# Mingqj/DFU3D

Hardware: AMD Instinct MI355X
Metric: pseudo-box frames/sec (34k pts, 6 cams) (higher is better)
Workload: dtype f64; 1 GPU; configs[1] with depth back-projection on (dense): 64 synthetic frames/GPU/step, 34720-pt sweep, 6 cams x 1600x900 depth + 8 instance masks (one bit-packed 1-byte word per pixel), 30-40 objects/scene; views_per_launch_chunk=192, streams=2, parallelism=frames sharded x1

## Files before the change

dfu3d_amd/_build.py:

```python
import glob
import os
import subprocess
import sys

HERE = os.path.dirname(os.path.abspath(__file__))
CSRC = os.path.join(HERE, "csrc")
INCLUDE = os.path.join(os.path.dirname(HERE), "include")
OUT = os.path.join(CSRC, "libdfu3d_hip.so")

FLAGS = [
    "--offload-arch=gfx950", "-O3", "-std=c++17", "-fPIC", "-shared",
    "-ffp-contract=off", "-fhip-fp32-correctly-rounded-divide-sqrt",
    "-fno-fast-math", "-Wall", "-Wno-unused-function",
]


def sources():
    return sorted(glob.glob(os.path.join(CSRC, "*.hip")))


def needs_build():
    return _stale(OUT)


def _deps():
    return (sources() + glob.glob(os.path.join(CSRC, "*.hpp")) + glob.glob(os.path.join(CSRC, "*.inc"))
            + [os.path.join(INCLUDE, "dfu3d.h")])


def _stale(out):
    return not os.path.exists(out) or any(os.path.getmtime(d) > os.path.getmtime(out) for d in _deps())


def _compile(out, extra, verbose):
    import fcntl
    import tempfile
    with open(out + ".lock", "w") as lock:
        fcntl.flock(lock, fcntl.LOCK_EX)
        try:
            if not _stale(out) and not extra.get("force"):
                return out
            hipcc = os.environ.get("HIPCC", "/opt/rocm/bin/hipcc")
            fd, tmp = tempfile.mkstemp(prefix=os.path.basename(out) + ".", suffix=".tmp", dir=os.path.dirname(out))
            os.close(fd)
            cmd = [hipcc] + FLAGS + extra.get("flags", []) + ["-I", INCLUDE, "-I", CSRC] + sources() + ["-o", tmp]
            if verbose:
                print(" ".join(cmd))
            try:
                subprocess.check_call(cmd)
                os.replace(tmp, out)
            finally:
                if os.path.exists(tmp):
                    os.unlink(tmp)
        finally:
            fcntl.flock(lock, fcntl.LOCK_UN)
    return out


def build(force=False, verbose=False):
    if not force and not needs_build():
        return OUT
    return _compile(OUT, {"force": force, "flags": os.environ.get("DFU3D_EXTRA_HIPCC_FLAGS", "").split()}, verbose)


VARIANTS = {
    "keybits14": ["-DDFU3D_DBG_COMBO_KEYBITS=14"],
    "no_mid": ["-DDFU3D_DBG_NO_MID"],
    "timing": ["-DDFU3D_DBG_TIMING"],
    "asan_host": ["-O1", "-g", "-Xarch_host", "-fsanitize=address", "-Xarch_host", "-fsanitize=undefined",
                  "-Xarch_host", "-fno-sanitize-recover=undefined", "-Xarch_host", "-fno-omit-frame-pointer", "-shared-libsan"],
}


def variant_path(name):
    return os.path.join(CSRC, "libdfu3d_hip_%s.so" % name)


def build_variant(name, force=False, verbose=False):
    out = variant_path(name)
    if not force and not _stale(out):
        return out
    return _compile(out, {"force": force, "flags": VARIANTS[name]}, verbose)


if __name__ == "__main__":
    print(build(force="--force" in sys.argv, verbose=True))
```

dfu3d_amd/csrc/chain_stage.hip:

```cpp
#include "common.hpp"

namespace {

struct ChainWs {
  int32_t *fov_idx, *cand_idx, *ag_pt, *ib_pix, *n_fov, *n_ag, *K;
  double *plane;
  uint32_t *a_bits;
  double *a_x, *a_y, *a_z;
  int32_t *n_vox;
  uint32_t *vox_pix, *b_bits;
  double *b_x, *b_y, *b_z;
  void *table;
  uint32_t *pix_bin;
  int32_t *blk_cnt;
  double *px, *py, *pz, *sx, *sy;
  int32_t *label, *sroot, *si3;
  double *fit_ws;
  uint8_t *flags;
  int64_t *base_a, *base_b, *base_ab;
  int32_t *cnt_a, *cnt_b, *cnt_all, *cnt_ab, *tile_off, *queue, *stat_enable;
  double *rad_ab, *mean_d;
  void *vd_scratch;
  void *shadow;
  int32_t *chunk_cnt;
  int64_t *pool_cursor;
  int64_t table_entries;
};

int64_t carve(const dfu3d_chain_cfg *c, char *base, ChainWs *w) {
  int64_t off = 0;
  auto take = [&](int64_t bytes) -> char * {
    char *p = base ? base + off : nullptr;
    off += (bytes + 255) / 256 * 256;
    return p;
  };
  const int64_t V = c->V, S = (int64_t)c->V * c->max_inst, N = V * c->cap_n, X = V * c->cap_vox, P = c->pool_cap;
  ChainWs t;
  t.fov_idx = (int32_t *)take(4 * N); t.cand_idx = (int32_t *)take(4 * N);
  t.ag_pt = (int32_t *)take(4 * N); t.ib_pix = (int32_t *)take(4 * N);
  t.n_fov = (int32_t *)take(4 * V); t.n_ag = (int32_t *)take(4 * V); t.K = (int32_t *)take(4 * V);
  t.plane = (double *)take(8 * V * 4);
  t.a_bits = (uint32_t *)take(4 * N);
  t.a_x = (double *)take(8 * N); t.a_y = (double *)take(8 * N); t.a_z = (double *)take(8 * N);
  t.n_vox = (int32_t *)take(4 * V);
  t.vox_pix = (uint32_t *)take(4 * X); t.b_bits = (uint32_t *)take(4 * X);
  t.b_x = (double *)take(8 * X); t.b_y = (double *)take(8 * X); t.b_z = (double *)take(8 * X);
  t.table_entries = (int64_t)c->geom.t_n * c->geom.p_n;
  int64_t pw = 0, bw = 0;
  if (c->dense) {
    dfu3d_backproject_scratch_words(c->V, c->H, c->W, c->cap_vox, c->geom.max_points_per_voxel, t.table_entries, &pw, &bw);
    t.table = take(V * t.table_entries * DFU3D_TABLE_ENTRY_BYTES);
    t.pix_bin = (uint32_t *)take(4 * pw);
    t.blk_cnt = (int32_t *)take(4 * bw);
  } else {
    t.table = nullptr; t.pix_bin = nullptr; t.blk_cnt = nullptr;
  }
  t.px = (double *)take(8 * P); t.py = (double *)take(8 * P); t.pz = (double *)take(8 * P);
  t.sx = (double *)take(8 * P); t.sy = (double *)take(8 * P);
  t.label = (int32_t *)take(4 * P); t.sroot = (int32_t *)take(4 * P); t.si3 = (int32_t *)take(4 * 3 * P);
  t.fit_ws = (double *)take(8 * dfu3d_lshape_fit_ws_doubles(P, c->cap_rows));
  t.flags = (uint8_t *)take(P);
  t.base_a = (int64_t *)take(8 * S); t.base_b = (int64_t *)take(8 * S); t.base_ab = (int64_t *)take(8 * 2 * S);
  t.cnt_a = (int32_t *)take(4 * S); t.cnt_b = (int32_t *)take(4 * S); t.cnt_all = (int32_t *)take(4 * S);
  t.cnt_ab = (int32_t *)take(4 * 2 * S); t.tile_off = (int32_t *)take(4 * (2 * S + 2));
  t.queue = (int32_t *)take(4 * DFU3D_RF_QUEUE_INTS(P)); t.stat_enable = (int32_t *)take(4 * S);
  t.shadow = take(DFU3D_SHADOW_BYTES(P));
  t.chunk_cnt = (int32_t *)take(4 * dfu3d_segments_scratch_words(c->V, c->cap_n, c->cap_vox));
  t.rad_ab = (double *)take(8 * 2 * S);
  t.mean_d = c->stat_filter ? (double *)take(8 * P) : nullptr;
  t.vd_scratch = c->stat_filter ? (void *)take(dfu3d_voxel_down_sample_scratch_bytes(P)) : nullptr;
  t.pool_cursor = (int64_t *)take(8);
  if (w) *w = t;
  return off;
}

bool cfg_ok(const dfu3d_chain_cfg *c) {
  return c && c->V > 0 && c->H > 0 && c->W > 0 && c->max_inst > 0 && c->max_inst <= DFU3D_MAX_INST &&
         c->cap_n > 0 && c->cap_vox > 0 && c->cap_rows > 0 && c->pool_cap > 0 && c->n_theta > 0 &&
         c->bounds_h > 0 && c->bounds_w > 0 && c->bounds_h <= c->H && c->bounds_w <= c->W &&
         mask_format_ok(c->mask_format, c->max_inst) &&
         (!c->dense || (c->geom.t_n > 0 && c->geom.p_n > 0)) &&
         (!c->stat_filter || (c->stat_voxel > 0.0 && c->stat_nb_neighbors >= 1));
}

__global__ void k_all_points(const int *__restrict__ pt_off, const int *__restrict__ view_frame,
                             int cap_n, int *__restrict__ fov_idx, int *__restrict__ n_fov) {
  const int v = blockIdx.y;
  const int f = view_frame[v];
  const int n = min(pt_off[f + 1] - pt_off[f], cap_n);
  for (int i = blockIdx.x * blockDim.x + threadIdx.x; i < cap_n; i += gridDim.x * blockDim.x)
    fov_idx[(size_t)v * cap_n + i] = i;
  if (blockIdx.x == 0 && threadIdx.x == 0) n_fov[v] = n;
}

__global__ void k_sum_counts(int S, const int *__restrict__ a, const int *__restrict__ b, int *__restrict__ out) {
  const int s = blockIdx.x * blockDim.x + threadIdx.x;
  if (s < S) out[s] = a[s] + b[s];
}

__global__ void k_fill_i32(int n, int v, int *__restrict__ p) {
  const int i = blockIdx.x * blockDim.x + threadIdx.x;
  if (i < n) p[i] = v;
}

}

extern "C" int64_t dfu3d_chain_workspace_bytes(const dfu3d_chain_cfg *cfg) {
  if (!cfg_ok(cfg)) return DFU3D_EINVAL;
  return carve(cfg, nullptr, nullptr);
}

extern "C" int64_t dfu3d_workspace_bytes(int32_t stage, const dfu3d_sizes *z) {
  if (!z || z->V <= 0 || z->max_inst <= 0 || z->max_inst > DFU3D_MAX_INST) return DFU3D_EINVAL;
  auto up = [](int64_t b) { return (b + 255) / 256 * 256; };
  const int64_t V = z->V, S = V * z->max_inst, P = z->pool_cap, N = V * (int64_t)z->cap_n;
  switch (stage) {
    case DFU3D_STAGE_FOV_FILTER:
      return 0;
    case DFU3D_STAGE_SEGMENTS_BUILD:
      return (z->cap_n > 0 && z->cap_vox > 0) ? up(4 * dfu3d_segments_scratch_words(z->V, z->cap_n, z->cap_vox)) : DFU3D_EINVAL;
    case DFU3D_STAGE_PLANE_RANSAC:
      return z->cap_n > 0 ? up(4 * N) : DFU3D_EINVAL;
    case DFU3D_STAGE_PROJECT_LABEL:
      return z->cap_n > 0 ? 2 * up(4 * N) : DFU3D_EINVAL;
    case DFU3D_STAGE_BACKPROJECT_BIN: {
      int64_t pw = 0, bw = 0;
      if (z->table_entries <= 0 ||
          dfu3d_backproject_scratch_words(z->V, z->H, z->W, z->cap_vox, z->max_points_per_voxel, z->table_entries, &pw, &bw))
        return DFU3D_EINVAL;
      return up(V * z->table_entries * DFU3D_TABLE_ENTRY_BYTES) + up(4 * pw) + up(4 * bw);
    }
    case DFU3D_STAGE_RADIUS_FILTER:
      return P > 0 ? up(DFU3D_SHADOW_BYTES(P)) + up(4 * (2 * S + 1)) + up(P) + up(4 * DFU3D_RF_QUEUE_INTS(P)) : DFU3D_EINVAL;
    case DFU3D_STAGE_STAT_FILTER:
      return P > 0 ? up(4 * (S + 1)) + up(P) + up(8 * P) : DFU3D_EINVAL;
    case DFU3D_STAGE_VOXEL_DOWN_SAMPLE:
      return P > 0 ? up(dfu3d_voxel_down_sample_scratch_bytes(P)) : DFU3D_EINVAL;
    case DFU3D_STAGE_BALLQUERY_FUSE:
      return P > 0 ? up(4 * (2 * S + 2)) + up(P) : DFU3D_EINVAL;
    case DFU3D_STAGE_RANGE_CLUSTER:
      return P > 0 ? 2 * up(8 * P) + up(12 * P) : DFU3D_EINVAL;
    case DFU3D_STAGE_LSHAPE_FIT:
      return (P > 0 && z->cap_rows > 0)
                 ? 2 * up(8 * P) + up(4 * P) + up(8 * dfu3d_lshape_fit_ws_doubles(P, z->cap_rows)) : DFU3D_EINVAL;
    case DFU3D_STAGE_PSEUDO_BOXES: {
      dfu3d_chain_cfg c = {};
      c.V = z->V; c.H = z->H; c.W = z->W; c.max_inst = z->max_inst; c.cap_n = z->cap_n; c.cap_vox = z->cap_vox;
      c.cap_rows = z->cap_rows; c.dense = z->dense; c.stat_filter = z->stat_filter; c.pool_cap = z->pool_cap;
      c.bounds_h = z->H; c.bounds_w = z->W; c.n_theta = 1;
      c.geom.max_points_per_voxel = z->max_points_per_voxel;
      c.geom.t_n = 1; c.geom.p_n = (int32_t)z->table_entries;
      if (z->dense && (z->table_entries <= 0 || z->table_entries > 0x7FFFFFFF)) return DFU3D_EINVAL;
      return dfu3d_chain_workspace_bytes(&c);
    }
    default:
      return DFU3D_EINVAL;
  }
}

extern "C" int dfu3d_chain_workspace_init(const dfu3d_chain_cfg *cfg, void *workspace, void *stream) {
  DFU3D_CLEAR_STALE_ERROR();
  if (!cfg_ok(cfg) || !workspace) return DFU3D_EINVAL;
  ChainWs w;
  carve(cfg, (char *)workspace, &w);
  if (cfg->dense) {
    const int rc = dfu3d_bin_table_init(w.table, (int64_t)cfg->V * w.table_entries, stream);
    if (rc) return rc;
  }
  hipLaunchKernelGGL(k_fill_i32, dim3((cfg->V * cfg->max_inst + 255) / 256), dim3(256), 0,
                     (hipStream_t)stream, cfg->V * cfg->max_inst, 1, w.stat_enable);
  DFU3D_LAUNCH_CHECK();
  return DFU3D_OK;
}

#define CHAIN_TRY(call)      \
  do {                       \
    const int rc_ = (call);  \
    if (rc_) return rc_;     \
  } while (0)

extern "C" int dfu3d_pseudo_boxes(
    const dfu3d_chain_cfg *cfg, const float *points, const int32_t *pt_off,
    const int32_t *view_frame, const float *calib, const void *masks, const int32_t *n_inst,
    const float *depth, const int64_t *view_key, const double *plane_in, const int32_t *inst_class,
    const int32_t *inst_is_car, const double *inst_r_lidar, const double *inst_r_pseudo,
    const float *inst_box, const float *inst_score, void *workspace, double *rows, int32_t *n_rows,
    uint32_t *status, void *stream) {
  DFU3D_CLEAR_STALE_ERROR();
  if (!cfg_ok(cfg) || !points || !pt_off || !view_frame || !calib || !masks || !n_inst || !inst_class ||
      !inst_is_car || !inst_r_lidar || !inst_r_pseudo || !inst_box || !inst_score || !workspace || !rows ||
      !n_rows || !status)
    return DFU3D_EINVAL;
  if (!plane_in && !view_key) return DFU3D_EINVAL;
  if (cfg->dense && !depth) return DFU3D_EINVAL;
  ChainWs w;
  carve(cfg, (char *)workspace, &w);
  hipStream_t st = (hipStream_t)stream;
  const int V = cfg->V, M = cfg->max_inst, S = V * M, cap_n = cfg->cap_n;
  if (dfu3d_fill_small_async(n_rows, sizeof(int32_t), status, sizeof(uint32_t), w.pool_cursor, sizeof(int64_t), st) != hipSuccess)
    return DFU3D_ELAUNCH;
  if (cfg->apply_fov) {
    CHAIN_TRY(dfu3d_fov_filter(points, pt_off, view_frame, calib, V, cfg->fov_h, cfg->fov_w, cap_n,
                               w.fov_idx, w.n_fov, stream));
  } else {
    hipLaunchKernelGGL(k_all_points, dim3((cap_n + 255) / 256 < 64 ? (cap_n + 255) / 256 : 64, V), dim3(256), 0, st,
                       pt_off, view_frame, cap_n, w.fov_idx, w.n_fov);
    DFU3D_LAUNCH_CHECK();
  }
  const double *plane = plane_in;
  if (!plane) {
    CHAIN_TRY(dfu3d_plane_ransac(points, pt_off, view_frame, w.fov_idx, w.n_fov, V, cap_n, cfg->plane_max_hs,
                                 cfg->plane_range, cfg->ransac_trials, cfg->ransac_seed, view_key,
                                 w.cand_idx, w.plane, stream));
    plane = w.plane;
  }
  CHAIN_TRY(dfu3d_project_label(points, pt_off, view_frame, calib, plane, w.fov_idx, w.n_fov, masks,
                                cfg->mask_format, n_inst, V, M, cfg->H, cfg->W, cfg->bounds_h, cfg->bounds_w,
                                cap_n, cfg->plane_offset, cfg->plane_range, w.ag_pt,
                                w.ib_pix, w.n_ag, w.K, w.a_bits, w.a_x, w.a_y, w.a_z, stream));
  if (cfg->dense) {
    CHAIN_TRY(dfu3d_backproject_bin(depth, calib, masks, cfg->mask_format, n_inst, V, M, cfg->H, cfg->W, &cfg->geom, 1, w.table,
                                    w.pix_bin, w.blk_cnt, cfg->cap_vox, w.n_vox, w.vox_pix, w.b_bits, w.b_x,
                                    w.b_y, w.b_z, status, DFU3D_BP_ALL, stream));
  } else {
    if (dfu3d_fill_async(w.n_vox, 0, sizeof(int32_t) * V, st) != hipSuccess) return DFU3D_ELAUNCH;
  }
  const bool joint = !cfg->stat_filter;
  CHAIN_TRY(dfu3d_segments_build(w.a_bits, w.a_x, w.a_y, w.a_z, w.K, cap_n, w.b_bits, w.b_x, w.b_y, w.b_z,
                                 w.n_vox, cfg->cap_vox, V, M, cfg->pool_cap, w.pool_cursor, w.px, w.py, w.pz,
                                 w.base_a, w.cnt_a, w.base_b, w.cnt_b, status, inst_r_lidar, inst_r_pseudo,
                                 joint ? w.shadow : nullptr, joint ? w.base_ab : nullptr, w.cnt_ab, w.rad_ab,
                                 w.chunk_cnt, stream));
  if (joint) {
    CHAIN_TRY(dfu3d_radius_filter(w.px, w.py, w.pz, w.base_ab, w.cnt_ab, w.rad_ab, cfg->nb_points, 2 * S,
                                  cfg->pool_cap, w.pool_cursor, w.shadow, w.tile_off, w.flags, w.queue,
                                  DFU3D_RF_FLAGS | DFU3D_RF_RESOLVE, stream));
    CHAIN_TRY(dfu3d_ballquery_fuse_joint(w.px, w.py, w.pz, w.base_a, w.cnt_a, w.base_b, w.cnt_b, cfg->fuse_C,
                                          S, cfg->pool_cap, w.tile_off, w.flags, stream));
  } else {
    CHAIN_TRY(dfu3d_radius_filter(w.px, w.py, w.pz, w.base_a, w.cnt_a, inst_r_lidar, cfg->nb_points, S,
                                  cfg->pool_cap, w.pool_cursor, w.shadow, w.tile_off, w.flags, w.queue,
                                  DFU3D_RF_ALL, stream));
    CHAIN_TRY(dfu3d_radius_filter(w.px, w.py, w.pz, w.base_b, w.cnt_b, inst_r_pseudo, cfg->nb_points, S,
                                  cfg->pool_cap, w.pool_cursor, w.shadow, w.tile_off, w.flags, w.queue,
                                  DFU3D_RF_ALL, stream));
    CHAIN_TRY(dfu3d_voxel_down_sample(w.px, w.py, w.pz, w.base_b, w.cnt_b, w.stat_enable, cfg->stat_voxel, S,
                                      cfg->pool_cap, w.vd_scratch, status, stream));
    CHAIN_TRY(dfu3d_stat_filter(w.px, w.py, w.pz, w.base_b, w.cnt_b, w.stat_enable, cfg->stat_nb_neighbors,
                                cfg->stat_std_ratio, S, cfg->pool_cap, w.tile_off, w.flags, w.mean_d, nullptr,
                                stream));
    CHAIN_TRY(dfu3d_ballquery_fuse(w.px, w.py, w.pz, w.base_a, w.cnt_a, w.base_b, w.cnt_b, cfg->fuse_C, S,
                                   cfg->pool_cap, w.tile_off, w.flags, stream));
  }
  hipLaunchKernelGGL(k_sum_counts, dim3((S + 255) / 256), dim3(256), 0, st, S, w.cnt_a, w.cnt_b, w.cnt_all);
  DFU3D_LAUNCH_CHECK();
  CHAIN_TRY(dfu3d_range_cluster(w.px, w.py, w.base_a, w.cnt_all, S, cfg->R0, cfg->Rd, w.label, w.sx, w.sy,
                                w.si3, cfg->pool_cap, stream));
  CHAIN_TRY(dfu3d_lshape_fit(w.px, w.py, w.pz, w.label, w.base_a, w.cnt_all, S, M, calib, inst_class,
                             inst_is_car, inst_box, inst_score, cfg->n_theta, cfg->dtheta, cfg->car_aspect_max,
                             w.sx, w.sy, w.sroot, cfg->cap_rows, rows, n_rows, status, w.fit_ws, cfg->pool_cap,
                             stream));
  return DFU3D_OK;
}
```

dfu3d_amd/csrc/common.hpp:

```cpp
#pragma once
#include <hip/hip_runtime.h>
#include <stdint.h>

#include "dfu3d.h"

#define DFU3D_WAVE 64

struct ViewCalib {
  float M43[12];
  float P2[12];
  float cu, cv, fu, fv, tx, ty;
  float Minv[12];
  float pad[6];
};
static_assert(sizeof(ViewCalib) == DFU3D_CALIB_FLOATS * 4, "calib record");

__device__ __forceinline__ int lane_id() { return threadIdx.x & 63; }

__device__ __forceinline__ int wave_rank(bool flag, int &wave_total) {
  const unsigned long long m = __ballot(flag);
  wave_total = __popcll(m);
  return __popcll(m & ((1ull << lane_id()) - 1ull));
}

template <int NW>
__device__ __forceinline__ int block_rank(bool flag, int *s_w, int &block_total) {
  int wt;
  const int r = wave_rank(flag, wt);
  const int w = threadIdx.x >> 6;
  if (lane_id() == 0) s_w[w] = wt;
  __syncthreads();
  int off = 0, tot = 0;
#pragma unroll
  for (int i = 0; i < NW; i++) {
    const int c = s_w[i];
    off += (i < w) ? c : 0;
    tot += c;
  }
  __syncthreads();
  block_total = tot;
  return off + r;
}

template <int CTRL, int ROW_MASK>
__device__ __forceinline__ int dpp_move_i(int old, int v) {
  return __builtin_amdgcn_update_dpp(old, v, CTRL, ROW_MASK, 0xF, false);
}
__device__ __forceinline__ int wave_incl_scan(int v) {
  v += dpp_move_i<0x111, 0xF>(0, v);
  v += dpp_move_i<0x112, 0xF>(0, v);
  v += dpp_move_i<0x114, 0xF>(0, v);
  v += dpp_move_i<0x118, 0xF>(0, v);
  v += dpp_move_i<0x142, 0xA>(0, v);
  v += dpp_move_i<0x143, 0xC>(0, v);
  return v;
}
__device__ __forceinline__ int wave_sum_i_dpp(int v) {
  v += dpp_move_i<0xB1, 0xF>(v, v);
  v += dpp_move_i<0x4E, 0xF>(v, v);
  v += dpp_move_i<0x141, 0xF>(v, v);
  v += dpp_move_i<0x140, 0xF>(v, v);
  v += dpp_move_i<0x142, 0xA>(0, v);
  v += dpp_move_i<0x143, 0xC>(0, v);
  return __builtin_amdgcn_readlane(v, 63);
}
__device__ __forceinline__ int wave_min_i_dpp(int v) {
  v = min(v, dpp_move_i<0xB1, 0xF>(v, v));
  v = min(v, dpp_move_i<0x4E, 0xF>(v, v));
  v = min(v, dpp_move_i<0x141, 0xF>(v, v));
  v = min(v, dpp_move_i<0x140, 0xF>(v, v));
  v = min(v, dpp_move_i<0x142, 0xA>(v, v));
  v = min(v, dpp_move_i<0x143, 0xC>(v, v));
  return __builtin_amdgcn_readlane(v, 63);
}
__device__ __forceinline__ uint32_t wave_or_u32_dpp(uint32_t x) {
  int v = (int)x;
  v |= dpp_move_i<0xB1, 0xF>(v, v);
  v |= dpp_move_i<0x4E, 0xF>(v, v);
  v |= dpp_move_i<0x141, 0xF>(v, v);
  v |= dpp_move_i<0x140, 0xF>(v, v);
  v |= dpp_move_i<0x142, 0xA>(0, v);
  v |= dpp_move_i<0x143, 0xC>(0, v);
  return (uint32_t)__builtin_amdgcn_readlane(v, 63);
}

template <int NW>
__device__ __forceinline__ int block_excl_scan(int v, int *s_w, int &block_total) {
  const int inc = wave_incl_scan(v);
  const int w = threadIdx.x >> 6;
  if (lane_id() == 63) s_w[w] = inc;
  __syncthreads();
  int off = 0, tot = 0;
#pragma unroll
  for (int i = 0; i < NW; i++) {
    const int c = s_w[i];
    off += (i < w) ? c : 0;
    tot += c;
  }
  __syncthreads();
  block_total = tot;
  return off + inc - v;
}

__device__ __forceinline__ double shfl_xor_d(double v, int m) {
  int lo = __double2loint(v), hi = __double2hiint(v);
  lo = __shfl_xor(lo, m, 64);
  hi = __shfl_xor(hi, m, 64);
  return __hiloint2double(hi, lo);
}
__device__ __forceinline__ double wave_sum_d(double v) {
#pragma unroll
  for (int m = 32; m >= 1; m >>= 1) v += shfl_xor_d(v, m);
  return v;
}
template <int CTRL, int ROW_MASK>
__device__ __forceinline__ double dpp_move_d(double v) {
  int lo = __double2loint(v), hi = __double2hiint(v);
  lo = __builtin_amdgcn_update_dpp(lo, lo, CTRL, ROW_MASK, 0xF, false);
  hi = __builtin_amdgcn_update_dpp(hi, hi, CTRL, ROW_MASK, 0xF, false);
  return __hiloint2double(hi, lo);
}
__device__ __forceinline__ double min_f64_raw(double a, double b) {
  double r;
  asm("v_min_f64 %0, %1, %2" : "=v"(r) : "v"(a), "v"(b));
  return r;
}
__device__ __forceinline__ double max_f64_raw(double a, double b) {
  double r;
  asm("v_max_f64 %0, %1, %2" : "=v"(r) : "v"(a), "v"(b));
  return r;
}
__device__ __forceinline__ double lane63_d(double v) {
  return __hiloint2double(__builtin_amdgcn_readlane(__double2hiint(v), 63), __builtin_amdgcn_readlane(__double2loint(v), 63));
}
__device__ __forceinline__ double wave_min_d(double v) {
  v = min_f64_raw(v, dpp_move_d<0xB1, 0xF>(v));
  v = min_f64_raw(v, dpp_move_d<0x4E, 0xF>(v));
  v = min_f64_raw(v, dpp_move_d<0x141, 0xF>(v));
  v = min_f64_raw(v, dpp_move_d<0x140, 0xF>(v));
  v = min_f64_raw(v, dpp_move_d<0x142, 0xA>(v));
  v = min_f64_raw(v, dpp_move_d<0x143, 0xC>(v));
  return lane63_d(v);
}
__device__ __forceinline__ double wave_max_d(double v) {
  v = max_f64_raw(v, dpp_move_d<0xB1, 0xF>(v));
  v = max_f64_raw(v, dpp_move_d<0x4E, 0xF>(v));
  v = max_f64_raw(v, dpp_move_d<0x141, 0xF>(v));
  v = max_f64_raw(v, dpp_move_d<0x140, 0xF>(v));
  v = max_f64_raw(v, dpp_move_d<0x142, 0xA>(v));
  v = max_f64_raw(v, dpp_move_d<0x143, 0xC>(v));
  return lane63_d(v);
}
__device__ __forceinline__ unsigned long long wave_sum_u64(unsigned long long v) {
#pragma unroll
  for (int m = 32; m >= 1; m >>= 1) {
    const unsigned int lo = (unsigned int)__shfl_xor((int)(v & 0xFFFFFFFFull), m, 64);
    const unsigned int hi = (unsigned int)__shfl_xor((int)(v >> 32), m, 64);
    v += ((unsigned long long)hi << 32) | lo;
  }
  return v;
}
__device__ __forceinline__ int wave_sum_i(int v) { return wave_sum_i_dpp(v); }

__device__ __forceinline__ void lidar_to_rect_f32(const float *M, float x, float y,
                                                  float z, float r[3]) {
#pragma unroll
  for (int j = 0; j < 3; j++) {
    float acc = x * M[0 * 3 + j];
    acc = __fmaf_rn(y, M[1 * 3 + j], acc);
    acc = __fmaf_rn(z, M[2 * 3 + j], acc);
    acc = acc + M[3 * 3 + j];
    r[j] = acc;
  }
}
__device__ __forceinline__ void rect_to_img_f32(const float *P2, const float r[3],
                                                float &u, float &v, float &depth) {
  float h[3];
#pragma unroll
  for (int j = 0; j < 3; j++) {
    float acc = r[0] * P2[j * 4 + 0];
    acc = __fmaf_rn(r[1], P2[j * 4 + 1], acc);
    acc = __fmaf_rn(r[2], P2[j * 4 + 2], acc);
    acc = acc + P2[j * 4 + 3];
    h[j] = acc;
  }
  u = h[0] / r[2];
  v = h[1] / r[2];
  depth = h[2] - P2[2 * 4 + 3];
}
struct Recip { double rfu, rfv; };
__device__ __forceinline__ Recip make_recip(const ViewCalib &c) {
  Recip r;
  r.rfu = 1.0 / (double)c.fu;
  r.rfv = 1.0 / (double)c.fv;
  return r;
}
__device__ __forceinline__ double div_reused(double a, double b, double r) {
  const double q0 = a * r;
  const uint32_t hi = (uint32_t)__double2hiint(q0) & 0x7FFFFFFFu;
  if (__builtin_expect(hi - 0x07B00000u >= 0x78400000u - 0x07B00000u, 0)) return a / b;
  const double rem = fma(-q0, b, a);
  return fma(rem, r, q0);
}
__device__ __forceinline__ void pixel_to_lidar(const ViewCalib &c, const Recip &rc, int u, int v,
                                               float d, double &x, double &y,
                                               double &z) {
  const double dd = (double)d;
  const double xr = div_reused(((double)u - (double)c.cu) * dd, (double)c.fu, rc.rfu) + (double)c.tx;
  const double yr = div_reused(((double)v - (double)c.cv) * dd, (double)c.fv, rc.rfv) + (double)c.ty;
  const double zr = dd;
  const float *M = c.Minv;
  x = fma(zr, (double)M[6], fma(yr, (double)M[3], xr * (double)M[0])) + (double)M[9];
  y = fma(zr, (double)M[7], fma(yr, (double)M[4], xr * (double)M[1])) + (double)M[10];
  z = fma(zr, (double)M[8], fma(yr, (double)M[5], xr * (double)M[2])) + (double)M[11];
}
struct KeyCol { float m0, m3, m6, m9; };
__device__ __forceinline__ KeyCol load_key_col(const ViewCalib *c, int axis) {
  const float *M = c->Minv + axis;
  KeyCol k;
  k.m0 = M[0]; k.m3 = M[3]; k.m6 = M[6]; k.m9 = M[9];
  return k;
}
struct KeyCal { float cu, cv, fu, fv, tx, ty; };
__device__ __forceinline__ KeyCal key_cal(const ViewCalib &c) { return KeyCal{c.cu, c.cv, c.fu, c.fv, c.tx, c.ty}; }
template <class Cal>
__device__ __forceinline__ double pixel_to_lidar_axis(const Cal &c, const Recip &rc, const KeyCol &kc, int u, int v,
                                                      float d) {
  const double dd = (double)d;
  const double xr = div_reused(((double)u - (double)c.cu) * dd, (double)c.fu, rc.rfu) + (double)c.tx;
  const double yr = div_reused(((double)v - (double)c.cv) * dd, (double)c.fv, rc.rfv) + (double)c.ty;
  return fma(dd, (double)kc.m6, fma(yr, (double)kc.m3, xr * (double)kc.m0)) + (double)kc.m9;
}

__host__ __device__ inline bool mask_format_ok(int fmt, int max_inst) {
  return fmt == 0 || (fmt == 1 && max_inst <= 8) || (fmt == 2 && max_inst <= 16) || fmt == 4;
}
__device__ __forceinline__ uint32_t mask_bits_at(const void *masks, int fmt, int v, int max_inst, int m,
                                                 int HW, int pix) {
  if (fmt == 0) {
    const uint8_t *mb = (const uint8_t *)masks + (size_t)v * max_inst * HW + pix;
    uint32_t bits = 0u;
    for (int j = 0; j < m; j++) bits |= (mb[(size_t)j * HW] > 0) ? (1u << j) : 0u;
    return bits;
  }
  const size_t o = (size_t)v * HW + pix;
  const uint32_t w = fmt == 1 ? (uint32_t)((const uint8_t *)masks)[o]
                   : fmt == 2 ? (uint32_t)((const uint16_t *)masks)[o] : ((const uint32_t *)masks)[o];
  return m >= 32 ? w : (w & ((1u << m) - 1u));
}

__device__ __forceinline__ unsigned long long ordered_key(double v) {
  const unsigned long long b = (unsigned long long)__double_as_longlong(v);
  return (b & 0x8000000000000000ull) ? ~b : (b | 0x8000000000000000ull);
}

__device__ __forceinline__ unsigned long long mix64(unsigned long long z) {
  z += 0x9E3779B97F4A7C15ull;
  z = (z ^ (z >> 30)) * 0xBF58476D1CE4E5B9ull;
  z = (z ^ (z >> 27)) * 0x94D049BB133111EBull;
  return z ^ (z >> 31);
}

#define DFU3D_CLEAR_STALE_ERROR() (void)hipGetLastError()

#define DFU3D_LAUNCH_CHECK()                                      \
  do {                                                            \
    if (hipGetLastError() != hipSuccess) return DFU3D_ELAUNCH;    \
  } while (0)

namespace {
__global__ __launch_bounds__(256) void k_fill_words(uint32_t *__restrict__ p, size_t n, uint32_t v) {
  const size_t head = ((16u - (unsigned)((uintptr_t)p & 15u)) & 15u) / 4u < n ? ((16u - (unsigned)((uintptr_t)p & 15u)) & 15u) / 4u : n;
  uint4 *q = (uint4 *)(p + head);
  const size_t nq = (n - head) / 4;
  const size_t tid = (size_t)blockIdx.x * 256 + threadIdx.x, nth = (size_t)gridDim.x * 256;
  for (size_t i = tid; i < nq; i += nth) q[i] = make_uint4(v, v, v, v);
  const size_t done = head + nq * 4;
  if (tid < head) p[tid] = v;
  if (tid < n - done) p[done + tid] = v;
}
__global__ void k_fill_small(uint32_t *a, int na, uint32_t *b, int nb, uint32_t *c, int nc, uint32_t v) {
  for (int i = threadIdx.x; i < na; i += blockDim.x) a[i] = v;
  for (int i = threadIdx.x; i < nb; i += blockDim.x) b[i] = v;
  for (int i = threadIdx.x; i < nc; i += blockDim.x) c[i] = v;
}
}
static inline hipError_t dfu3d_fill_async(void *p, int value, size_t bytes, hipStream_t st) {
  if (bytes == 0) return hipSuccess;
  if (((uintptr_t)p & 3u) || (bytes & 3u)) return hipMemsetAsync(p, value, bytes, st);
  const uint32_t b = (uint32_t)(value & 0xFF), v = b | (b << 8) | (b << 16) | (b << 24);
  const size_t n = bytes / 4, quads = (n + 3) / 4;
  const unsigned grid = (unsigned)((quads + 255) / 256 < 8192 ? (quads + 255) / 256 : 8192);
  hipLaunchKernelGGL(k_fill_words, dim3(grid ? grid : 1), dim3(256), 0, st, (uint32_t *)p, n, v);
  return hipGetLastError();
}
static inline hipError_t dfu3d_fill_small_async(void *a, size_t bytes_a, void *b, size_t bytes_b, void *c, size_t bytes_c, hipStream_t st) {
  hipLaunchKernelGGL(k_fill_small, dim3(1), dim3(256), 0, st, (uint32_t *)a, (int)(bytes_a / 4), (uint32_t *)b, (int)(bytes_b / 4),
                     (uint32_t *)c, (int)(bytes_c / 4), 0u);
  return hipGetLastError();
}
```

dfu3d_amd/csrc/dbg.hpp:

```cpp
#pragma once

#ifdef DFU3D_DBG_COMBO_KEYBITS
constexpr int DBG_COMBO_KEYBITS = DFU3D_DBG_COMBO_KEYBITS;
#else
constexpr int DBG_COMBO_KEYBITS = 64;
#endif

#ifdef DFU3D_DBG_NO_MID
constexpr bool DBG_NO_MID = true;
#else
constexpr bool DBG_NO_MID = false;
#endif

#ifdef DFU3D_DBG_TIMING
constexpr int DBG_T_SLOTS = 32;
static __device__ unsigned long long g_dbg_cycles[DBG_T_SLOTS];
#define DBG_T_START() long long dbg_t_ = clock64(); const long long dbg_t0_ = dbg_t_; (void)dbg_t0_
#define DBG_T(k) do { if (threadIdx.x == 0) { const long long t_ = clock64(); atomicAdd(&g_dbg_cycles[k], (unsigned long long)(t_ - dbg_t_)); dbg_t_ = t_; } } while (0)
#define DBG_T_COUNT(k) do { if (threadIdx.x == 0) atomicAdd(&g_dbg_cycles[k], 1ull); } while (0)
#define DBG_T_ADD(k, v) do { if (threadIdx.x == 0) atomicAdd(&g_dbg_cycles[k], (unsigned long long)(v)); } while (0)
#define DBG_T_MAX(k, v) do { if (threadIdx.x == 0) atomicMax(&g_dbg_cycles[k], (unsigned long long)(v)); } while (0)
#define DBG_T_READER(name)                                                                                              \
  extern "C" int name(unsigned long long *out, int reset) {                                                            \
    if (hipMemcpyFromSymbol(out, HIP_SYMBOL(g_dbg_cycles), sizeof(unsigned long long) * DBG_T_SLOTS) != hipSuccess)     \
      return DFU3D_ELAUNCH;                                                                                             \
    if (reset) {                                                                                                        \
      unsigned long long z[DBG_T_SLOTS] = {0};                                                                          \
      if (hipMemcpyToSymbol(HIP_SYMBOL(g_dbg_cycles), z, sizeof(z)) != hipSuccess) return DFU3D_ELAUNCH;                \
    }                                                                                                                   \
    return DFU3D_OK;                                                                                                    \
  }
#else
#define DBG_T_START() do {} while (0)
#define DBG_T(k) do {} while (0)
#define DBG_T_COUNT(k) do {} while (0)
#define DBG_T_ADD(k, v) do {} while (0)
#define DBG_T_MAX(k, v) do {} while (0)
#define DBG_T_READER(name)
#endif
```

dfu3d_amd/csrc/fit_stage.hip:

```cpp
#include "common.hpp"

namespace {
__device__ __forceinline__ int rl_i(int v, int l) { return __builtin_amdgcn_readlane(v, l); }
__device__ __forceinline__ double rl_d(double v, int l) {
  return __hiloint2double(__builtin_amdgcn_readlane(__double2hiint(v), l), __builtin_amdgcn_readlane(__double2loint(v), l));
}

constexpr int CT = 512;
constexpr int GRP = 32;
constexpr int BLK = 32;
constexpr int PAIR_SMALL = 32;
constexpr int GU = 4;
constexpr int SMALL_N = 4096;
constexpr int LARGE_N = 61440;
constexpr int LARGE_GRP = LARGE_N / GRP;
constexpr int GRID_NC_SMALL = 4096;
constexpr int GRID_NC_LARGE = 12288;

struct ParI {
  int *p;
  bool global;
  __device__ __forceinline__ int load(int i) const {
    return __hip_atomic_load(p + i, __ATOMIC_RELAXED, __HIP_MEMORY_SCOPE_AGENT);
  }
// ... 353 lines not shown
__device__ __forceinline__ int grid_cell(const GridGeom<NC> &G, double x, double y, int &cx, int &cy) {
  cx = (int)fmin(fmax((x - G.x0) * G.inv, 0.0), (double)(G.nx - 1));
  cy = (int)fmin(fmax((y - G.y0) * G.inv, 0.0), (double)(G.ny - 1));
  return (int)__umul24((uint32_t)cy, (uint32_t)G.nx) + cx;
}
template <int NC>
__device__ __forceinline__ int grid_cell(const GridGeom<NC> &G, double x, double y) {
  int cx, cy;
  return grid_cell(G, x, y, cx, cy);
}

__device__ __forceinline__ int cell_find(int *par_, int a) {
  volatile int *par = par_;
  int p = par[a];
  while (p != a) {
    const int gp = par[p];
    if (gp != p) par[a] = gp;
    a = p;
    p = gp;
  }
  return a;
}
__device__ __forceinline__ void cell_unite(int *par, int a, int b) {
  while (true) {
    a = cell_find(par, a);
    b = cell_find(par, b);
    if (a == b) return;
    if (a < b) { const int t = a; a = b; b = t; }
    const int old = atomicMin(par + a, b);
    if (old == a) return;
    a = old;
  }
}

constexpr int CL_CLASSES = 3, CL_TOP = 8192;
template <int NC, int NC_MIN, int TCT>
__global__ __launch_bounds__(TCT, (NC <= GRID_NC_SMALL ? 8 : 4)) void k_range_cluster_grid(
    const double *__restrict__ px, const double *__restrict__ py,
    const long long *__restrict__ seg_base, const int *__restrict__ seg_cnt, double R0,
    double Rd, int *__restrict__ label, double *__restrict__ sx, double *__restrict__ sy,
    int *__restrict__ perm_all, long long pool_cap, int n_lo, int n_hi) {
  __shared__ int s_end[NC];
  __shared__ int s_par[NC];
  __shared__ int s_min[NC];
  __shared__ double s_red[5 * (TCT / 64)];
  __shared__ int s_w[TCT / 64];
  constexpr int NCLS = CL_CLASSES;
  const int S_ = (int)(gridDim.x / (unsigned)NCLS);
  const int cls = (int)(blockIdx.x / (unsigned)S_);
  const int s = (int)(blockIdx.x - (unsigned)cls * (unsigned)S_);
  const int n = seg_cnt[s];
  if (n <= n_lo || n > n_hi) return;
  {
    int mine = NCLS - 1;
#pragma unroll
    for (int k = NCLS - 2; k >= 0; k--) if (n > (CL_TOP >> k)) mine = k;
    if (mine != cls) return;
  }
  const long long base = seg_base[s];
  const double *X = px + base, *Y = py + base;
  double *SX = sx + base, *SY = sy + base;
  int *perm = perm_all + base;
  int *mark = perm_all + 2 * pool_cap + base;
  if (NC_MIN > 0 && *mark) return;
  const GridGeom<NC> G = grid_geometry<NC, TCT>(X, Y, n, R0, Rd, s_red);
  if (threadIdx.x == 0 && (NC_MIN == 0 || G.ok)) *mark = G.ok ? 1 : 0;
  if (!G.ok) return;
  const int ncell = G.ncell;
  for (int c = threadIdx.x; c < ncell; c += TCT) { s_end[c] = 0; s_par[c] = c; s_min[c] = 0x7FFFFFFF; }
  __syncthreads();
  for (int i0 = threadIdx.x; i0 < n; i0 += GU * TCT) {
    double xs[GU], ys[GU];
#pragma unroll
    for (int u = 0; u < GU; u++) {
      const int i = i0 + u * TCT;
      xs[u] = (i < n) ? X[i] : 0.0; ys[u] = (i < n) ? Y[i] : 0.0;
    }
#pragma unroll
    for (int u = 0; u < GU; u++)
      if (i0 + u * TCT < n) atomicAdd(&s_end[grid_cell(G, xs[u], ys[u])], 1);
  }
  __syncthreads();
  {
    const int per = (ncell + TCT - 1) / TCT;
    const int c_lo = min((int)threadIdx.x * per, ncell), c_hi = min(c_lo + per, ncell);
    int mine = 0;
    for (int c = c_lo; c < c_hi; c++) mine += s_end[c];
    int tot;
    int run = block_excl_scan<TCT / 64>(mine, s_w, tot);
    for (int c = c_lo; c < c_hi; c++) { const int h = s_end[c]; s_end[c] = run; run += h; }
  }
  __syncthreads();
  for (int i0 = threadIdx.x; i0 < n; i0 += GU * TCT) {
    double xs[GU], ys[GU];
#pragma unroll
    for (int u = 0; u < GU; u++) {
      const int i = i0 + u * TCT;
      xs[u] = (i < n) ? X[i] : 0.0; ys[u] = (i < n) ? Y[i] : 0.0;
    }
#pragma unroll
    for (int u = 0; u < GU; u++) {
      const int i = i0 + u * TCT;
      if (i >= n) break;
      const int pos = atomicAdd(&s_end[grid_cell(G, xs[u], ys[u])], 1);
      SX[pos] = xs[u];
      SY[pos] = ys[u];
      perm[pos] = i;
    }
  }
  __syncthreads();
  const double S_HI = G.Rmax * G.Rmax * (1.0 + 1e-9);
  const double S_LO = R0 * R0 * (1.0 - 1e-12);
  const int lane = lane_id();
  int *s_box = s_min;
  for (int c = threadIdx.x; c < ncell; c += TCT) s_box[c] = (int)0x00FF00FFu;
  __syncthreads();
  for (int i0 = threadIdx.x; i0 < n; i0 += GU * TCT) {
    double xs[GU], ys[GU];
#pragma unroll
    for (int u = 0; u < GU; u++) {
      const int i = i0 + u * TCT;
      xs[u] = (i < n) ? SX[i] : 0.0; ys[u] = (i < n) ? SY[i] : 0.0;
    }
#pragma unroll
    for (int u = 0; u < GU; u++) {
      if (i0 + u * TCT >= n) break;
      int cx, cy;
      const int c = grid_cell(G, xs[u], ys[u], cx, cy);
      const double fu = (xs[u] - G.x0) * G.inv - (double)cx, fv = (ys[u] - G.y0) * G.inv - (double)cy;
      const unsigned ulo = (unsigned)(int)fmin(fmax(floor(fu * 256.0), 0.0), 255.0);
      const unsigned uhi = (unsigned)(int)fmin(fmax(ceil(fu * 256.0) - 1.0, 0.0), 255.0);
      const unsigned vlo = (unsigned)(int)fmin(fmax(floor(fv * 256.0), 0.0), 255.0);
      const unsigned vhi = (unsigned)(int)fmin(fmax(ceil(fv * 256.0) - 1.0, 0.0), 255.0);
      unsigned old = (unsigned)__hip_atomic_load(&s_box[c], __ATOMIC_RELAXED, __HIP_MEMORY_SCOPE_WORKGROUP);
      while (true) {
        const unsigned nw = min(old & 255u, ulo) | (max((old >> 8) & 255u, uhi) << 8) |
                            (min((old >> 16) & 255u, vlo) << 16) | (max(old >> 24, vhi) << 24);
        if (nw == old) break;
        const unsigned seen = (unsigned)atomicCAS(&s_box[c], (int)old, (int)nw);
        if (seen == old) break;
        old = seen;
      }
    }
  }
  __syncthreads();
  const double box_lim = S_HI * (1.0 + 1e-6) * (G.inv * G.inv);
  auto boxes_apart = [&](int c, int cx, int cy, int nbc, int qx, int qy) {
    const unsigned a = (unsigned)s_box[c], b = (unsigned)s_box[nbc];
    const int ax0 = cx * 256 + (int)(a & 255u), ax1 = cx * 256 + (int)((a >> 8) & 255u) + 1;
    const int ay0 = cy * 256 + (int)((a >> 16) & 255u), ay1 = cy * 256 + (int)(a >> 24) + 1;
    const int bx0 = qx * 256 + (int)(b & 255u), bx1 = qx * 256 + (int)((b >> 8) & 255u) + 1;
    const int by0 = qy * 256 + (int)((b >> 16) & 255u), by1 = qy * 256 + (int)(b >> 24) + 1;
    const int gx = max(max(bx0 - ax1, ax0 - bx1) - 2, 0), gy = max(max(by0 - ay1, ay0 - by1) - 2, 0);
    const double g2 = (double)(gx * gx + gy * gy) * (1.0 / 65536.0);
    return g2 > box_lim;
  };
  struct CellBox { double x0, x1, y0, y1; };
  auto cell_box = [&](int c) {
    const unsigned a = (unsigned)s_box[c];
    const int cx = c % G.nx, cy = c / G.nx;
    CellBox B;
    B.x0 = G.x0 + ((double)cx + (double)((int)(a & 255u) - 1) * (1.0 / 256.0)) * G.g;
    B.x1 = G.x0 + ((double)cx + (double)((int)((a >> 8) & 255u) + 2) * (1.0 / 256.0)) * G.g;
    B.y0 = G.y0 + ((double)cy + (double)((int)((a >> 16) & 255u) - 1) * (1.0 / 256.0)) * G.g;
    B.y1 = G.y0 + ((double)cy + (double)((int)(a >> 24) + 2) * (1.0 / 256.0)) * G.g;
    return B;
  };
  const double reach2 = S_HI * (1.0 + 1e-6);
  auto near_box = [&](const CellBox &B, double x, double y) {
    const double dx = fmax(fmax(B.x0 - x, x - B.x1), 0.0), dy = fmax(fmax(B.y0 - y, y - B.y1), 0.0);
    return dx * dx + dy * dy <= reach2;
  };
  const int ODX[12] = {1, -1, 0, 1, 2, -2, -1, 0, 1, 2, -2, 2};
  const int ODY[12] = {0, 1, 1, 1, 0, 2, 2, 2, 2, 2, 1, 1};
  for (int round = 0; round < 2; round++) {
    const int o_lo = round ? 4 : 0, n_off = round ? 8 : 4;
    const int items = ncell * n_off;
    const int iters = (items + TCT - 1) / TCT;
    for (int it = 0; it < iters; it++) {
      const int idx = it * TCT + threadIdx.x;
      int c = 0, nb = 0;
      bool need = false;
      if (idx < items) {
        c = idx / n_off;
        const int o = o_lo + (idx - c * n_off);
        const int cx = c % G.nx, cy = c / G.nx;
        const int qx = cx + ODX[o], qy = cy + ODY[o];
        if (qx >= 0 && qx < G.nx && qy < G.ny) {
          nb = qy * G.nx + qx;
          const int a0 = c ? s_end[c - 1] : 0, b0 = s_end[nb - 1];
          need = (s_end[c] > a0) && (s_end[nb] > b0) && !boxes_apart(c, cx, cy, nb, qx, qy) &&
                 (cell_find(s_par, c) != cell_find(s_par, nb));
        }
      }
      if (need) {
        const int a0 = c ? s_end[c - 1] : 0, a1 = s_end[c];
        const int b0 = s_end[nb - 1], b1 = s_end[nb];
        if (a1 - a0 <= PAIR_SMALL && b1 - b0 <= PAIR_SMALL) {
          need = false;
          bool found = false;
          const CellBox BB = cell_box(nb);
          for (int i = a0; i < a1 && !found; i++) {
            const double xa = SX[i], ya = SY[i];
            if (!near_box(BB, xa, ya)) continue;
            const double Ra = R0 + Rd * sqrt(xa * xa + ya * ya);
            for (int j0 = b0; j0 < b1 && !found; j0 += 4) {
              double xb4[4], yb4[4];
#pragma unroll
              for (int u = 0; u < 4; u++) {
                const int j = min(j0 + u, b1 - 1);
                xb4[u] = SX[j]; yb4[u] = SY[j];
              }
#pragma unroll
              for (int u = 0; u < 4; u++) {
                if (j0 + u >= b1) break;
                const double xb = xb4[u], yb = yb4[u];
                const double dx = xa - xb, dy = ya - yb;
                const double sq = dx * dx + dy * dy;
                if (sq > S_HI) continue;
                if (sq <= S_LO) { found = true; break; }
                const double d = sqrt(sq);
                if (d <= Ra || d <= R0 + Rd * sqrt(xb * xb + yb * yb)) { found = true; break; }
              }
            }
          }
          if (found) cell_unite(s_par, c, nb);
        }
      }
      unsigned long long todo = __ballot(need);
      while (todo) {
        const int src = __ffsll(todo) - 1;
        todo &= todo - 1ull;
        const int cc = rl_i(c, src), nn = rl_i(nb, src);
        if (cell_find(s_par, cc) == cell_find(s_par, nn)) continue;
        const int a0 = cc ? s_end[cc - 1] : 0, a1 = s_end[cc];
        const int b0 = s_end[nn - 1], b1 = s_end[nn];
        bool found = false;
        const CellBox BA = cell_box(cc), BB = cell_box(nn);
        for (int b_lo = b0; b_lo < b1 && !found; b_lo += 64) {
          const int ib = b_lo + lane;
          const double xb = (ib < b1) ? SX[ib] : 0.0, yb = (ib < b1) ? SY[ib] : 0.0;
          const bool vb = (ib < b1) && near_box(BA, xb, yb);
          if (!__any(vb)) continue;
          for (int a_lo = a0; a_lo < a1 && !found; a_lo += 64) {
            const int ia = a_lo + lane;
            const double xal = (ia < a1) ? SX[ia] : 0.0, yal = (ia < a1) ? SY[ia] : 0.0;
            unsigned long long am = __ballot((ia < a1) && near_box(BB, xal, yal));
            bool adj = false;
            int steps = 0;
            while (am) {
              const int k = __ffsll((long long)am) - 1;
              am &= am - 1ull;
              const double xa = rl_d(xal, k), ya = rl_d(yal, k);
              const double dx = xa - xb, dy = ya - yb;
              const double sq = dx * dx + dy * dy;
              if (vb && sq <= S_HI) {
                if (sq <= S_LO) adj = true;
                else {
                  const double d = sqrt(sq);
                  adj = adj || (d <= R0 + Rd * sqrt(xa * xa + ya * ya)) ||
                        (d <= R0 + Rd * sqrt(xb * xb + yb * yb));
                }
              }
              if ((++steps & 15) == 0 && __any(adj)) break;
            }
            found = __any(adj);
          }
        }
        if (found && lane == 0) cell_unite(s_par, cc, nn);
      }
    }
    __syncthreads();
  }
  for (int c = threadIdx.x; c < ncell; c += TCT) s_min[c] = 0x7FFFFFFF;
  __syncthreads();
  for (int i0 = threadIdx.x; i0 < n; i0 += GU * TCT) {
    double xs[GU], ys[GU];
    int pm[GU];
#pragma unroll
    for (int u = 0; u < GU; u++) {
      const int i = i0 + u * TCT;
      xs[u] = (i < n) ? SX[i] : 0.0; ys[u] = (i < n) ? SY[i] : 0.0; pm[u] = (i < n) ? perm[i] : 0;
    }
#pragma unroll
    for (int u = 0; u < GU; u++)
      if (i0 + u * TCT < n) atomicMin(&s_min[cell_find(s_par, grid_cell(G, xs[u], ys[u]))], pm[u]);
  }
  __syncthreads();
  int *glabel = label + base;
  for (int i0 = threadIdx.x; i0 < n; i0 += GU * TCT) {
    double xs[GU], ys[GU];
    int pm[GU];
#pragma unroll
    for (int u = 0; u < GU; u++) {
      const int i = i0 + u * TCT;
      xs[u] = (i < n) ? SX[i] : 0.0; ys[u] = (i < n) ? SY[i] : 0.0; pm[u] = (i < n) ? perm[i] : 0;
    }
#pragma unroll
    for (int u = 0; u < GU; u++)
      if (i0 + u * TCT < n) glabel[pm[u]] = s_min[cell_find(s_par, grid_cell(G, xs[u], ys[u]))];
  }
}

__global__ __launch_bounds__(CT) void k_range_cluster_small(
    const double *__restrict__ px, const double *__restrict__ py,
    const long long *__restrict__ seg_base, const int *__restrict__ seg_cnt, double R0,
    double Rd, int *__restrict__ label, double *__restrict__ sx, double *__restrict__ sy,
    int *__restrict__ si, long long pool_cap) {
  __shared__ __attribute__((aligned(16))) int s_parent[SMALL_N];
  __shared__ int s_summ[SMALL_N / GRP];
  __shared__ float4 s_box[SMALL_N / GRP];
  __shared__ int s_summ2[SMALL_N / GRP / BLK];
  __shared__ float4 s_box2[SMALL_N / GRP / BLK];
  __shared__ double s_red[4 * (CT / 64)];
  __shared__ int s_w[CT / 64];
  const int s = blockIdx.x;
  const int n = seg_cnt[s];
  if (n == 0 || n > SMALL_N) return;
  const long long base = seg_base[s];
  if (si[2 * pool_cap + base]) return;
  cell_sort<SMALL_N>(px + base, py + base, n, s_parent, s_red, s_w, sx + base, sy + base, si + base);
  ParI par{s_parent, false};
  cluster_body<ParI, SMALL_N / GRP>(par, s_summ, s_box, s_summ2, s_box2, s_red, sx + base, sy + base,
                                    n, R0, Rd, si + base, si + pool_cap + base, label + base);
}

__global__ __launch_bounds__(CT) void k_range_cluster_large(
    const double *__restrict__ px, const double *__restrict__ py,
    const long long *__restrict__ seg_base, const int *__restrict__ seg_cnt, double R0,
    double Rd, int *__restrict__ label, double *__restrict__ sx, double *__restrict__ sy,
    int *__restrict__ si, long long pool_cap) {
  __shared__ __attribute__((aligned(16))) unsigned short s_parent[LARGE_N];
  __shared__ int s_summ[LARGE_GRP];
  __shared__ float4 s_box[LARGE_GRP];
  __shared__ int s_summ2[LARGE_GRP / BLK];
  __shared__ float4 s_box2[LARGE_GRP / BLK];
  __shared__ double s_red[4 * (CT / 64)];
  __shared__ int s_w[CT / 64];
  const int s = blockIdx.x;
  const int n = seg_cnt[s];
  if (n <= SMALL_N) return;
  const long long base = seg_base[s];
  if (si[2 * pool_cap + base]) return;
  cell_sort<LARGE_N / 2>(px + base, py + base, n, (int *)s_parent, s_red, s_w, sx + base, sy + base,
                         si + base);
  if (n <= LARGE_N) {
    ParH par{s_parent};
    cluster_body<ParH, LARGE_GRP>(par, s_summ, s_box, s_summ2, s_box2, s_red, sx + base, sy + base,
                                  n, R0, Rd, si + base, si + pool_cap + base, label + base);
  } else {
    ParI par{si + 2 * pool_cap + base, true};
    cluster_body<ParI, LARGE_GRP>(par, s_summ, s_box, s_summ2, s_box2, s_red, sx + base, sy + base,
                                  n, R0, Rd, si + base, si + pool_cap + base, label + base);
  }
}

constexpr int FT = 512;
constexpr int FW = FT / 64;
constexpr int MAXTH = 128;
constexpr int LDS_MEMBERS = 2048;

struct OpSum { __device__ static double f(double a, double b) { return a + b; } };
struct OpMin { __device__ static double f(double a, double b) { return fmin(a, b); } };
struct OpMax { __device__ static double f(double a, double b) { return fmax(a, b); } };
template <class OP>
__device__ __forceinline__ double wave_red(double v) {
#pragma unroll
  for (int m = 32; m >= 1; m >>= 1) v = OP::f(v, shfl_xor_d(v, m));
  return v;
}

struct Ext { double c1min, c1max, c2min, c2max; };

__device__ __forceinline__ double readlane_f64(double v, int l) {
  const int lo = __builtin_amdgcn_readlane(__double2loint(v), l);
  const int hi = __builtin_amdgcn_readlane(__double2hiint(v), l);
  return __hiloint2double(hi, lo);
}

__device__ __forceinline__ void cross_point(double a0, double a1, double b0, double b1,
                                            double c0, double c1, double &x, double &y) {
  x = (b0 * -c1 - b1 * -c0) / (a0 * b1 - a1 * b0);
  y = (a1 * -c0 - a0 * -c1) / (a0 * b1 - a1 * b0);
}

__device__ void emit_box(double thb, double sin_s, double cos_s, double c1min, double c1max,
                         double c2min, double c2max, double zmax, int s, int v, int jinst, int kc,
                         int root, int m, const ViewCalib *calib, const int *inst_class,
                         const int *inst_is_car, const float *inst_box, const float *inst_score,
                         double car_aspect_max, int cap_rows, double *rows, int *n_rows,
                         uint32_t *status) {
  const double a[4] = {cos_s, -sin_s, cos_s, -sin_s};
  const double b[4] = {sin_s, cos_s, sin_s, cos_s};
  const double c[4] = {c1min, c2min, c1max, c2max};
  double cx[4], cy[4];
  cross_point(a[0], a[1], b[0], b[1], c[0], c[1], cx[0], cy[0]);
  cross_point(a[1], a[2], b[1], b[2], c[1], c[2], cx[1], cy[1]);
  cross_point(a[2], a[3], b[2], b[3], c[2], c[3], cx[2], cy[2]);
  cross_point(a[3], a[0], b[3], b[0], c[3], c[0], cx[3], cy[3]);
  double center_x = (cx[0] + cx[2]) / 2.0;
  double center_y = (cy[0] + cy[2]) / 2.0;
  const double center_z = zmax / 2.0 - 1.5;
  const double height = zmax;
  const double e03x = cx[0] - cx[3], e03y = cy[0] - cy[3];
  const double e01x = cx[0] - cx[1], e01y = cy[0] - cy[1];
  const double l1 = sqrt(e03x * e03x + e03y * e03y);
  const double l2 = sqrt(e01x * e01x + e01y * e01y);
  bool skip = false;
  if (inst_is_car[s] && (l1 / l2 > car_aspect_max || l2 / l1 > car_aspect_max)) skip = true;
  double length = 0.0, width = 0.0, rotation = 0.0;
  if (l1 >= l2) {
    length = l1; width = l2;
    rotation = atan((cy[3] - cy[0]) / (cx[3] - cx[0] + 1e-8));
  } else if (l1 < l2) {
    length = l2; width = l1;
    rotation = atan((cy[1] - cy[0]) / (cx[1] - cx[0] + 1e-8));
  } else {
    skip = true;
  }
  if (!skip) {
    const double kPi = 3.141592653589793;
    rotation = -rotation - kPi / 2.0;
    const double theta = atan(-center_x / (center_y + 1e-8));
    const double alpha = rotation - theta;
    const float *M = calib[v].M43;
    const double rx = ((center_x * (double)M[0] + center_y * (double)M[3]) + center_z * (double)M[6]) + (double)M[9];
    const double ry = ((center_x * (double)M[1] + center_y * (double)M[4]) + center_z * (double)M[7]) + (double)M[10];
    const double rz = ((center_x * (double)M[2] + center_y * (double)M[5]) + center_z * (double)M[8]) + (double)M[11];
    const int slot = atomicAdd(n_rows, 1);
    if (slot < cap_rows) {
      double *o = rows + (size_t)slot * DFU3D_ROW_DOUBLES;
      o[0] = (double)v; o[1] = (double)jinst; o[2] = (double)kc;
      o[3] = (double)inst_class[s]; o[4] = alpha;
      o[5] = (double)inst_box[s * 4 + 0]; o[6] = (double)inst_box[s * 4 + 1];
      o[7] = (double)inst_box[s * 4 + 2]; o[8] = (double)inst_box[s * 4 + 3];
      o[9] = height; o[10] = width; o[11] = length;
      o[12] = rx; o[13] = ry; o[14] = rz; o[15] = rotation;
      o[16] = (double)inst_score[s]; o[17] = (double)m;
      o[18] = thb; o[19] = c1min; o[20] = c2min; o[21] = c1max; o[22] = c2max;
      o[23] = (double)root;
    } else {
      atomicOr(status, DFU3D_ST_ROW_OVERFLOW);
    }
  }
}

struct FitWs {
  int *counters;
  double *dsc;
  int *big_list;
  double *big_cost;
  int cap_q, cap_big;
};
__host__ __device__ inline int fit_cap_q(int cap_rows) { return 2 * cap_rows + 64; }
__host__ __device__ inline FitWs fit_ws_view(double *ws, int cap_rows, int cap_big) {
  FitWs w;
  w.cap_q = fit_cap_q(cap_rows);
  w.cap_big = cap_big;
  w.counters = (int *)ws;
  w.dsc = ws + 2;
  w.big_list = (int *)(w.dsc + (size_t)8 * w.cap_q);
  w.big_cost = w.dsc + (size_t)8 * w.cap_q + (cap_big / 2 + 1);
  return w;
}

constexpr int GK = 512;

__device__ __forceinline__ int rank_in(const int *roots, int nk, int L) {
  int lo = 0, hi = nk - 1;
  while (lo < hi) {
    const int mid = (lo + hi) >> 1;
    if (roots[mid] < L) lo = mid + 1; else hi = mid;
  }
  return (roots[lo] == L) ? lo : -1;
}

constexpr int GGU = 4;
__global__ __launch_bounds__(FT) void k_fit_gather(
    const double *__restrict__ px, const double *__restrict__ py,
    const double *__restrict__ pz, const int *__restrict__ label,
    const long long *__restrict__ seg_base, const int *__restrict__ seg_cnt,
    double *__restrict__ gsx, double *__restrict__ gsy, int *__restrict__ sroot,
    uint32_t *__restrict__ status, double *__restrict__ fit_ws, int cap_rows, int cap_big) {
  __shared__ int s_roots[GK];
  __shared__ int s_cnt[FW][GK];
  __shared__ int s_tot[GK], s_off[GK];
  __shared__ double s_red[FW];
  __shared__ int s_w[FW];
  __shared__ int s_q0, s_total;
  const int S_ = (int)(gridDim.x / 3u);
  const int cls = (int)(blockIdx.x / (unsigned)S_);
  const int s = (int)(blockIdx.x - (unsigned)cls * (unsigned)S_);
  const int n = seg_cnt[s];
  if (n == 0) return;
  if (cls != (n > 16384 ? 0 : (n > 8192 ? 1 : 2))) return;
  const long long base = seg_base[s];
  const int wave = threadIdx.x >> 6, lane = lane_id();
  const FitWs W = fit_ws_view(fit_ws, cap_rows, cap_big);

  const int R = (((n + FW - 1) / FW) + 63) & ~63;
  const int r0 = min(n, wave * R), r1 = min(n, r0 + R);
  double zm = -INFINITY;
  int mine = 0;
  for (int c = r0; c < r1; c += 64 * GGU) {
    int L[GGU];
    double zz[GGU];
#pragma unroll
    for (int u = 0; u < GGU; u++) {
      const int i = c + u * 64 + lane;
      L[u] = (i < r1) ? label[base + i] : -1;
      zz[u] = (i < r1) ? pz[base + i] : -INFINITY;
    }
#pragma unroll
    for (int u = 0; u < GGU; u++) {
      const int i = c + u * 64 + lane;
      mine += __popcll(__ballot(i < r1 && L[u] == i));
      zm = fmax(zm, zz[u]);
    }
  }
  zm = wave_max_d(zm);
  if (lane == 0) { s_red[wave] = zm; s_w[wave] = mine; }
  __syncthreads();
  double zmax = s_red[0];
  int nroots = 0, my_off = 0;
#pragma unroll
  for (int w = 0; w < FW; w++) {
    zmax = fmax(zmax, s_red[w]);
    my_off += (w < wave) ? s_w[w] : 0;
    nroots += s_w[w];
  }
  for (int c = r0; c < r1; c += 64 * GGU) {
    int L[GGU];
#pragma unroll
    for (int u = 0; u < GGU; u++) {
      const int i = c + u * 64 + lane;
      L[u] = (i < r1) ? label[base + i] : -1;
    }
#pragma unroll
    for (int u = 0; u < GGU; u++) {
      const int i = c + u * 64 + lane;
      const bool f = (i < r1) && (L[u] == i);
      const unsigned long long m = __ballot(f);
      if (f) sroot[base + my_off + __popcll(m & ((1ull << lane) - 1ull))] = i;
      my_off += __popcll(m);
    }
  }
  if (threadIdx.x == 0) s_q0 = atomicAdd(&W.counters[0], nroots);
  __syncthreads();
  const int q0 = s_q0;

  long long goff = 0;
  for (int k0 = 0; k0 < nroots; k0 += GK) {
    const int nk = min(GK, nroots - k0);
    __syncthreads();
    if (threadIdx.x < nk) s_roots[threadIdx.x] = sroot[base + k0 + threadIdx.x];
    for (int i = threadIdx.x; i < FW * GK; i += FT) (&s_cnt[0][0])[i] = 0;
    __syncthreads();
    const int lo_root = s_roots[0], hi_root = s_roots[nk - 1];
    int memo_L = -2, memo_key = -1;
    for (int c0 = r0; c0 < r1; c0 += 64 * GGU) {
      int Ls[GGU];
#pragma unroll
      for (int u = 0; u < GGU; u++) {
        const int i = c0 + u * 64 + lane;
        Ls[u] = (i < r1) ? label[base + i] : -1;
      }
#pragma unroll
      for (int u = 0; u < GGU; u++) {
        if (c0 + u * 64 >= r1) break;
        const int L = Ls[u];
        int key = -1;
        if (L == memo_L) key = memo_key;
        else if (L >= lo_root && L <= hi_root) { key = rank_in(s_roots, nk, L); memo_L = L; memo_key = key; }
        unsigned long long rem = __ballot(key >= 0);
        while (rem) {
          const int src = __ffsll((long long)rem) - 1;
          const int k = rl_i(key, src);
          const unsigned long long m = __ballot(key == k);
          if (lane == src) s_cnt[wave][k] += __popcll(m);
          rem &= ~m;
        }
      }
    }
    __syncthreads();
    if (threadIdx.x < nk) {
      int t = 0;
#pragma unroll
      for (int w = 0; w < FW; w++) { const int c = s_cnt[w][threadIdx.x]; s_cnt[w][threadIdx.x] = t; t += c; }
      s_tot[threadIdx.x] = t;
    }
    __syncthreads();
    {
      int tot;
      const int ex = block_excl_scan<FW>(((int)threadIdx.x < nk) ? s_tot[threadIdx.x] : 0, s_w, tot);
      if ((int)threadIdx.x < nk) s_off[threadIdx.x] = ex;
      if (threadIdx.x == 0) s_total = tot;
    }
    __syncthreads();
    for (int c0 = r0; c0 < r1; c0 += 64 * GGU) {
      int keys[GGU];
      double xs[GGU], ys[GGU];
#pragma unroll
      for (int u = 0; u < GGU; u++) {
        const int i = c0 + u * 64 + lane;
        const int L = (i < r1) ? label[base + i] : -1;
        if (L == memo_L) keys[u] = memo_key;
        else if (L >= lo_root && L <= hi_root) { keys[u] = rank_in(s_roots, nk, L); memo_L = L; memo_key = keys[u]; }
        else keys[u] = -1;
      }
#pragma unroll
      for (int u = 0; u < GGU; u++) {
        const int i = c0 + u * 64 + lane;
        xs[u] = 0.0; ys[u] = 0.0;
        if (keys[u] >= 0) { xs[u] = px[base + i]; ys[u] = py[base + i]; }
      }
#pragma unroll
      for (int u = 0; u < GGU; u++) {
        if (c0 + u * 64 >= r1) break;
        const int key = keys[u];
        unsigned long long rem = __ballot(key >= 0);
        while (rem) {
          const int src = __ffsll((long long)rem) - 1;
          const int k = rl_i(key, src);
          const unsigned long long m = __ballot(key == k);
          const int cur = s_cnt[wave][k];
          if (key == k) {
            const long long d = base + goff + s_off[k] + cur + __popcll(m & ((1ull << lane) - 1ull));
            gsx[d] = xs[u];
            gsy[d] = ys[u];
          }
          if (lane == src) s_cnt[wave][k] = cur + __popcll(m);
          rem &= ~m;
        }
      }
    }
    if (threadIdx.x < nk) {
      const int k = threadIdx.x, e = q0 + k0 + k;
      if (e < W.cap_q) {
        double *d = W.dsc + (size_t)8 * e;
        const int m = s_tot[k];
        d[0] = (double)s; d[1] = (double)(k0 + k); d[2] = (double)s_roots[k]; d[3] = (double)m;
        d[4] = (double)(base + goff + s_off[k]); d[5] = zmax; d[6] = -1.0; d[7] = 0.0;
        if (m > LDS_MEMBERS) {
          const int bi = atomicAdd(&W.counters[1], 1);
          if (bi < cap_big) { W.big_list[bi] = e; d[6] = (double)bi; }
        }
// ... 196 lines not shown
          }
          double V1 = 0.0, V2 = 0.0;
          if (n1) V1 = -(q1 / (double)n1);
          if (n2) V2 = -(q2 / (double)n2);
          const double c = V1 + V2;
          if (c1t[k] >= band && bestc < c) { bestc = c; bestth = th; }
        }
      }
    }
#pragma unroll
    for (int msk = 32; msk >= 1; msk >>= 1) {
      const double oc = shfl_xor_d(bestc, msk);
      const int ot = __shfl_xor(bestth, msk, 64);
      if (oc > bestc || (oc == bestc && ot < bestth)) { bestc = oc; bestth = ot; }
    }
    const int best = (bestth == 0x7FFFFFFF) ? 0 : bestth;
    const double thb = (double)best * dtheta;
    const double sin_s = sin(thb), cos_s = cos(thb);
    double a0 = INFINITY, a1 = -INFINITY, b0 = INFINITY, b1 = -INFINITY;
    if (lane < m) {
      const double c1 = x * cos_s + y * sin_s;
      const double c2 = x * (-sin_s) + y * cos_s;
      a0 = c1; a1 = c1; b0 = c2; b1 = c2;
    }
    a0 = wave_min_d(a0); a1 = wave_max_d(a1);
    b0 = wave_min_d(b0); b1 = wave_max_d(b1);
    if (lane == 0) {
      const int s = (int)d[0], kc = (int)d[1], root = (int)d[2];
      const int v = s / max_inst, jinst = s - v * max_inst;
      emit_box(thb, sin_s, cos_s, a0, a1, b0, b1, d[5], s, v, jinst, kc, root, m, calib, inst_class,
               inst_is_car, inst_box, inst_score, car_aspect_max, cap_rows, rows, n_rows, status);
    }
  }
}

__global__ __launch_bounds__(FT, 8) void k_fit_medium(
    const double *__restrict__ gsx, const double *__restrict__ gsy, int max_inst,
    const ViewCalib *__restrict__ calib, const int *__restrict__ inst_class,
    const int *__restrict__ inst_is_car, const float *__restrict__ inst_box,
    const float *__restrict__ inst_score, int n_theta, double dtheta, double car_aspect_max,
    int cap_rows, double *__restrict__ rows, int *__restrict__ n_rows,
    uint32_t *__restrict__ status, double *__restrict__ fit_ws, int cap_big) {
  __shared__ double lx[LDS_MEMBERS], ly[LDS_MEMBERS];
  __shared__ double s_cost[MAXTH], s_mag[MAXTH], s_ct[MAXTH], s_st[MAXTH];
  __shared__ double s_ext[FW][4];
  const FitWs W = fit_ws_view(fit_ws, cap_rows, cap_big);
  const int nq = min(W.counters[0], W.cap_q);
  const int wave = threadIdx.x >> 6, lane = lane_id();
  if (threadIdx.x < MAXTH) {
    const double theta = (double)threadIdx.x * dtheta;
    s_ct[threadIdx.x] = cos(theta);
    s_st[threadIdx.x] = sin(theta);
  }
  __shared__ int s_item;
  while (true) {
    __syncthreads();
    if (wave == 0) {
      const int ticket = atomicAdd(&W.counters[3], 1);
      if (lane == 0) s_item = ticket >> 6;
    }
    __syncthreads();
    const int e = s_item;
    if (e >= nq) break;
    const double *d = W.dsc + (size_t)8 * e;
    const int m = (int)d[3];
    if (m <= 64 || m > LDS_MEMBERS) continue;
    __syncthreads();
    const long long P = (long long)d[4];
    for (int i = threadIdx.x; i < m; i += FT) { lx[i] = gsx[P + i]; ly[i] = gsy[P + i]; }
    __syncthreads();
    const double *mx = lx;
    const double *my = ly;
    for (int th0 = 2 * wave; th0 < n_theta; th0 += 2 * FW) {
      const int th1 = min(th0 + 1, n_theta - 1);
      const double ct0 = s_ct[th0], st0 = s_st[th0], ct1 = s_ct[th1], st1 = s_st[th1];
      double a0 = INFINITY, a1 = -INFINITY, b0 = INFINITY, b1 = -INFINITY;
      double e0 = INFINITY, e1 = -INFINITY, f0 = INFINITY, f1 = -INFINITY;
      for (int i = lane; i < m; i += 64) {
        const double x = mx[i], y = my[i];
        double c1 = x * ct0 + y * st0;
        double c2 = x * (-st0) + y * ct0;
        a0 = min_raw_d(a0, c1); a1 = max_raw_d(a1, c1);
        b0 = min_raw_d(b0, c2); b1 = max_raw_d(b1, c2);
        c1 = x * ct1 + y * st1;
        c2 = x * (-st1) + y * ct1;
        e0 = min_raw_d(e0, c1); e1 = max_raw_d(e1, c1);
        f0 = min_raw_d(f0, c2); f1 = max_raw_d(f1, c2);
      }
      a0 = wave_min_d(a0); a1 = wave_max_d(a1); b0 = wave_min_d(b0); b1 = wave_max_d(b1);
      e0 = wave_min_d(e0); e1 = wave_max_d(e1); f0 = wave_min_d(f0); f1 = wave_max_d(f1);
      FitAcc A, B;
      A.clear(); B.clear();
      for (int i = lane; i < m; i += 64) {
        const double x = mx[i], y = my[i];
        A.add(x, y, ct0, st0, a0, a1, b0, b1);
        B.add(x, y, ct1, st1, e0, e1, f0, f1);
      }
      A.wave_reduce(); B.wave_reduce();
      double magA, magB;
      const double cA = A.cost(magA), cB = B.cost(magB);
      if (lane == 0) { s_cost[th0] = cA; s_mag[th0] = magA; s_cost[th1] = cB; s_mag[th1] = magB; }
    }
    __syncthreads();
    double magmax = 0.0;
    for (int th = 0; th < n_theta; th++) { const double g = s_mag[th]; if (g > magmax) magmax = g; }
    const int best = wave_pick_heading(s_cost, n_theta, magmax, mx, my, m, s_ct, s_st);
    const double thb = (double)best * dtheta;
    const double sin_s = sin(thb), cos_s = cos(thb);
    {
      double a0 = INFINITY, a1 = -INFINITY, b0 = INFINITY, b1 = -INFINITY;
      for (int i = threadIdx.x; i < m; i += FT) {
        const double x = mx[i], y = my[i];
        const double c1 = x * cos_s + y * sin_s;
        const double c2 = x * (-sin_s) + y * cos_s;
        a0 = fmin(a0, c1); a1 = fmax(a1, c1);
        b0 = fmin(b0, c2); b1 = fmax(b1, c2);
      }
      a0 = wave_min_d(a0); a1 = wave_max_d(a1);
      b0 = wave_min_d(b0); b1 = wave_max_d(b1);
      if (lane == 0) { s_ext[wave][0] = a0; s_ext[wave][1] = a1; s_ext[wave][2] = b0; s_ext[wave][3] = b1; }
    }
    __syncthreads();
    if (threadIdx.x == 0) {
      double c1min = s_ext[0][0], c1max = s_ext[0][1], c2min = s_ext[0][2], c2max = s_ext[0][3];
      for (int w = 1; w < FW; w++) {
        c1min = fmin(c1min, s_ext[w][0]); c1max = fmax(c1max, s_ext[w][1]);
        c2min = fmin(c2min, s_ext[w][2]); c2max = fmax(c2max, s_ext[w][3]);
      }
      const int s = (int)d[0], kc = (int)d[1], root = (int)d[2];
      const int v = s / max_inst, jinst = s - v * max_inst;
      emit_box(thb, sin_s, cos_s, c1min, c1max, c2min, c2max, d[5], s, v, jinst, kc, root, m, calib,
               inst_class, inst_is_car, inst_box, inst_score, car_aspect_max, cap_rows, rows,
               n_rows, status);
    }
  }
}

constexpr int BIGC_T = 512, BIGC_WAVES = BIGC_T / 64, BIGC_HPW = 2, BIGC_HB = BIGC_WAVES * BIGC_HPW;
constexpr int BIGC_CH = 4096;
constexpr int BIGC_LONG = 16384, BIGC_MID = 6144;
__global__ __launch_bounds__(BIGC_T) void k_fit_big_cost(const double *__restrict__ gsx,
                                                         const double *__restrict__ gsy, int n_theta,
                                                         double dtheta, double *__restrict__ fit_ws,
                                                         int cap_rows, int cap_big) {
  __shared__ double lx[BIGC_CH], ly[BIGC_CH];
  __shared__ double s_ct[MAXTH], s_st[MAXTH];
  __shared__ int s_item;
  const FitWs W = fit_ws_view(fit_ws, cap_rows, cap_big);
  const int nbig = min(W.counters[1], cap_big);
  if (nbig == 0) return;
  if (threadIdx.x < MAXTH) {
    const double theta = (double)threadIdx.x * dtheta;
    s_ct[threadIdx.x] = cos(theta);
    s_st[threadIdx.x] = sin(theta);
  }
  const int wave = threadIdx.x >> 6, lane = lane_id();
  const int nb = (n_theta + BIGC_HB - 1) / BIGC_HB;
  const int items = nbig * nb;
  while (true) {
    __syncthreads();
    if (wave == 0) {
      const int ticket = atomicAdd(&W.counters[2], 1);
      if (lane == 0) s_item = ticket >> 6;
    }
    __syncthreads();
    const int ticket_item = s_item;
    if (ticket_item >= 3 * items) break;
    const int round = ticket_item / items;
    const int item = ticket_item - round * items;
    const int c = item / nb, tb = (item - c * nb) * BIGC_HB;
    const double *dsc = W.dsc + (size_t)8 * W.big_list[c];
    const int m = (int)dsc[3];
    if ((m > BIGC_LONG ? 0 : (m > BIGC_MID ? 1 : 2)) != round) continue;
    const double *mx = gsx + (long long)dsc[4], *my = gsy + (long long)dsc[4];
    int th[BIGC_HPW];
    double ct[BIGC_HPW], st[BIGC_HPW], nst[BIGC_HPW];
#pragma unroll
    for (int h = 0; h < BIGC_HPW; h++) {
      th[h] = tb + wave * BIGC_HPW + h;
      const int tc = min(th[h], n_theta - 1);
      ct[h] = s_ct[tc]; st[h] = s_st[tc]; nst[h] = -st[h];
    }
    double a0[BIGC_HPW], a1[BIGC_HPW], b0[BIGC_HPW], b1[BIGC_HPW];
#pragma unroll
    for (int h = 0; h < BIGC_HPW; h++) { a0[h] = INFINITY; a1[h] = -INFINITY; b0[h] = INFINITY; b1[h] = -INFINITY; }
    for (int c0 = 0; c0 < m; c0 += BIGC_CH) {
      const int cm = min(BIGC_CH, m - c0);
      __syncthreads();
      for (int i = threadIdx.x; i < cm; i += BIGC_T) { lx[i] = mx[c0 + i]; ly[i] = my[c0 + i]; }
      __syncthreads();
      for (int i = lane; i < cm; i += 64) {
        const double x = lx[i], y = ly[i];
#pragma unroll
        for (int h = 0; h < BIGC_HPW; h++) {
          const double c1 = x * ct[h] + y * st[h];
          const double c2 = x * nst[h] + y * ct[h];
          a0[h] = min_raw_d(a0[h], c1); a1[h] = max_raw_d(a1[h], c1);
          b0[h] = min_raw_d(b0[h], c2); b1[h] = max_raw_d(b1[h], c2);
        }
      }
    }
#pragma unroll
    for (int h = 0; h < BIGC_HPW; h++) {
      a0[h] = wave_min_d(a0[h]); a1[h] = wave_max_d(a1[h]);
      b0[h] = wave_min_d(b0[h]); b1[h] = wave_max_d(b1[h]);
    }
    FitAcc A[BIGC_HPW];
#pragma unroll
    for (int h = 0; h < BIGC_HPW; h++) A[h].clear();
    for (int c0 = 0; c0 < m; c0 += BIGC_CH) {
      const int cm = min(BIGC_CH, m - c0);
      __syncthreads();
      for (int i = threadIdx.x; i < cm; i += BIGC_T) { lx[i] = mx[c0 + i]; ly[i] = my[c0 + i]; }
      __syncthreads();
      for (int i = lane; i < cm; i += 64) {
        const double x = lx[i], y = ly[i];
#pragma unroll
        for (int h = 0; h < BIGC_HPW; h++) A[h].add(x, y, ct[h], st[h], a0[h], a1[h], b0[h], b1[h]);
      }
    }
#pragma unroll
    for (int h = 0; h < BIGC_HPW; h++) {
      A[h].wave_reduce();
      double mag;
      const double cst = A[h].cost(mag);
      if (lane == 0 && th[h] < n_theta) {
        W.big_cost[(size_t)c * MAXTH + th[h]] = cst;
        if (mag > 0.0) atomicMax((unsigned long long *)(W.dsc + (size_t)8 * W.big_list[c] + 7), (unsigned long long)__double_as_longlong(mag));
      }
    }
  }
}

__global__ __launch_bounds__(FT) void k_fit_big_box(
    const double *__restrict__ gsx, const double *__restrict__ gsy, int max_inst,
    const ViewCalib *__restrict__ calib, const int *__restrict__ inst_class,
    const int *__restrict__ inst_is_car, const float *__restrict__ inst_box,
    const float *__restrict__ inst_score, int n_theta, double dtheta, double car_aspect_max,
    int cap_rows, double *__restrict__ rows, int *__restrict__ n_rows,
    uint32_t *__restrict__ status, double *__restrict__ fit_ws, int cap_big) {
  __shared__ double s_ext[FW][4];
  __shared__ double s_ct[MAXTH], s_st[MAXTH];
  const FitWs W = fit_ws_view(fit_ws, cap_rows, cap_big);
  const int nbig = min(W.counters[1], cap_big);
  if (threadIdx.x < MAXTH) {
    const double theta = (double)threadIdx.x * dtheta;
    s_ct[threadIdx.x] = cos(theta);
    s_st[threadIdx.x] = sin(theta);
  }
  for (int c = blockIdx.x; c < nbig; c += gridDim.x) {
  __syncthreads();
  const double *dsc = W.dsc + (size_t)8 * W.big_list[c];
  const int s = (int)dsc[0], kc = (int)dsc[1], root = (int)dsc[2], m = (int)dsc[3];
  const double zmax = dsc[5];
  const double *mx = gsx + (long long)dsc[4], *my = gsy + (long long)dsc[4];
  const double *cost = W.big_cost + (size_t)c * MAXTH;
  const int wave = threadIdx.x >> 6, lane = lane_id();
  const int best = wave_pick_heading(cost, n_theta, dsc[7], mx, my, m, s_ct, s_st);
  const double thb = (double)best * dtheta;
  const double sin_s = sin(thb), cos_s = cos(thb);
  double a0 = INFINITY, a1 = -INFINITY, b0 = INFINITY, b1 = -INFINITY;
  for (int i = threadIdx.x; i < m; i += FT) {
    const double x = mx[i], y = my[i];
    const double c1 = x * cos_s + y * sin_s;
    const double c2 = x * (-sin_s) + y * cos_s;
    a0 = fmin(a0, c1); a1 = fmax(a1, c1);
    b0 = fmin(b0, c2); b1 = fmax(b1, c2);
  }
  a0 = wave_min_d(a0); a1 = wave_max_d(a1);
  b0 = wave_min_d(b0); b1 = wave_max_d(b1);
  if (lane == 0) { s_ext[wave][0] = a0; s_ext[wave][1] = a1; s_ext[wave][2] = b0; s_ext[wave][3] = b1; }
  __syncthreads();
  if (threadIdx.x == 0) {
    double c1min = s_ext[0][0], c1max = s_ext[0][1], c2min = s_ext[0][2], c2max = s_ext[0][3];
    for (int w = 1; w < FW; w++) {
      c1min = fmin(c1min, s_ext[w][0]); c1max = fmax(c1max, s_ext[w][1]);
      c2min = fmin(c2min, s_ext[w][2]); c2max = fmax(c2max, s_ext[w][3]);
    }
    const int v = s / max_inst, jinst = s - v * max_inst;
    emit_box(thb, sin_s, cos_s, c1min, c1max, c2min, c2max, zmax, s, v, jinst, kc, root, m, calib,
             inst_class, inst_is_car, inst_box, inst_score, car_aspect_max, cap_rows, rows, n_rows,
             status);
  }
  }
}

}

extern "C" int dfu3d_range_cluster(const double *px, const double *py, const int64_t *seg_base,
                                   const int32_t *seg_cnt, int32_t S, double R0, double Rd,
                                   int32_t *label, double *sx, double *sy, int32_t *si,
                                   int64_t pool_cap, void *stream) {
  DFU3D_CLEAR_STALE_ERROR();
  if (!px || !py || !seg_base || !seg_cnt || !label || !sx || !sy || !si) return DFU3D_EINVAL;
  if (S <= 0 || pool_cap <= 0 || !(R0 > 0.0) || !(Rd >= 0.0)) return DFU3D_EINVAL;
  hipLaunchKernelGGL((k_range_cluster_grid<GRID_NC_SMALL, 0, 1024>), dim3(CL_CLASSES * S), dim3(1024), 0,
                     (hipStream_t)stream, px, py, (const long long *)seg_base, seg_cnt, R0, Rd,
                     label, sx, sy, si, (long long)pool_cap, 0, 0x7FFFFFFF);
  DFU3D_LAUNCH_CHECK();
  hipLaunchKernelGGL((k_range_cluster_grid<GRID_NC_LARGE, GRID_NC_SMALL, 1024>), dim3(CL_CLASSES * S), dim3(1024), 0,
                     (hipStream_t)stream, px, py, (const long long *)seg_base, seg_cnt, R0, Rd,
                     label, sx, sy, si, (long long)pool_cap, 0, 0x7FFFFFFF);
  DFU3D_LAUNCH_CHECK();
  hipLaunchKernelGGL(k_range_cluster_small, dim3(S), dim3(CT), 0, (hipStream_t)stream, px, py,
                     (const long long *)seg_base, seg_cnt, R0, Rd, label, sx, sy, si,
                     (long long)pool_cap);
  DFU3D_LAUNCH_CHECK();
  hipLaunchKernelGGL(k_range_cluster_large, dim3(S), dim3(CT), 0, (hipStream_t)stream, px, py,
                     (const long long *)seg_base, seg_cnt, R0, Rd, label, sx, sy, si,
                     (long long)pool_cap);
  DFU3D_LAUNCH_CHECK();
  return DFU3D_OK;
}


extern "C" int64_t dfu3d_lshape_fit_ws_doubles(int64_t pool_cap, int32_t cap_rows) {
  if (pool_cap <= 0 || cap_rows <= 0) return DFU3D_EINVAL;
  const int64_t cap_big = pool_cap / LDS_MEMBERS + 1;
  return 2 + (int64_t)8 * fit_cap_q(cap_rows) + (cap_big / 2 + 1) + cap_big * MAXTH;
}

extern "C" int dfu3d_lshape_fit(const double *px, const double *py, const double *pz,
                                const int32_t *label, const int64_t *seg_base,
                                const int32_t *seg_cnt, int32_t S, int32_t max_inst,
                                const float *calib, const int32_t *inst_class,
                                const int32_t *inst_is_car, const float *inst_box,
                                const float *inst_score, int32_t n_theta, double dtheta,
                                double car_aspect_max, double *sx, double *sy, int32_t *sroot,
                                int32_t cap_rows, double *rows, int32_t *n_rows,
                                uint32_t *status, double *fit_ws, int64_t pool_cap,
                                void *stream) {
  DFU3D_CLEAR_STALE_ERROR();
  if (!px || !py || !pz || !label || !seg_base || !seg_cnt || !calib || !inst_class ||
      !inst_is_car || !inst_box || !inst_score || !sx || !sy || !sroot || !rows || !n_rows ||
      !status || !fit_ws)
    return DFU3D_EINVAL;
  if (S <= 0 || max_inst <= 0 || cap_rows <= 0 || n_theta <= 0 || pool_cap <= 0) return DFU3D_EINVAL;
  if (n_theta > MAXTH) return DFU3D_ERANGE;
  hipStream_t st = (hipStream_t)stream;
  const int cap_big = (int)(pool_cap / LDS_MEMBERS + 1);
  const ViewCalib *vc = (const ViewCalib *)calib;
  if (dfu3d_fill_small_async(fit_ws, 16, nullptr, 0, nullptr, 0, st) != hipSuccess) return DFU3D_ELAUNCH;
  hipLaunchKernelGGL(k_fit_gather, dim3(3 * S), dim3(FT), 0, st, px, py, pz, label,
                     (const long long *)seg_base, seg_cnt, sx, sy, sroot, status, fit_ws,
                     cap_rows, cap_big);
  DFU3D_LAUNCH_CHECK();
  const int cap_q = fit_cap_q(cap_rows);
  const int g_tiny = cap_q / 4 + 1 < 2048 ? cap_q / 4 + 1 : 2048;
  hipLaunchKernelGGL(k_fit_tiny, dim3(g_tiny), dim3(256), 0, st, sx, sy, max_inst, vc, inst_class,
                     inst_is_car, inst_box, inst_score, n_theta, dtheta, car_aspect_max, cap_rows,
                     rows, n_rows, status, fit_ws, cap_big);
  DFU3D_LAUNCH_CHECK();
  hipLaunchKernelGGL(k_fit_medium, dim3(cap_q < 2048 ? cap_q : 2048), dim3(FT), 0, st, sx, sy, max_inst,
                     vc, inst_class, inst_is_car, inst_box, inst_score, n_theta, dtheta,
                     car_aspect_max, cap_rows, rows, n_rows, status, fit_ws, cap_big);
  DFU3D_LAUNCH_CHECK();
  const long long bi = (long long)cap_big * ((n_theta + BIGC_HB - 1) / BIGC_HB);
  const int g2 = (int)(bi < 2048 ? bi : 2048);
  hipLaunchKernelGGL(k_fit_big_cost, dim3(g2), dim3(BIGC_T), 0, st, sx, sy, n_theta, dtheta,
                     fit_ws, cap_rows, cap_big);
  DFU3D_LAUNCH_CHECK();
  hipLaunchKernelGGL(k_fit_big_box, dim3(cap_big < 2048 ? cap_big : 2048), dim3(FT), 0, st, sx, sy, max_inst,
                     vc, inst_class, inst_is_car, inst_box, inst_score,
                     n_theta, dtheta, car_aspect_max, cap_rows, rows, n_rows, status, fit_ws,
                     cap_big);
  DFU3D_LAUNCH_CHECK();
  return DFU3D_OK;
}

extern "C" int dfu3d_version(void) { return DFU3D_VERSION; }

extern "C" const char *dfu3d_strerror(int code) {
  switch (code) {
    case DFU3D_OK: return "ok";
    case DFU3D_EINVAL: return "invalid argument";
    case DFU3D_ELAUNCH: return "kernel launch failed";
    case DFU3D_ERANGE: return "size exceeds a compiled-in limit";
    default: return "unknown error";
  }
}
```

dfu3d_amd/csrc/pixel_stage.hip:

```cpp
#include "common.hpp"
#include "dbg.hpp"

namespace {

constexpr int PB = 256;
constexpr int PPT = 4;
constexpr int PBLK = PB * PPT;
constexpr uint32_t NOBIN = 0xFFFFFFFFu;
constexpr uint32_t OVF_FLAG = 0x80000000u;

struct Table {
  unsigned long long *kmin, *combo;
  uint32_t *cnt, *first, *rep;
};
__host__ __device__ inline Table table_view(void *base, int64_t E) {
  Table t;
  t.kmin = (unsigned long long *)base;
  t.combo = t.kmin + E;
  t.cnt = (uint32_t *)(t.combo + E);
  t.first = t.cnt + E;
  t.rep = t.first + E;
  return t;
}
static_assert(DFU3D_TABLE_ENTRY_BYTES == 28, "table entry");

template <class T> __device__ __forceinline__ T &at32(T *p, uint32_t i) {
  return *(T *)((char *)p + i * (uint32_t)sizeof(T));
}

__device__ __forceinline__ unsigned long long combo_word(unsigned long long okey, uint32_t pix,
                                                         int pix_bits) {
  if (DBG_COMBO_KEYBITS < 64) okey &= ~0ull << (64 - DBG_COMBO_KEYBITS);
  return ((okey >> pix_bits) << pix_bits) | (unsigned long long)pix;
}

__global__ void k_table_init(unsigned long long *kmin, unsigned long long *combo, uint32_t *cnt,
                             uint32_t *first, uint32_t *rep, int64_t E) {
  for (int64_t i = (int64_t)blockIdx.x * blockDim.x + threadIdx.x; i < E;
       i += (int64_t)gridDim.x * blockDim.x) {
    kmin[i] = ~0ull;
    combo[i] = ~0ull;
    cnt[i] = 0u;
    first[i] = NOBIN;
    rep[i] = NOBIN;
  }
}

__device__ __forceinline__ uint32_t pixel_bin(const ViewCalib &c, const Recip &rc,
                                              const dfu3d_bin_geom &g,
                                              int W, int pix, float d, int key_axis,
                                              double &key, bool &range_err) {
  if (!(d >= (float)g.depth_min) || !(d > 0.0f)) return NOBIN;
  const int row = pix / W, col = pix - row * W;
  double x, y, z;
  pixel_to_lidar(c, rc, col, row, d, x, y, z);
  if (!(z < g.z_max)) return NOBIN;
  double s = x * x;
  s = s + y * y;
  s = s + z * z;
  const double r = sqrt(s);
  const double theta = acos(z / r);
  if (!(theta > g.theta_min)) return NOBIN;
  const double phi = atan(y / x);
  const double cr = floor((r - g.rmin_r) / g.vsize_r);
  const double ct = floor((theta - g.rmin_t) / g.vsize_t);
  const double cp = floor((phi - g.rmin_p) / g.vsize_p);
  if (!(cr >= 0.0 && cr < (double)g.grid_r)) return NOBIN;
  if (!(ct >= 0.0 && ct < (double)g.grid_t)) return NOBIN;
  if (!(cp >= 0.0 && cp < (double)g.grid_p)) return NOBIN;
  const int it = (int)ct - g.t_lo, ip = (int)cp - g.p_lo;
  if (it < 0 || it >= g.t_n || ip < 0 || ip >= g.p_n) { range_err = true; return NOBIN; }
  key = (key_axis == 2) ? z : y;
  key += 0.0;
  return (uint32_t)(it * g.p_n + ip);
}

__device__ __forceinline__ double pixel_key(const ViewCalib &c, const Recip &rc, int W, int pix, float d,
                                            int key_axis) {
  const int row = pix / W, col = pix - row * W;
  double x, y, z;
  pixel_to_lidar(c, rc, col, row, d, x, y, z);
  double key = (key_axis == 2) ? z : y;
  key += 0.0;
  return key;
}

__device__ __forceinline__ void load4(const float *p, uint32_t i, float d[PPT]) {
  const float4 q = *(const float4 *)&at32(p, i);
  d[0] = q.x; d[1] = q.y; d[2] = q.z; d[3] = q.w;
}

constexpr int TILE_W = 64, TILE_H = 16;
__device__ __forceinline__ void toggle_first_bit(uint32_t *bitmap_v, int W, int tiles_x, uint32_t pix) {
  const int row = (int)pix / W, col = (int)pix - row * W;
  const int tile = (row >> 4) * tiles_x + (col >> 6);
  const int local = (row & 15) * TILE_W + (col & 63);
  atomicXor(&at32(bitmap_v, (uint32_t)(tile * 32 + (local >> 5))), 1u << (local & 31));
}

constexpr int SEG_SHIFT = 6;
__device__ __forceinline__ void mark_segment(uint8_t *occ_v, uint32_t b) { occ_v[b >> SEG_SHIFT] = 1; }
__device__ __forceinline__ void commit_pixel(const Table &T, int64_t e, int pix, double key, int pix_bits,
                                             uint32_t *bitmap_v, int W, int tiles_x) {
  atomicAdd(&T.cnt[e], 1u);
  const uint32_t oldf = atomicMin(&T.first[e], (uint32_t)pix);
  atomicMin(&T.kmin[e], ordered_key(key));
  atomicMin(&T.combo[e], combo_word(ordered_key(key), (uint32_t)pix, pix_bits));
  if (oldf > (uint32_t)pix) {
    toggle_first_bit(bitmap_v, W, tiles_x, (uint32_t)pix);
    if (oldf != NOBIN) toggle_first_bit(bitmap_v, W, tiles_x, oldf);
  }
}

constexpr int TAB_T_MAX = 65534, TAB_P_MAX = 16382;
constexpr double TAB_SLOP_W = 1.0 / 16;
constexpr float TAB_DMAX = 1.0e-4f;
constexpr uint32_t AMBIG = 0xFFFFFFFEu;

struct FastGeom {
  float r_lo, r_hi, z_max, q_tmin;
  float tinv, tc1, pinv, pc1;
  float dmax, pad0;
  int tJ, pJ;
  double tq0d, twd, pq0d, pwd;
  double q_tmin_d;
  int mid_ok, pad1;
};
inline FastGeom make_fast_geom(const dfu3d_bin_geom &g) {
  const double pi = 3.14159265358979323846;
  FastGeom f;
  f.r_lo = (g.grid_r == 1) ? __builtin_fmaxf((float)(g.rmin_r + 2e-3), 1e-3f) : 1.0f;
  f.r_hi = (g.grid_r == 1) ? __builtin_fminf((float)((g.rmin_r + g.vsize_r) * 0.9998), 1e15f) : 0.0f;
  f.z_max = (float)g.z_max;
  f.q_tmin = g.theta_min <= 0.0 ? -INFINITY : (g.theta_min >= pi ? INFINITY : (float)-__builtin_cos(g.theta_min));
  f.q_tmin_d = g.theta_min <= 0.0 ? -(double)INFINITY : (g.theta_min >= pi ? (double)INFINITY : -__builtin_cos(g.theta_min));
  auto cells = [](double lo, double hi, double min_width, int cap, double &q0, double &w) {
    if (!(hi > lo) || !(min_width > 0.0)) { q0 = lo; w = 1.0; return 1; }
    double J = __builtin_ceil((hi - lo) / (0.5 * min_width));
    if (!(J >= 1.0)) J = 1.0;
    if (J > (double)cap) J = (double)cap;
    q0 = lo; w = (hi - lo) / J;
    return (int)J;
  };
  {
    const double a_lo = __builtin_fmax(g.rmin_t + (double)g.t_lo * g.vsize_t, 0.0100002);
    const double a_hi = __builtin_fmin(g.rmin_t + (double)(g.t_lo + g.t_n) * g.vsize_t, pi - 0.0100002);
    const double smin = __builtin_fmax(__builtin_fmin(__builtin_sin(a_lo), __builtin_sin(a_hi)), 0.2);
    f.tJ = cells(-__builtin_cos(a_lo), -__builtin_cos(a_hi), g.vsize_t * smin, TAB_T_MAX, f.tq0d, f.twd);
  }
  {
    const double b_lo = __builtin_fmax(g.rmin_p + (double)g.p_lo * g.vsize_p, -pi / 2);
    const double b_hi = __builtin_fmin(g.rmin_p + (double)(g.p_lo + g.p_n) * g.vsize_p, pi / 2);
    auto qphi = [](double P) { return __builtin_sin(P) / (__builtin_fabs(__builtin_cos(P)) + __builtin_fabs(__builtin_sin(P))); };
    f.pJ = cells(qphi(b_lo), qphi(b_hi), 0.5 * g.vsize_p, TAB_P_MAX, f.pq0d, f.pwd);
  }
  f.tinv = (float)(1.0 / f.twd); f.tc1 = (float)(1.0 - f.tq0d / f.twd);
  f.pinv = (float)(1.0 / f.pwd); f.pc1 = (float)(1.0 - f.pq0d / f.pwd);
  f.dmax = TAB_DMAX;
  const double slop_t = 1.8e-7 * ((1.0 + __builtin_fabs(f.tq0d)) / f.twd + 1.0), slop_p = 1.8e-7 * ((1.0 + __builtin_fabs(f.pq0d)) / f.pwd + 1.0);
  if (!(__builtin_fmax(slop_t, slop_p) <= TAB_SLOP_W)) f.dmax = 0.0f;
  if (g.t_n >= (1 << 16) || g.p_n >= (1 << 16)) f.dmax = 0.0f;
  f.mid_ok = (f.dmax > 0.0f) && ((int64_t)f.tJ + f.pJ + 4 + (int64_t)g.t_n + g.p_n + 2 <= 2 * (int64_t)(TAB_T_MAX + TAB_P_MAX));
  f.pad1 = 0;
  if (DBG_NO_MID) f.mid_ok = 0;
  f.pad0 = 0.0f;
  return f;
}

struct HotGeom {
  float depth_min, r_lo, r_hi, z_max, q_tmin;
  float tinv, tc1, pinv, pc1, dmax;
  int tJ, pJ, t_lo, t_n, p_lo, p_n, mid_ok;
};
inline HotGeom make_hot_geom(const dfu3d_bin_geom &g, const FastGeom &fg) {
  return HotGeom{(float)g.depth_min, fg.r_lo, fg.r_hi, fg.z_max, fg.q_tmin, fg.tinv, fg.tc1, fg.pinv, fg.pc1, fg.dmax,
                 fg.tJ, fg.pJ, g.t_lo, g.t_n, g.p_lo, g.p_n, fg.mid_ok};
}
struct BinCold {
  dfu3d_bin_geom g;
  FastGeom fg;
};
static_assert(sizeof(BinCold) % 16 == 0, "BinCold: the edge tables behind it stay 16-byte aligned");

__device__ __forceinline__ const double *edge_tab_t(const float2 *tab, const FastGeom &fg) { return (const double *)(tab + fg.tJ + fg.pJ + 4); }
__device__ __forceinline__ const double *edge_tab_p(const float2 *tab, const FastGeom &fg, const dfu3d_bin_geom &g) {
  return edge_tab_t(tab, fg) + g.t_n + 1;
}
inline int tables_threads(const FastGeom &fg, const dfu3d_bin_geom &g) {
  return fg.tJ + fg.pJ + 4 + (fg.mid_ok ? g.t_n + g.p_n + 2 : 0);
}
__global__ void k_bp_tables(dfu3d_bin_geom g, FastGeom fg, float2 *__restrict__ tab, BinCold *__restrict__ cold) {
  const int i = blockIdx.x * blockDim.x + threadIdx.x;
  const double pi = 3.14159265358979323846;
  if (i == 0 && cold) { cold->g = g; cold->fg = fg; }
  if (i >= fg.tJ + fg.pJ + 4) {
    const int e = i - (fg.tJ + fg.pJ + 4);
    if (!fg.mid_ok || e >= g.t_n + g.p_n + 2) return;
    double *et = (double *)(tab + fg.tJ + fg.pJ + 4);
    if (e <= g.t_n) {
      const double B = g.rmin_t + (double)(g.t_lo + e) * g.vsize_t;
      et[e] = B <= 0.0 ? -(double)INFINITY : (B >= pi ? (double)INFINITY : -cos(B));
    } else {
      const double B = g.rmin_p + (double)(g.p_lo + (e - g.t_n - 1)) * g.vsize_p;
      et[e] = B <= -pi / 2 ? -(double)INFINITY : (B >= pi / 2 ? (double)INFINITY : tan(B));
    }
    return;
  }
  const bool is_t = i < fg.tJ + 2;
  const int jj = is_t ? i : i - (fg.tJ + 2);
  const int J = is_t ? fg.tJ : fg.pJ;
  if (jj == 0 || jj == J + 1) { tab[i] = make_float2(__int_as_float(0x7FC00000), __int_as_float(0)); return; }
  const double w = is_t ? fg.twd : fg.pwd;
  const double c = (is_t ? fg.tq0d : fg.pq0d) + ((double)(jj - 1) + 0.5) * w;
  const double rmin = is_t ? g.rmin_t : g.rmin_p, vs = is_t ? g.vsize_t : g.vsize_p;
  auto edge = [&](long long k) -> double {
    const double B = rmin + (double)k * vs;
    if (is_t) return B <= 0.0 ? -INFINITY : (B >= pi ? INFINITY : -cos(B));
    return B <= -pi / 2 ? -INFINITY : (B >= pi / 2 ? INFINITY : sin(B) / (fabs(cos(B)) + fabs(sin(B))));
  };
  const double a = is_t ? acos(fmin(fmax(-c, -1.0), 1.0)) : (fabs(c) < 1.0 ? atan(c / (1.0 - fabs(c))) : copysign(pi / 2, c));
  double kf = floor((a - rmin) / vs);
  kf = fmin(fmax(kf, -1.0e9), 1.0e9);
  long long kn = (long long)kf;
  for (int r = 0; r < 8 && edge(kn) > c; r++) kn--;
  for (int r = 0; r < 8 && edge(kn + 1) <= c; r++) kn++;
  const double below = c - edge(kn), above = edge(kn + 1) - c;
  const bool up = above < below;
  const long long k1 = up ? kn + 1 : kn;
  const double others = fmin(up ? below : above, up ? edge(kn + 2) - c : c - edge(kn - 1));
  const bool ok = (edge(kn) <= c) && (c < edge(kn + 1)) && others >= (0.5 + TAB_SLOP_W) * w + 1.001 * (double)TAB_DMAX;
  tab[i] = ok ? make_float2((float)edge(k1), __int_as_float((int)k1)) : make_float2(__int_as_float(0x7FC00000), __int_as_float(0));
}

__device__ __forceinline__ bool tab_bin(const float2 *__restrict__ tab, float inv_w, float c1, int J, float q,
                                        float delta, uint32_t &k) {
  const uint32_t j = min((uint32_t)(int)__fmaf_rn(q, inv_w, c1), (uint32_t)(J + 1));
  const float2 e = *(const float2 *)((const char *)tab + (j << 3));
  const float t = q - e.x;
  k = (uint32_t)(__float_as_int(e.y) + (__float_as_int(t) >> 31));
  return fabsf(t) > delta;
}

struct FastCal {
  float a[3], b[3], c[3], e[3];
  float wsum, esum, pad0, pad1;
  double rfu, rfv;
};
static_assert(sizeof(FastCal) == 80, "FastCal");
__device__ __forceinline__ Recip recip_of(const FastCal &f) {
  Recip r;
  r.rfu = f.rfu; r.rfv = f.rfv;
  return r;
}

__global__ void k_bp_prep(const ViewCalib *__restrict__ calib, int V, int H, int W, FastCal *__restrict__ out) {
  const int v = blockIdx.x * blockDim.x + threadIdx.x;
  if (v >= V) return;
  const ViewCalib c = calib[v];
  FastCal f;
  double wsum = 0.0, esum = 0.0;
  for (int j = 0; j < 3; j++) {
    const double a = (double)c.Minv[0 + j] / (double)c.fu, b = (double)c.Minv[3 + j] / (double)c.fv;
    const double cc = (double)c.Minv[6 + j] - (double)c.cu * a - (double)c.cv * b;
    const double e = (double)c.tx * (double)c.Minv[0 + j] + (double)c.ty * (double)c.Minv[3 + j] + (double)c.Minv[9 + j];
    f.a[j] = (float)a; f.b[j] = (float)b; f.c[j] = (float)cc; f.e[j] = (float)e;
    wsum += fabs(a) * (double)(W > 1 ? W - 1 : 1) + fabs(b) * (double)(H > 1 ? H - 1 : 1) + fabs((double)c.Minv[6 + j]) +
            fabs((double)c.cu * a) + fabs((double)c.cv * b);
    esum += fabs((double)c.tx * (double)c.Minv[0 + j]) + fabs((double)c.ty * (double)c.Minv[3 + j]) + fabs((double)c.Minv[9 + j]);
  }
  f.wsum = (float)(wsum * 1.0000002);
  f.esum = (float)(esum * 1.0000002);
  f.pad0 = f.pad1 = 0.0f;
  const Recip r = make_recip(c);
  f.rfu = r.rfu; f.rfv = r.rfv;
  out[v] = f;
}

__device__ __forceinline__ void backproject_f32(const FastCal &fc, int col, int row, float d, float &xf, float &yf,
                                                float &zf, float &err) {
  const float u = (float)col, v = (float)row;
  const float w0 = __fmaf_rn(fc.a[0], u, __fmaf_rn(fc.b[0], v, fc.c[0]));
  const float w1 = __fmaf_rn(fc.a[1], u, __fmaf_rn(fc.b[1], v, fc.c[1]));
  const float w2 = __fmaf_rn(fc.a[2], u, __fmaf_rn(fc.b[2], v, fc.c[2]));
  xf = __fmaf_rn(d, w0, fc.e[0]);
  yf = __fmaf_rn(d, w1, fc.e[1]);
  zf = __fmaf_rn(d, w2, fc.e[2]);
  err = 2.3841858e-07f * (__fmaf_rn(fabsf(d), fc.wsum, fc.esum) + fabsf(xf) + fabsf(yf) + fabsf(zf));
}

template <int N>
__device__ __forceinline__ void classify_fast(const FastCal &fc, const HotGeom &fg,
                                              const float2 *__restrict__ tab, int row, const int (&col)[N],
                                              const float (&d)[N], uint32_t (&res)[N], int (&it)[N], int (&ip)[N]) {
  float xf[N], yf[N], zf[N], err[N];
  bool dead[N];
  bool any_live = false;
#pragma unroll
  for (int k = 0; k < N; k++) {
    backproject_f32(fc, col[k], row, d[k], xf[k], yf[k], zf[k], err[k]);
    const bool dok = (d[k] >= fg.depth_min) && (d[k] > 0.0f);
    dead[k] = !dok || (zf[k] > fg.z_max + err[k]);
    any_live = any_live || !dead[k];
    res[k] = NOBIN; it[k] = 0; ip[k] = 0;
  }
  if (!any_live) return;
#pragma unroll
  for (int k = 0; k < N; k++) {
    bool ok = zf[k] < fg.z_max - err[k];
    const float r2 = xf[k] * xf[k] + yf[k] * yf[k] + zf[k] * zf[k];
    const float ir = __builtin_amdgcn_rsqf(r2);
    const float rf = r2 * ir;
    const float er = 2.5f * err[k];
    const bool rin = (rf - er > fg.r_lo) & (rf + er < fg.r_hi);
    ok = ok & rin;
    const float cz = zf[k] * ir;
    const float s2 = __fmaf_rn(-cz, cz, 1.0f);
    ok = ok & (s2 > 1e-4f);
    const float turn = err[k] * ir * 1.7320510f;
    const float dq = 1.5e-6f + 1.05f * turn;
    const float qt = -cz;
    const bool th_out = rin & (qt < fg.q_tmin - dq);
    ok = ok & (qt > fg.q_tmin + dq);
    uint32_t kt, kp;
    ok = ok & tab_bin(tab, fg.tinv, fg.tc1, fg.tJ, qt, dq, kt);
    ok = ok & (fabsf(xf[k]) > __fmaf_rn(8.0f, err[k], 1e-20f));
    const float qa = yf[k] * __builtin_amdgcn_rcpf(fabsf(xf[k]) + fabsf(yf[k]));
    const float qp = xf[k] < 0.0f ? -qa : qa;
    const float dp = 1.5e-6f + 1.1f * turn * __builtin_amdgcn_rsqf(s2);
    ok = ok & tab_bin(tab + fg.tJ + 2, fg.pinv, fg.pc1, fg.pJ, qp, dp, kp);
    ok = ok & (dp < fg.dmax);
    const uint32_t itk = kt - (uint32_t)fg.t_lo, ipk = kp - (uint32_t)fg.p_lo;
    ok = ok & (itk < (uint32_t)fg.t_n) & (ipk < (uint32_t)fg.p_n);
    it[k] = (int)itk;
    ip[k] = (int)ipk;
    res[k] = (dead[k] | th_out) ? NOBIN : (ok ? __umul24(itk, (uint32_t)fg.p_n) + ipk : AMBIG);
  }
}

__device__ __forceinline__ uint32_t pixel_bin_fast(const ViewCalib &c, const Recip &rc, const FastCal &fc,
                                                   const HotGeom &hg, const float2 *__restrict__ tab,
                                                   int row, int col, float d, const KeyCol &kc, bool want_key,
                                                   double &key, int &it_out, int &ip_out) {
  const int cols[1] = {col};
  const float ds[1] = {d};
  uint32_t res[1];
  int it[1], ip[1];
  classify_fast<1>(fc, hg, tab, row, cols, ds, res, it, ip);
  it_out = it[0];
  ip_out = ip[0];
  if (want_key && res[0] < AMBIG) {
    key = pixel_to_lidar_axis(c, rc, kc, col, row, d);
    key += 0.0;
  }
  return res[0];
}

struct MidOut { uint32_t it, ip; double y, z; };
__device__ __forceinline__ uint32_t pixel_bin_mid(const ViewCalib &c, const Recip &rc, const dfu3d_bin_geom &g,
                                                  const FastGeom &fg, const float2 *__restrict__ tab, int W, int pix,
                                                  float d, bool &decided, MidOut *mo = nullptr) {
  const bool dok = (d >= (float)g.depth_min) && (d > 0.0f);
  const int row = pix / W, col = pix - row * W;
  double x, y, z;
  pixel_to_lidar(c, rc, col, row, d, x, y, z);
  double s = x * x;
  s = s + y * y;
  s = s + z * z;
  const double r = sqrt(s);
  const double qt = -(z / r);
  const double cr = floor((r - g.rmin_r) / g.vsize_r);
  const double t = y / x;
  const float tf = (float)t;
  const float qpf = tf * __builtin_amdgcn_rcpf(1.0f + fabsf(tf));
  const uint32_t jt = min((uint32_t)(int)__fmaf_rn((float)qt, fg.tinv, fg.tc1), (uint32_t)(fg.tJ + 1));
  const uint32_t jp = min((uint32_t)(int)__fmaf_rn(qpf, fg.pinv, fg.pc1), (uint32_t)(fg.pJ + 1));
  const float2 et = tab[jt];
  const float2 ep = tab[fg.tJ + 2 + jp];
  const uint32_t i_t = (uint32_t)(__float_as_int(et.y) - g.t_lo);
  const uint32_t i_p = (uint32_t)(__float_as_int(ep.y) - g.p_lo);
  const double e_t = edge_tab_t(tab, fg)[min(i_t, (uint32_t)g.t_n)];
  const double e_p = edge_tab_p(tab, fg, g)[min(i_p, (uint32_t)g.p_n)];
  const double dt = qt - e_t, dp = t - e_p;
  const uint32_t it = i_t - (dt < 0.0 ? 1u : 0u), ip = i_p - (dp < 0.0 ? 1u : 0u);
  decided = true;
  if (!dok) return NOBIN;
  if (!(z < g.z_max)) return NOBIN;
  if (qt < fg.q_tmin_d - 1e-12) return NOBIN;
  decided = qt > fg.q_tmin_d + 1e-12;
  if (decided && !(cr >= 0.0 && cr < (double)g.grid_r)) return NOBIN;
  decided = decided && (et.x == et.x) && (i_t <= (uint32_t)g.t_n) && (fabs(dt) > 1e-12);
  decided = decided && (ep.x == ep.x) && (i_p <= (uint32_t)g.p_n) && (fabs(dp) > 1e-12 * fma(t, t, 1.0));
  decided = decided && (it < (uint32_t)g.t_n) && (ip < (uint32_t)g.p_n);
  if (mo) { mo->it = it; mo->ip = ip; mo->y = y; mo->z = z; }
  return it * (uint32_t)g.p_n + ip;
}

constexpr int WIN_T = 16, WIN_P = 48;

constexpr int P1_AMB = 256;
constexpr int P1_OCC = 7;
constexpr int RPT = 2;
__global__ __launch_bounds__(PB, P1_OCC) void k_bp_bin(
    const float *__restrict__ depth, const ViewCalib *__restrict__ calib,
    const FastCal *__restrict__ fastcal, const float2 *__restrict__ tab, HotGeom hg, int W, int H, int tiles_x, int tiles_y, int key_axis,
    int64_t E_view, void *table, int64_t E_total, int *__restrict__ n_amb, uint32_t *__restrict__ amb_list,
    int pix_bits, uint32_t *__restrict__ bitmap, int BW, uint8_t *__restrict__ occ, int OW) {
  __shared__ uint32_t s_bits[32 * RPT];
  __shared__ uint32_t s_amb[P1_AMB];
  __shared__ unsigned long long s_kmin[WIN_T * WIN_P], s_combo[WIN_T * WIN_P];
  __shared__ uint32_t s_cnt[WIN_T * WIN_P], s_first[WIN_T * WIN_P];
  __shared__ int s_namb, s_t0, s_p0;
  DBG_T_START();
  DBG_T_COUNT(8);
  const int v = blockIdx.y;
  const int HW = H * W;
  const ViewCalib &c = calib[v];
  const FastCal fc = fastcal[v];
  const BinCold *cold = (const BinCold *)tab - 1;
  const Table T = table_view(table, E_total);
  const int64_t tb0 = (int64_t)v * E_view;
  uint32_t *const cnt_v = T.cnt + tb0, *const first_v = T.first + tb0;
  unsigned long long *const kmin_v = T.kmin + tb0, *const combo_v = T.combo + tb0;
  const float *const depth_v = depth + (size_t)v * HW;
  uint32_t *const amb_v = amb_list + (size_t)v * HW;
  const int ty = blockIdx.x / tiles_x, tx = blockIdx.x - ty * tiles_x;
  const int trow = (int)(((threadIdx.x >> 4) & 3u) * 4u + (threadIdx.x >> 6));
  const int row0 = ty * (RPT * TILE_H) + trow;
  const int col = tx * TILE_W + (threadIdx.x & 15) * PPT;
  if (threadIdx.x == 0) { s_namb = 0; s_t0 = 0x7FFFFFFF; s_p0 = 0x7FFFFFFF; }
  static_assert(32 * RPT == DFU3D_WAVE, "one bit-map word per lane of wave 0");
  const bool wave0 = __builtin_amdgcn_readfirstlane(threadIdx.x) < DFU3D_WAVE;
  if (wave0) s_bits[threadIdx.x] = 0u;
  uint32_t *bitmap_v = bitmap + (size_t)v * BW;
  uint8_t *occ_v = occ + (size_t)v * OW * 4;
  auto new_first = [&](uint32_t loc, uint32_t oldf) {
    atomicOr(&s_bits[loc >> 5], 1u << (loc & 31));
    if (oldf != NOBIN) toggle_first_bit(bitmap_v, W, tiles_x, oldf);
  };
  const uint32_t pix00 = (uint32_t)(ty * (RPT * TILE_H) * W + tx * TILE_W);
  auto global_pix = [&](uint32_t loc) { return pix00 + __umul24(loc >> 6, (uint32_t)W) + (loc & 63u); };
  static_assert(TILE_W == 64, "tile-local pixel index");
  static_assert(WIN_T * WIN_P % PB == 0, "window reset and flush: every thread takes the same number of slots");
#pragma unroll
  for (int j = 0; j < WIN_T * WIN_P / PB; j++) {
    const int i = threadIdx.x + j * PB;
    s_kmin[i] = ~0ull; s_combo[i] = ~0ull; s_cnt[i] = 0u; s_first[i] = NOBIN;
  }
  __syncthreads();
  DBG_T(0);
  uint32_t tp[RPT][PPT];
  bool inside[RPT];
  int tmin = 0x7FFFFFFF, pmin = 0x7FFFFFFF;
  uint32_t amb_mask = 0u;
#pragma unroll
  for (int r = 0; r < RPT; r++) {
    const int row = row0 + r * TILE_H;
    inside[r] = (row < H) && (col < W);
#pragma unroll
    for (int k = 0; k < PPT; k++) tp[r][k] = NOBIN;
    if (!inside[r]) continue;
    float d[PPT];
    load4(depth_v, __umul24((uint32_t)row, (uint32_t)W) + (uint32_t)col, d);
    int cols[PPT];
#pragma unroll
    for (int k = 0; k < PPT; k++) cols[k] = col + k;
    uint32_t res[PPT];
    int its[PPT], ips[PPT];
    classify_fast<PPT>(fc, hg, tab, row, cols, d, res, its, ips);
#pragma unroll
    for (int k = 0; k < PPT; k++) {
      const uint32_t b = res[k];
      if (b == AMBIG) {
        amb_mask |= 1u << (r * PPT + k);
      } else if (b != NOBIN) {
        tp[r][k] = (uint32_t)its[k] | ((uint32_t)ips[k] << 16);
        tmin = min(tmin, its[k]); pmin = min(pmin, ips[k]);
      }
    }
  }
  if (amb_mask) {
    int slot = atomicAdd(&s_namb, (int)__popc(amb_mask));
    while (amb_mask) {
      const int bit = __ffs((int)amb_mask) - 1;
      amb_mask &= amb_mask - 1u;
      const uint32_t pix = (uint32_t)((row0 + (bit / PPT) * TILE_H) * W + col + (bit % PPT));
      if (slot < P1_AMB) s_amb[slot] = pix;
      else at32(amb_v, (uint32_t)atomicAdd(&n_amb[v], 1)) = pix;
      slot++;
    }
  }
  DBG_T(1);
  tmin = wave_min_i_dpp(tmin);
  pmin = wave_min_i_dpp(pmin);
  if (lane_id() == 0 && tmin != 0x7FFFFFFF) { atomicMin(&s_t0, tmin); atomicMin(&s_p0, pmin); }
  __syncthreads();
  const int t0 = s_t0, p0 = s_p0;
  const KeyCal kcal = key_cal(c);
  const Recip rc = recip_of(fc);
  const KeyCol kcol = load_key_col(calib + v, key_axis);
  DBG_T(2);
#pragma unroll
  for (int r = 0; r < RPT; r++) {
    if (!inside[r]) continue;
    const uint32_t ro = __umul24((uint32_t)(row0 + r * TILE_H), (uint32_t)W);
    const uint32_t base = ro + (uint32_t)col;
    float dk[PPT];
    load4(depth_v, base, dk);
    const uint32_t loc0 = (uint32_t)((trow + r * TILE_H) * TILE_W + (threadIdx.x & 15) * PPT);
#pragma unroll
    for (int k = 0; k < PPT; k++) {
      if (tp[r][k] == NOBIN) continue;
      const uint32_t it_k = tp[r][k] & 0xFFFFu, ip_k = tp[r][k] >> 16;
      double key = pixel_to_lidar_axis(kcal, rc, kcol, col + k, row0 + r * TILE_H, dk[k]);
      key += 0.0;
      const unsigned long long ok = ordered_key(key);
      const unsigned long long cm = combo_word(ok, base + k, pix_bits);
      const uint32_t lt = it_k - (uint32_t)t0, lp = ip_k - (uint32_t)p0;
      if ((lt < (uint32_t)WIN_T) & (lp < (uint32_t)WIN_P)) {
        const uint32_t w = __umul24(lt, (uint32_t)WIN_P) + lp;
        atomicAdd(&s_cnt[w], 1u);
        atomicMin(&s_first[w], loc0 + k);
        atomicMin(&s_kmin[w], ok);
        atomicMin(&s_combo[w], cm);
      } else {
        const uint32_t b = __umul24(it_k, (uint32_t)hg.p_n) + ip_k;
        atomicAdd(&at32(cnt_v, b), 1u);
        const uint32_t oldf = atomicMin(&at32(first_v, b), base + k);
        atomicMin(&at32(kmin_v, b), ok);
        atomicMin(&at32(combo_v, b), cm);
        mark_segment(occ_v, b);
        if (oldf > base + k) new_first(loc0 + k, oldf);
      }
    }
  }
  {
    const int na_l = min(s_namb, P1_AMB);
    for (int i = threadIdx.x; i < na_l; i += PB) {
      const uint32_t pix = s_amb[i];
      bool decided = false;
      MidOut mo;
      uint32_t b = NOBIN;
      if (hg.mid_ok) b = pixel_bin_mid(c, rc, cold->g, cold->fg, tab, W, (int)pix, at32(depth_v, pix), decided, &mo);
      if (!decided) continue;
      s_amb[i] = NOBIN;
      if (b == NOBIN) continue;
      double key = (key_axis == 2) ? mo.z : mo.y;
      key += 0.0;
      const unsigned long long ok = ordered_key(key);
      const unsigned long long cm = combo_word(ok, pix, pix_bits);
      const int prow = (int)pix / W, pcol = (int)pix - prow * W;
      const uint32_t loc = (uint32_t)((prow - ty * (RPT * TILE_H)) * TILE_W + (pcol - tx * TILE_W));
      const uint32_t lt = mo.it - (uint32_t)t0, lp = mo.ip - (uint32_t)p0;
      if ((lt < (uint32_t)WIN_T) & (lp < (uint32_t)WIN_P)) {
        const uint32_t w = __umul24(lt, (uint32_t)WIN_P) + lp;
        atomicAdd(&s_cnt[w], 1u);
        atomicMin(&s_first[w], loc);
        atomicMin(&s_kmin[w], ok);
        atomicMin(&s_combo[w], cm);
      } else {
        atomicAdd(&at32(cnt_v, b), 1u);
        const uint32_t oldf = atomicMin(&at32(first_v, b), pix);
        atomicMin(&at32(kmin_v, b), ok);
        atomicMin(&at32(combo_v, b), cm);
        mark_segment(occ_v, b);
        if (oldf > pix) new_first(loc, oldf);
      }
    }
  }
  DBG_T(3);
  __syncthreads();
  DBG_T(4);
  constexpr int FL = WIN_T * WIN_P / PB;
  uint32_t f_loc[FL], f_new[FL], f_old[FL], f_seg[FL];
#pragma unroll
  for (int i = 0; i < FL; i++) {
    const int w = threadIdx.x + i * PB;
    f_loc[i] = 0u; f_new[i] = NOBIN; f_old[i] = 0u; f_seg[i] = NOBIN;
    const uint32_t cw = s_cnt[w];
    if (cw == 0u) continue;
    static_assert(WIN_T * WIN_P <= 768 && WIN_P == 48, "w / 48 as (w * 1366) >> 16 is exact below 768 * 48 / 18");
    const uint32_t wq = __umul24((uint32_t)w, 1366u) >> 16, wr = (uint32_t)w - __umul24(wq, (uint32_t)WIN_P);
    const uint32_t b = __umul24((uint32_t)t0 + wq, (uint32_t)hg.p_n) + ((uint32_t)p0 + wr);
    f_seg[i] = b >> SEG_SHIFT;
    f_loc[i] = s_first[w];
    f_new[i] = global_pix(f_loc[i]);
    atomicAdd(&at32(cnt_v, b), cw);
    f_old[i] = atomicMin(&at32(first_v, b), f_new[i]);
    atomicMin(&at32(kmin_v, b), s_kmin[w]);
    atomicMin(&at32(combo_v, b), s_combo[w]);
  }
#pragma unroll
  for (int i = 0; i < FL; i++)
    if (f_seg[i] != NOBIN) occ_v[f_seg[i]] = 1;
#pragma unroll
  for (int i = 0; i < FL; i++)
    if (f_old[i] > f_new[i]) new_first(f_loc[i], f_old[i]);
  DBG_T(5);
  __syncthreads();
  DBG_T(6);
  if (wave0 && s_bits[threadIdx.x]) {
    const int sub = threadIdx.x >> 5;
    if (ty * RPT + sub < tiles_y)
      atomicXor(&at32(bitmap_v, (uint32_t)(((ty * RPT + sub) * tiles_x + tx) * 32) + (threadIdx.x & 31)), s_bits[threadIdx.x]);
  }
  const int na = min(s_namb, P1_AMB);
  DBG_T(7);
  for (int i = threadIdx.x; i < na; i += PB)
    if (s_amb[i] != NOBIN) at32(amb_v, (uint32_t)atomicAdd(&n_amb[v], 1)) = s_amb[i];
}


__global__ __launch_bounds__(256) void k_bp_bin_amb(
    const float *__restrict__ depth, const ViewCalib *__restrict__ calib, dfu3d_bin_geom g, int W,
    int HW, int key_axis, int64_t E_view, void *table, int64_t E_total, const int *__restrict__ n_amb,
    const uint32_t *__restrict__ amb_list, uint32_t *__restrict__ status, int pix_bits,
    uint32_t *__restrict__ bitmap, int BW, int tiles_x, uint8_t *__restrict__ occ, int OW) {
  const int v = blockIdx.y;
  const int na = n_amb[v];
  const ViewCalib c = calib[v];
  const Recip rc = make_recip(c);
  const Table T = table_view(table, E_total);
  const int64_t tb0 = (int64_t)v * E_view;
  bool rerr = false;
  for (int e = blockIdx.x * 256 + threadIdx.x; e < na; e += gridDim.x * 256) {
    const int pix = (int)amb_list[(size_t)v * HW + e];
    double key;
    const uint32_t b = pixel_bin(c, rc, g, W, pix, depth[(size_t)v * HW + pix], key_axis, key, rerr);
    if (b != NOBIN) {
      commit_pixel(T, tb0 + b, pix, key, pix_bits, bitmap + (size_t)v * BW, W, tiles_x);
      mark_segment(occ + (size_t)v * OW * 4, b);
    }
  }
  if (rerr) atomicOr(status, DFU3D_ST_BIN_RANGE);
}

constexpr int SCB = 1024;
__device__ __forceinline__ unsigned long long row_piece(const uint32_t *bitmap_v, int tiles_x, int y, int tx) {
  return *(const unsigned long long *)(bitmap_v + ((size_t)(y >> 4) * tiles_x + tx) * 32 + (y & 15) * 2);
}
__global__ __launch_bounds__(SCB) void k_bp_scan(int BW, int NJ, int tiles_x, const uint32_t *__restrict__ bitmap,
                                                 uint32_t *__restrict__ wpre, int *__restrict__ n_vox, int cap_vox,
                                                 uint32_t *__restrict__ status, const uint32_t *__restrict__ occ, int OW,
                                                 int NSEG, int *__restrict__ seg_list, int *__restrict__ n_occ) {
  __shared__ int s_w[SCB / 64];
  const int v = blockIdx.x;
  {
    const uint32_t *ov = occ + (size_t)v * OW;
    int run = 0;
    for (int w0 = 0; w0 < OW; w0 += SCB) {
      const int w = w0 + threadIdx.x;
      const uint32_t word = (w < OW) ? ov[w] : 0u;
      int tot;
      int at = run + block_excl_scan<SCB / 64>(__popc(word & 0x01010101u), s_w, tot);
#pragma unroll
      for (int q = 0; q < 4; q++)
        if ((word >> (8 * q)) & 1u) seg_list[(size_t)v * NSEG + at++] = w * 4 + q;
      run += tot;
    }
    if (threadIdx.x == 0) n_occ[v] = run;
  }
  const uint32_t *bv = bitmap + (size_t)v * BW;
  int running = 0;
  for (int j0 = 0; j0 < NJ; j0 += SCB) {
    const int j = j0 + threadIdx.x;
    int c = 0;
    if (j < NJ) {
      const int y = j / tiles_x, tx = j - y * tiles_x;
      c = __popcll(row_piece(bv, tiles_x, y, tx));
    }
    int tot;
    const int ex = block_excl_scan<SCB / 64>(c, s_w, tot);
    if (j < NJ) wpre[(size_t)v * NJ + j] = (uint32_t)(running + ex);
    running += tot;
  }
  if (threadIdx.x == 0) {
    n_vox[v] = running;
    if (running > cap_vox) atomicOr(status, DFU3D_ST_VOX_OVERFLOW);
  }
}

struct VoxOut {
  uint32_t *vox_pix, *it_bits;
  double *it_x, *it_y, *it_z;
};

__device__ __forceinline__ void emit_voxel(const VoxOut &o, size_t at, const ViewCalib &c, const Recip &rc,
                                           const float *depth_v, int W, uint32_t pix, const void *masks,
                                           int mask_format, int m, int max_inst, int HW, int v) {
  const int row = (int)pix / W, col = (int)pix - row * W;
  double x, y, z;
  pixel_to_lidar(c, rc, col, row, depth_v[pix], x, y, z);
  o.vox_pix[at] = pix;
  o.it_bits[at] = masks ? mask_bits_at(masks, mask_format, v, max_inst, m, HW, (int)pix) : 0u;
  o.it_x[at] = x;
  o.it_y[at] = y;
  o.it_z[at] = z;
}

constexpr int VXB = 256;
constexpr int VOX_GX = 512;
struct VoxWalk {
  const int *seg_list, *n_occ;
  const uint32_t *bitmap, *wpre;
  int NSEG, BW, NJ, tiles_x;
};
__global__ __launch_bounds__(VXB) void k_bp_vox(
    const float *__restrict__ depth, const ViewCalib *__restrict__ calib, const void *__restrict__ masks, int mask_format,
    const int *__restrict__ n_inst, int max_inst, int W, int HW, int64_t E_view, void *table, int64_t E_total, int cap_vox,
    VoxWalk Wk, VoxOut out, int key_axis, int pix_bits, int max_points, int max_voxels, int cap_q,
    uint32_t *__restrict__ q_bins, int *__restrict__ q_rank, int *__restrict__ n_q, uint32_t *__restrict__ status, int V) {
  const unsigned lin = blockIdx.y * gridDim.x + blockIdx.x, turn = lin >> 3;
  const int v = (int)((turn / gridDim.x) * 8u + (lin & 7u)), bx = (int)(turn % gridDim.x);
  if (v >= V) return;
  const int n_occ = Wk.n_occ[v];
  const int lane = lane_id();
  const int wave = __builtin_amdgcn_readfirstlane((int)(bx * (VXB / 64) + (threadIdx.x >> 6)));
  if (wave >= n_occ) return;
  const ViewCalib c = calib[v];
  const Recip rc = make_recip(c);
  const Table T = table_view(table, E_total);
  const int64_t tb0 = (int64_t)v * E_view;
  const float *dv = depth + (size_t)v * HW;
  const uint32_t *bv = Wk.bitmap + (size_t)v * Wk.BW;
  const int m_inst = masks ? min(max(n_inst[v], 0), max_inst) : 0;
  const unsigned long long pix_mask = (1ull << pix_bits) - 1ull;
  for (int i = wave; i < n_occ; i += gridDim.x * (VXB / 64)) {
    const int sg = Wk.seg_list[(size_t)v * Wk.NSEG + i];
    const int64_t b = ((int64_t)sg << SEG_SHIFT) + lane;
    const bool in = b < E_view;
    const int64_t e = tb0 + (in ? b : 0);
    const uint32_t cw = in ? T.cnt[e] : 0u;
    const uint32_t f = T.first[e];
    const unsigned long long e_kmin = T.kmin[e], e_combo = T.combo[e];
    const bool vox = cw != 0u && cw < OVF_FLAG;
    if (__ballot(vox) == 0ull) continue;
    int k = 0;
    uint32_t pix = 0u, m_bits = 0u;
    float d_pix = 0.0f;
    if (vox) {
      const int fr = (int)f / W, fc = (int)f - fr * W;
      const unsigned long long word = row_piece(bv, Wk.tiles_x, fr, fc >> 6);
      const uint32_t pre = Wk.wpre[(size_t)v * Wk.NJ + (size_t)fr * Wk.tiles_x + (fc >> 6)];
      pix = (uint32_t)(e_combo & pix_mask);
      d_pix = dv[pix];
      m_bits = masks ? mask_bits_at(masks, mask_format, v, max_inst, m_inst, HW, (int)pix) : 0u;
      k = (int)pre + __popcll(word & ((1ull << (fc & 63)) - 1ull));
    }
    bool keep = !in || cw >= OVF_FLAG || (vox && k >= cap_vox);
    if (vox && !keep) {
      const int row = (int)pix / W, col = (int)pix - row * W;
      double x, yy, z;
      pixel_to_lidar(c, rc, col, row, d_pix, x, yy, z);
      double key = (key_axis == 2) ? z : yy;
      key += 0.0;
      if (cw > (uint32_t)max_points || ordered_key(key) != e_kmin) {
        const int slot = atomicAdd(&n_q[v], 1);
        if (slot < cap_q) { q_bins[(size_t)v * cap_q + slot] = (uint32_t)b; q_rank[(size_t)v * cap_q + slot] = k; }
        else atomicOr(status, DFU3D_ST_VOX_PTS_OVERFLOW);
        keep = true;
      } else if (k < max_voxels) {
        const size_t at = (size_t)v * cap_vox + k;
        out.vox_pix[at] = pix;
        out.it_bits[at] = m_bits;
        out.it_x[at] = x;
        out.it_y[at] = yy;
        out.it_z[at] = z;
      }
    }
    if (!keep) {
      T.kmin[e] = ~0ull;
      T.combo[e] = ~0ull;
      T.cnt[e] = 0u;
      T.first[e] = NOBIN;
    }
  }
}

__global__ __launch_bounds__(PB) void k_bp_rebin(
    const float *__restrict__ depth, const ViewCalib *__restrict__ calib, dfu3d_bin_geom g, int W, int HW,
    int key_axis, const int *__restrict__ n_q, uint32_t *__restrict__ pix_bin) {
  const int v = blockIdx.y;
  if (n_q[v] == 0) return;
  const ViewCalib c = calib[v];
  const Recip rc = make_recip(c);
  bool rerr = false;
  for (int pix = blockIdx.x * PB + threadIdx.x; pix < HW; pix += gridDim.x * PB) {
    double key;
    pix_bin[(size_t)v * HW + pix] = pixel_bin(c, rc, g, W, pix, depth[(size_t)v * HW + pix], key_axis, key, rerr);
  }
}

__global__ void k_ovf_alloc(void *table, int64_t E_total, int64_t E_view, int cap_q,
                            const uint32_t *__restrict__ q_bins,
                            const int *__restrict__ n_q, int *__restrict__ q_cnt,
                            int *__restrict__ q_cursor, int HW,
                            uint32_t *__restrict__ status) {
  const int v = blockIdx.y;
  const int no = min(n_q[v], cap_q);
  const Table T = table_view(table, E_total);
  for (int s = blockIdx.x * blockDim.x + threadIdx.x; s < no; s += gridDim.x * blockDim.x) {
    const int64_t e = (int64_t)v * E_view + q_bins[(size_t)v * cap_q + s];
    const int c = (int)T.cnt[e];
    const int off = atomicAdd(&q_cursor[v], c);
    if (off + c > HW) atomicOr(status, DFU3D_ST_VOX_PTS_OVERFLOW);
    q_cnt[(size_t)v * cap_q + s] = c;
    T.rep[e] = (uint32_t)off;
    T.cnt[e] = OVF_FLAG;
  }
}

__global__ __launch_bounds__(PB) void k_ovf_gather(
    const uint32_t *__restrict__ pix_bin, void *table, int64_t E_total, int64_t E_view,
    int HW, const int *__restrict__ n_q, uint32_t *__restrict__ q_list) {
  const int v = blockIdx.y;
  if (n_q[v] == 0) return;
  const Table T = table_view(table, E_total);
  for (int base = blockIdx.x * PBLK + threadIdx.x * PPT; base < HW; base += gridDim.x * PBLK) {
    for (int k = 0; k < PPT; k++) {
      const int pix = base + k;
      if (pix >= HW) break;
      const uint32_t b = pix_bin[(size_t)v * HW + pix];
      if (b == NOBIN) continue;
      const int64_t e = (int64_t)v * E_view + b;
      if (T.cnt[e] & OVF_FLAG) {
        const uint32_t pos = atomicAdd(&T.cnt[e], 1u) & ~OVF_FLAG;
        q_list[(size_t)v * HW + T.rep[e] + pos] = (uint32_t)pix;
      }
    }
  }
}

__global__ __launch_bounds__(256) void k_ovf_select(
    const float *__restrict__ depth, const ViewCalib *__restrict__ calib, int W, int HW,
    int key_axis, int max_points, void *table, int64_t E_total, int64_t E_view,
    int cap_ovf, const uint32_t *__restrict__ ovf_bins, const int *__restrict__ n_ovf,
    const int *__restrict__ ovf_cnt, const uint32_t *__restrict__ ovf_list) {
  __shared__ int hist[256];
  __shared__ uint32_t s_sel[2];
  __shared__ unsigned long long s_min[4];
  const int v = blockIdx.y;
  const int no = min(n_ovf[v], cap_ovf);
  const Table T = table_view(table, E_total);
  const ViewCalib c = calib[v];
  const Recip rc = make_recip(c);
  for (int s = blockIdx.x; s < no; s += gridDim.x) {
  const int64_t e = (int64_t)v * E_view + ovf_bins[(size_t)v * cap_ovf + s];
  const int n = ovf_cnt[(size_t)v * cap_ovf + s];
  const uint32_t *lst = ovf_list + (size_t)v * HW + T.rep[e];
  __syncthreads();
  uint32_t prefix = 0u, mask = 0u;
  int kk = max_points - 1;
  for (int shift = 16; shift >= 0; shift -= 8) {
    hist[threadIdx.x] = 0;
    __syncthreads();
    for (int i = threadIdx.x; i < n; i += 256) {
      const uint32_t key = lst[i];
      if ((key & mask) == prefix) atomicAdd(&hist[(key >> shift) & 0xFFu], 1);
    }
    __syncthreads();
    if (threadIdx.x == 0) {
      int acc = 0, b = 0;
      for (; b < 256; b++) {
        const int c = hist[b];
        if (acc + c > kk) break;
        acc += c;
      }
      if (b > 255) b = 255;
      s_sel[0] = prefix | ((uint32_t)b << shift);
      s_sel[1] = (uint32_t)(kk - acc);
    }
    __syncthreads();
    prefix = s_sel[0];
    kk = (int)s_sel[1];
    mask |= (0xFFu << shift);
    __syncthreads();
  }
  const uint32_t thr = prefix;
  unsigned long long m = ~0ull;
  for (int i = threadIdx.x; i < n; i += 256) {
    const uint32_t pix = lst[i];
    if (pix <= thr) {
      const unsigned long long k = ordered_key(
          pixel_key(c, rc, W, (int)pix, depth[(size_t)v * HW + pix], key_axis));
      m = k < m ? k : m;
    }
  }
#pragma unroll
  for (int x = 32; x >= 1; x >>= 1) {
    const unsigned long long o = __shfl_xor(m, x, 64);
    m = o < m ? o : m;
  }
  if (lane_id() == 0) s_min[threadIdx.x >> 6] = m;
  __syncthreads();
  for (int w = 0; w < 4; w++) m = s_min[w] < m ? s_min[w] : m;
  uint32_t rp = NOBIN;
  for (int i = threadIdx.x; i < n; i += 256) {
    const uint32_t pix = lst[i];
    if (pix <= thr && pix < rp) {
      const unsigned long long k = ordered_key(
          pixel_key(c, rc, W, (int)pix, depth[(size_t)v * HW + pix], key_axis));
      if (k == m) rp = pix;
    }
  }
#pragma unroll
  for (int x = 32; x >= 1; x >>= 1) rp = min(rp, (uint32_t)__shfl_xor((int)rp, x, 64));
  __syncthreads();
  if (lane_id() == 0) s_min[threadIdx.x >> 6] = (unsigned long long)rp;
  __syncthreads();
  if (threadIdx.x == 0) {
    for (int w = 0; w < 4; w++) rp = min(rp, (uint32_t)s_min[w]);
    T.kmin[e] = m;
    T.cnt[e] = OVF_FLAG | thr;
    T.rep[e] = rp;
  }
  }
}

__global__ __launch_bounds__(256) void k_bp_fix(
    const float *__restrict__ depth, const ViewCalib *__restrict__ calib,
    const void *__restrict__ masks, int mask_format, const int *__restrict__ n_inst, int max_inst, int W,
    int HW, int max_voxels, int64_t E_view, void *table, int64_t E_total, int cap_vox, VoxOut out, int cap_q,
    const uint32_t *__restrict__ q_bins, const int *__restrict__ q_rank, const int *__restrict__ n_q) {
  const int v = blockIdx.y;
  const int no = min(n_q[v], cap_q);
  if (blockIdx.x * 256 >= no) return;
  const Table T = table_view(table, E_total);
  const ViewCalib c = calib[v];
  const Recip rc = make_recip(c);
  const int m = masks ? min(max(n_inst[v], 0), max_inst) : 0;
  for (int s = blockIdx.x * 256 + threadIdx.x; s < no; s += gridDim.x * 256) {
    const int64_t e = (int64_t)v * E_view + q_bins[(size_t)v * cap_q + s];
    const int k = q_rank[(size_t)v * cap_q + s];
    if (k < max_voxels)
      emit_voxel(out, (size_t)v * cap_vox + k, c, rc, depth + (size_t)v * HW, W, T.rep[e], masks, mask_format, m,
                 max_inst, HW, v);
    T.kmin[e] = ~0ull;
    T.combo[e] = ~0ull;
    T.cnt[e] = 0u;
    T.first[e] = NOBIN;
    T.rep[e] = NOBIN;
  }
}

__global__ void k_bp_finalize(int V, int max_voxels, int cap_vox, int *__restrict__ n_vox) {
  const int v = blockIdx.x * blockDim.x + threadIdx.x;
  if (v >= V) return;
  n_vox[v] = min(min(n_vox[v], cap_vox), max_voxels);
}

__global__ void k_selftest_classify(const ViewCalib *__restrict__ calib, const FastCal *__restrict__ fastcal,
                                    const float2 *__restrict__ tab, dfu3d_bin_geom g, FastGeom fg, HotGeom hg, int H,
                                    int W, int key_axis, long long n, unsigned long long seed, double d_lo, double d_hi,
                                    unsigned long long *out) {
  const ViewCalib c = calib[0];
  const FastCal fc = fastcal[0];
  const Recip rc = make_recip(c);
  const KeyCol kcol = load_key_col(calib, key_axis);
  unsigned long long tried = 0, undecided = 0, wrong = 0, kept = 0;
  for (long long i = (long long)blockIdx.x * blockDim.x + threadIdx.x; i < n;
       i += (long long)gridDim.x * blockDim.x) {
    const unsigned long long a = mix64(seed + 3ull * (unsigned long long)i),
                             b = mix64(seed + 3ull * (unsigned long long)i + 1ull),
                             e = mix64(seed + 3ull * (unsigned long long)i + 2ull);
    const int col = (int)(a % (unsigned long long)W), row = (int)(b % (unsigned long long)H);
    const double ud = (double)(e >> 11) * (1.0 / 9007199254740992.0);
    const float d = (float)((d_lo + (d_hi - d_lo) * ud) * ((i & 3) == 0 ? 0.02 : 1.0));
    double k1 = 0.0, k2 = 0.0;
    int it_, ip_;
    bool rerr = false;
    const uint32_t b1 = pixel_bin_fast(c, rc, fc, hg, tab, row, col, d, kcol, true, k1, it_, ip_);
    const uint32_t b2 = pixel_bin(c, rc, g, W, row * W + col, d, key_axis, k2, rerr);
    tried++;
    if (b1 == AMBIG) {
      undecided++;
      if (fg.mid_ok) {
        bool dec = false;
        const uint32_t b3 = pixel_bin_mid(c, rc, g, fg, tab, W, row * W + col, d, dec);
        if (dec && b3 != b2) wrong++;
      }
      continue;
    }
    if (b1 != b2 || (b1 != NOBIN && __double_as_longlong(k1) != __double_as_longlong(k2))) wrong++;
    if (b1 != NOBIN) kept++;
  }
  tried = wave_sum_u64(tried); undecided = wave_sum_u64(undecided);
  wrong = wave_sum_u64(wrong); kept = wave_sum_u64(kept);
  if (lane_id() == 0) {
    atomicAdd(&out[0], tried); atomicAdd(&out[1], undecided); atomicAdd(&out[2], wrong); atomicAdd(&out[3], kept);
  }
}

__global__ void k_selftest_backproject(const ViewCalib *__restrict__ calib, const FastCal *__restrict__ fastcal,
                                       int H, int W, long long n, unsigned long long seed, double d_lo,
                                       double d_hi, unsigned long long *out) {
  const ViewCalib c = calib[0];
  const FastCal fc = fastcal[0];
  const Recip rc = make_recip(c);
  double worst = 0.0;
  for (long long i = (long long)blockIdx.x * blockDim.x + threadIdx.x; i < n;
       i += (long long)gridDim.x * blockDim.x) {
    const unsigned long long a = mix64(seed + 3ull * (unsigned long long)i),
                             b = mix64(seed + 3ull * (unsigned long long)i + 1ull),
                             e = mix64(seed + 3ull * (unsigned long long)i + 2ull);
    const int col = (int)(a % (unsigned long long)W), row = (int)(b % (unsigned long long)H);
    const double ud = (double)(e >> 11) * (1.0 / 9007199254740992.0);
    const float d = (float)((d_lo + (d_hi - d_lo) * ud) * ((i & 3) == 0 ? 0.02 : 1.0));
    if (!(d > 0.0f)) continue;
    double x, y, z;
    pixel_to_lidar(c, rc, col, row, d, x, y, z);
    float xf, yf, zf, err;
    backproject_f32(fc, col, row, d, xf, yf, zf, err);
    const double m = fmax(fmax(fabs((double)xf - x), fabs((double)yf - y)), fabs((double)zf - z));
    worst = fmax(worst, m / (double)err);
  }
  worst = wave_max_d(worst);
  if (lane_id() == 0) atomicMax(&out[0], (unsigned long long)__double_as_longlong(worst));
}

}

DBG_T_READER(dfu3d_debug_timing_pixel)

extern "C" int dfu3d_selftest_classify(const float *calib, int32_t H, int32_t W, const dfu3d_bin_geom *geom,
                                       int32_t key_axis, int64_t n, uint64_t seed, double d_lo, double d_hi,
                                       void *scratch, uint64_t *out4, void *stream) {
  DFU3D_CLEAR_STALE_ERROR();
  if (!calib || !geom || !scratch || !out4 || n <= 0 || H <= 0 || W <= 0 || !(d_hi > d_lo) || !(d_lo >= 0.0))
    return DFU3D_EINVAL;
  if (key_axis != 1 && key_axis != 2) return DFU3D_EINVAL;
  if ((uintptr_t)scratch & 15u) return DFU3D_EINVAL;
  hipStream_t st = (hipStream_t)stream;
  const FastGeom fg = make_fast_geom(*geom);
  FastCal *fastcal = (FastCal *)scratch;
  float2 *tab = (float2 *)((char *)scratch + 128);
  if (hipMemsetAsync(out4, 0, 32, st) != hipSuccess) return DFU3D_ELAUNCH;
  hipLaunchKernelGGL(k_bp_prep, dim3(1), dim3(64), 0, st, (const ViewCalib *)calib, 1, H, W, fastcal);
  DFU3D_LAUNCH_CHECK();
  hipLaunchKernelGGL(k_bp_tables, dim3((tables_threads(fg, *geom) + 255) / 256), dim3(256), 0, st, *geom, fg, tab,
                     (BinCold *)nullptr);
  DFU3D_LAUNCH_CHECK();
  hipLaunchKernelGGL(k_selftest_classify, dim3(2048), dim3(256), 0, st, (const ViewCalib *)calib, fastcal, tab,
                     *geom, fg, make_hot_geom(*geom, fg), H, W, key_axis, (long long)n, (unsigned long long)seed, d_lo, d_hi,
                     (unsigned long long *)out4);
  DFU3D_LAUNCH_CHECK();
  return DFU3D_OK;
}

extern "C" int dfu3d_selftest_backproject(const float *calib, int32_t H, int32_t W, int64_t n, uint64_t seed,
                                          double d_lo, double d_hi, void *scratch64, double *out1, void *stream) {
  DFU3D_CLEAR_STALE_ERROR();
  if (!calib || !scratch64 || !out1 || n <= 0 || H <= 0 || W <= 0 || !(d_hi > d_lo) || !(d_lo >= 0.0)) return DFU3D_EINVAL;
  hipStream_t st = (hipStream_t)stream;
  if (hipMemsetAsync(out1, 0, 8, st) != hipSuccess) return DFU3D_ELAUNCH;
  hipLaunchKernelGGL(k_bp_prep, dim3(1), dim3(64), 0, st, (const ViewCalib *)calib, 1, H, W, (FastCal *)scratch64);
  DFU3D_LAUNCH_CHECK();
  hipLaunchKernelGGL(k_selftest_backproject, dim3(2048), dim3(256), 0, st, (const ViewCalib *)calib,
                     (const FastCal *)scratch64, H, W, (long long)n, (unsigned long long)seed, d_lo, d_hi,
                     (unsigned long long *)out1);
  DFU3D_LAUNCH_CHECK();
  return DFU3D_OK;
}

extern "C" int64_t dfu3d_bin_table_geometry(dfu3d_bin_geom *g) {
  if (!g) return DFU3D_EINVAL;
  const double pi = 3.14159265358979323846;
  auto binf = [](double v, double mn, double vs) { return (int64_t)__builtin_floor((v - mn) / vs); };
  int64_t t0 = binf(g->theta_min, g->rmin_t, g->vsize_t) - 1;
  int64_t t1 = binf(pi, g->rmin_t, g->vsize_t) + 2;
  int64_t p0 = binf(-pi / 2, g->rmin_p, g->vsize_p) - 1;
  int64_t p1 = binf(pi / 2, g->rmin_p, g->vsize_p) + 2;
  if (t0 < 0) t0 = 0;
  if (p0 < 0) p0 = 0;
  if (t1 > g->grid_t) t1 = g->grid_t;
  if (p1 > g->grid_p) p1 = g->grid_p;
  if (t1 <= t0 || p1 <= p0) return DFU3D_EINVAL;
  g->t_lo = (int32_t)t0;
  g->t_n = (int32_t)(t1 - t0);
  g->p_lo = (int32_t)p0;
  g->p_n = (int32_t)(p1 - p0);
  return (int64_t)g->t_n * g->p_n;
}

extern "C" int dfu3d_bin_table_init(void *table, int64_t E, void *stream) {
  DFU3D_CLEAR_STALE_ERROR();
  if (!table || E <= 0) return DFU3D_EINVAL;
  const Table T = table_view(table, E);
  hipLaunchKernelGGL(k_table_init, dim3(2048), dim3(256), 0, (hipStream_t)stream, T.kmin,
                     T.combo, T.cnt, T.first, T.rep, E);
  DFU3D_LAUNCH_CHECK();
  return DFU3D_OK;
}

static inline int queue_cap(int64_t HW, int max_points, int cap_vox) {
  if (DBG_COMBO_KEYBITS < 64) return cap_vox;
  const int64_t q = HW / (max_points + 1) + 1 + 4096;
  return (int)(q < cap_vox ? q : cap_vox);
}

static inline int64_t table_segments(int64_t E_view) { return (E_view + 63) >> SEG_SHIFT; }

extern "C" int64_t dfu3d_backproject_scratch_words(int32_t V, int32_t H, int32_t W,
                                                    int32_t cap_vox, int32_t max_points, int64_t table_entries,
                                                    int64_t *pix_words, int64_t *blk_words) {
  if (V <= 0 || H <= 0 || W <= 0 || cap_vox <= 0 || max_points < 1 || table_entries <= 0) return DFU3D_EINVAL;
  const int64_t HW = (int64_t)H * W;
  const int64_t tiles_x = (W + TILE_W - 1) / TILE_W, tiles_y = (H + TILE_H - 1) / TILE_H;
  const int64_t BW = tiles_x * tiles_y * 32, NJ = (int64_t)H * tiles_x;
  const int64_t cap_q = queue_cap(HW, max_points, cap_vox);
  if (pix_words) *pix_words = 2 * V * HW;
  const int64_t NSEG = table_segments(table_entries), OW = (NSEG + 3) / 4;
  if (blk_words) *blk_words = 4 * (int64_t)V + V * BW + V * OW + V * NJ + V * NSEG + 3 * V * cap_q + 20 * (int64_t)V + (int64_t)(sizeof(BinCold) / 4) + 16 +
                              4 * (int64_t)(TAB_T_MAX + TAB_P_MAX) + 16;
  return 0;
}

extern "C" int dfu3d_backproject_bin(
    const float *depth, const float *calib, const void *masks, int32_t mask_format, const int32_t *n_inst,
    int32_t V, int32_t max_inst, int32_t H, int32_t W, const dfu3d_bin_geom *geom,
    int32_t key_axis, void *table, uint32_t *pix_bin, int32_t *blk_cnt, int32_t cap_vox,
    int32_t *n_vox, uint32_t *vox_pix, uint32_t *it_bits, double *it_x, double *it_y,
    double *it_z, uint32_t *status, int32_t phases, void *stream) {
  DFU3D_CLEAR_STALE_ERROR();
  if (!depth || !calib || !geom || !table || !pix_bin || !blk_cnt || !n_vox || !vox_pix ||
      !it_bits || !it_x || !it_y || !it_z || !status)
    return DFU3D_EINVAL;
  if (masks && !n_inst) return DFU3D_EINVAL;
  if (V <= 0 || H <= 0 || W <= 0 || cap_vox <= 0) return DFU3D_EINVAL;
  if (key_axis != 1 && key_axis != 2) return DFU3D_EINVAL;
  if (max_inst > DFU3D_MAX_INST) return DFU3D_ERANGE;
  if (masks && !mask_format_ok(mask_format, max_inst)) return DFU3D_EINVAL;
  const int64_t HW64 = (int64_t)H * W;
  if (HW64 >= (1ll << 24)) return DFU3D_ERANGE;
  if (W % 4) return DFU3D_EINVAL;
  if (geom->max_points_per_voxel < 1) return DFU3D_EINVAL;
  if (((uintptr_t)blk_cnt & 7u) != 0) return DFU3D_EINVAL;
  const int HW = (int)HW64;
  const int tiles_x = (W + TILE_W - 1) / TILE_W, tiles_y = (H + TILE_H - 1) / TILE_H;
  const int BW = tiles_x * tiles_y * 32, NJ = H * tiles_x;
  const int cap_q = queue_cap(HW64, geom->max_points_per_voxel, cap_vox);
  const int64_t E_view = (int64_t)geom->t_n * geom->p_n;
  if (E_view >= (1ll << 29)) return DFU3D_ERANGE;
  const int64_t E_total = E_view * V;
  hipStream_t st = (hipStream_t)stream;
  const int NSEG = (int)table_segments(E_view), OW = (NSEG + 3) / 4;
  int *n_amb = blk_cnt;
  int *n_q = n_amb + V;
  int *q_cursor = n_q + V;
  int *n_occ = q_cursor + V;
  uint32_t *bitmap = (uint32_t *)(n_occ + V);
  uint32_t *occ = bitmap + (size_t)V * BW;
  uint32_t *wpre = occ + (size_t)V * OW;
  int *seg_list = (int *)(wpre + (size_t)V * NJ);
  int *q_cnt = seg_list + (size_t)V * NSEG;
  uint32_t *q_bins = (uint32_t *)(q_cnt + (size_t)V * cap_q);
  int *q_rank = (int *)(q_bins + (size_t)V * cap_q);
  FastCal *fastcal = (FastCal *)(((uintptr_t)(q_rank + (size_t)V * cap_q) + 15) & ~(uintptr_t)15);
  BinCold *cold = (BinCold *)(fastcal + V);
  const float2 *tab = (const float2 *)(cold + 1);
  const FastGeom fg = make_fast_geom(*geom);
  int pix_bits = 1;
  while ((1ll << pix_bits) < HW64) pix_bits++;
  uint32_t *q_list = pix_bin + (size_t)V * HW;
  const ViewCalib *cal = (const ViewCalib *)calib;
  const VoxOut out = {vox_pix, it_bits, it_x, it_y, it_z};
  const VoxWalk Wk = {seg_list, n_occ, bitmap, wpre, NSEG, BW, NJ, tiles_x};

  if (phases & DFU3D_BP_BIN) {
    if (dfu3d_fill_async(blk_cnt, 0, sizeof(int) * (4 * (size_t)V + (size_t)V * BW + (size_t)V * OW), st) != hipSuccess) return DFU3D_ELAUNCH;
    hipLaunchKernelGGL(k_bp_prep, dim3((V + 63) / 64), dim3(64), 0, st, cal, V, H, W, fastcal);
    DFU3D_LAUNCH_CHECK();
    hipLaunchKernelGGL(k_bp_tables, dim3((tables_threads(fg, *geom) + 255) / 256), dim3(256), 0, st, *geom, fg, (float2 *)tab, cold);
    DFU3D_LAUNCH_CHECK();
    hipLaunchKernelGGL(k_bp_bin, dim3(tiles_x * ((tiles_y + RPT - 1) / RPT), V), dim3(PB), 0, st, depth, cal, fastcal, tab,
                       make_hot_geom(*geom, fg), W, H, tiles_x, tiles_y, key_axis, E_view, table, E_total, n_amb, q_list, pix_bits,
                       bitmap, BW, (uint8_t *)occ, OW);
    DFU3D_LAUNCH_CHECK();
  }
  if (phases & DFU3D_BP_AMB) {
    hipLaunchKernelGGL(k_bp_bin_amb, dim3(64, V), dim3(256), 0, st, depth, cal, *geom, W, HW,
                       key_axis, E_view, table, E_total, n_amb, q_list, status, pix_bits, bitmap, BW, tiles_x, (uint8_t *)occ, OW);
    DFU3D_LAUNCH_CHECK();
  }
  if (phases & DFU3D_BP_MARK) {
    hipLaunchKernelGGL(k_bp_scan, dim3(V), dim3(SCB), 0, st, BW, NJ, tiles_x, bitmap, wpre, n_vox, cap_vox, status, occ, OW,
                       NSEG, seg_list, n_occ);
    DFU3D_LAUNCH_CHECK();
  }
  if (phases & DFU3D_BP_VOX) {
    const int gx = std::min((NSEG + (VXB / 64) - 1) / (VXB / 64), VOX_GX);
    hipLaunchKernelGGL(k_bp_vox, dim3(gx, (V + 7) / 8 * 8), dim3(VXB), 0, st, depth, cal, masks, mask_format, n_inst, max_inst, W, HW, E_view,
                       table, E_total, cap_vox, Wk, out, key_axis, pix_bits, geom->max_points_per_voxel, geom->max_voxels,
                       cap_q, q_bins, q_rank, n_q, status, V);
    DFU3D_LAUNCH_CHECK();
  }
  if (phases & DFU3D_BP_REPAIR) {
    const int nblk = (HW + PB - 1) / PB;
    hipLaunchKernelGGL(k_bp_rebin, dim3(nblk < 16 ? nblk : 16, V), dim3(PB), 0, st, depth, cal, *geom, W, HW,
                       key_axis, n_q, pix_bin);
    DFU3D_LAUNCH_CHECK();
    const int ga = (cap_q + 255) / 256;
    hipLaunchKernelGGL(k_ovf_alloc, dim3(ga < 16 ? ga : 16, V), dim3(256), 0, st, table, E_total, E_view, cap_q,
                       q_bins, n_q, q_cnt, q_cursor, HW, status);
    DFU3D_LAUNCH_CHECK();
    const int nblk4 = (HW + PBLK - 1) / PBLK;
    hipLaunchKernelGGL(k_ovf_gather, dim3(nblk4 < 16 ? nblk4 : 16, V), dim3(PB), 0, st, pix_bin, table, E_total,
                       E_view, HW, n_q, q_list);
    DFU3D_LAUNCH_CHECK();
    hipLaunchKernelGGL(k_ovf_select, dim3(cap_q < 32 ? cap_q : 32, V), dim3(256), 0, st, depth, cal, W, HW,
                       key_axis, geom->max_points_per_voxel, table, E_total, E_view, cap_q,
                       q_bins, n_q, q_cnt, q_list);
    DFU3D_LAUNCH_CHECK();
    hipLaunchKernelGGL(k_bp_fix, dim3(ga < 16 ? ga : 16, V), dim3(256), 0, st, depth, cal, masks, mask_format, n_inst,
                       max_inst, W, HW, geom->max_voxels, E_view, table, E_total, cap_vox, out, cap_q, q_bins, q_rank,
                       n_q);
    DFU3D_LAUNCH_CHECK();
    hipLaunchKernelGGL(k_bp_finalize, dim3((V + 255) / 256), dim3(256), 0, st, V, geom->max_voxels, cap_vox, n_vox);
    DFU3D_LAUNCH_CHECK();
  }
  return DFU3D_OK;
}
```

Baseline: 10200 frames/s.

## Merge back-projection chain launches and cache bin tables across calls

In the dense chain path, the workspace clear and the small output resets become one fill kernel. Calibration prep and bin-table build become one kernel, which skips rebuilding the tables when the cached geometry matches. The repair phase's several launches become a single per-view kernel, and the small and large range-cluster kernels merge into one. A lean mode also skips writing voxel coordinates for points with no mask bits. The aim is fewer kernel launches and less redundant table work per call, at the cost of extra state (the table cache and a done counter) and possibly less parallelism in the one-block-per-view repair kernel.

```diff
diff --git a/dfu3d_amd/_build.py b/dfu3d_amd/_build.py
--- a/dfu3d_amd/_build.py
+++ b/dfu3d_amd/_build.py
@@ -67,6 +67,7 @@
     "keybits14": ["-DDFU3D_DBG_COMBO_KEYBITS=14"],
     "no_mid": ["-DDFU3D_DBG_NO_MID"],
     "timing": ["-DDFU3D_DBG_TIMING"],
+    "count": ["-DDFU3D_DBG_COUNT_LAUNCHES"],
     "asan_host": ["-O1", "-g", "-Xarch_host", "-fsanitize=address", "-Xarch_host", "-fsanitize=undefined",
                   "-Xarch_host", "-fno-sanitize-recover=undefined", "-Xarch_host", "-fno-omit-frame-pointer", "-shared-libsan"],
 }
diff --git a/dfu3d_amd/csrc/chain_stage.hip b/dfu3d_amd/csrc/chain_stage.hip
--- a/dfu3d_amd/csrc/chain_stage.hip
+++ b/dfu3d_amd/csrc/chain_stage.hip
@@ -166,6 +166,9 @@
   if (cfg->dense) {
     const int rc = dfu3d_bin_table_init(w.table, (int64_t)cfg->V * w.table_entries, stream);
     if (rc) return rc;
+    const int rt = dfu3d_bp_tables_forget(w.blk_cnt, cfg->V, cfg->H, cfg->W, cfg->cap_vox, cfg->geom.max_points_per_voxel,
+                                          w.table_entries, stream);
+    if (rt) return rt;
   }
   hipLaunchKernelGGL(k_fill_i32, dim3((cfg->V * cfg->max_inst + 255) / 256), dim3(256), 0,
                      (hipStream_t)stream, cfg->V * cfg->max_inst, 1, w.stat_enable);
@@ -197,8 +200,12 @@
   carve(cfg, (char *)workspace, &w);
   hipStream_t st = (hipStream_t)stream;
   const int V = cfg->V, M = cfg->max_inst, S = V * M, cap_n = cfg->cap_n;
-  if (dfu3d_fill_small_async(n_rows, sizeof(int32_t), status, sizeof(uint32_t), w.pool_cursor, sizeof(int64_t), st) != hipSuccess)
+  if (cfg->dense) {
+    CHAIN_TRY(dfu3d_bp_clear_chain(w.blk_cnt, V, cfg->H, cfg->W, w.table_entries, n_rows, sizeof(int32_t), status,
+                                   sizeof(uint32_t), w.pool_cursor, sizeof(int64_t), stream));
+  } else if (dfu3d_fill_small_async(n_rows, sizeof(int32_t), status, sizeof(uint32_t), w.pool_cursor, sizeof(int64_t), st) != hipSuccess) {
     return DFU3D_ELAUNCH;
+  }
   if (cfg->apply_fov) {
     CHAIN_TRY(dfu3d_fov_filter(points, pt_off, view_frame, calib, V, cfg->fov_h, cfg->fov_w, cap_n,
                                w.fov_idx, w.n_fov, stream));
@@ -219,9 +226,9 @@
                                 cap_n, cfg->plane_offset, cfg->plane_range, w.ag_pt,
                                 w.ib_pix, w.n_ag, w.K, w.a_bits, w.a_x, w.a_y, w.a_z, stream));
   if (cfg->dense) {
-    CHAIN_TRY(dfu3d_backproject_bin(depth, calib, masks, cfg->mask_format, n_inst, V, M, cfg->H, cfg->W, &cfg->geom, 1, w.table,
-                                    w.pix_bin, w.blk_cnt, cfg->cap_vox, w.n_vox, w.vox_pix, w.b_bits, w.b_x,
-                                    w.b_y, w.b_z, status, DFU3D_BP_ALL, stream));
+    CHAIN_TRY(dfu3d_backproject_bin_chain(depth, calib, masks, cfg->mask_format, n_inst, V, M, cfg->H, cfg->W, &cfg->geom, 1,
+                                          w.table, w.pix_bin, w.blk_cnt, cfg->cap_vox, w.n_vox, w.vox_pix, w.b_bits, w.b_x,
+                                          w.b_y, w.b_z, status, stream));
   } else {
     if (dfu3d_fill_async(w.n_vox, 0, sizeof(int32_t) * V, st) != hipSuccess) return DFU3D_ELAUNCH;
   }
@@ -262,3 +269,12 @@
                              stream));
   return DFU3D_OK;
 }
+
+#ifdef DFU3D_DBG_COUNT_LAUNCHES
+long long g_dbg_launches = 0;
+extern "C" long long dfu3d_debug_launch_count(int reset) {
+  const long long n = g_dbg_launches;
+  if (reset) g_dbg_launches = 0;
+  return n;
+}
+#endif
diff --git a/dfu3d_amd/csrc/common.hpp b/dfu3d_amd/csrc/common.hpp
--- a/dfu3d_amd/csrc/common.hpp
+++ b/dfu3d_amd/csrc/common.hpp
@@ -2,7 +2,10 @@
 #include <hip/hip_runtime.h>
 #include <stdint.h>
 
+#include <stddef.h>
+#include <string.h>
 #include "dfu3d.h"
+#include "dbg.hpp"
 
 #define DFU3D_WAVE 64
 
@@ -299,3 +302,14 @@
                      (uint32_t *)c, (int)(bytes_c / 4), 0u);
   return hipGetLastError();
 }
+
+int dfu3d_backproject_bin_chain(
+    const float *depth, const float *calib, const void *masks, int32_t mask_format, const int32_t *n_inst,
+    int32_t V, int32_t max_inst, int32_t H, int32_t W, const dfu3d_bin_geom *geom,
+    int32_t key_axis, void *table, uint32_t *pix_bin, int32_t *blk_cnt, int32_t cap_vox,
+    int32_t *n_vox, uint32_t *vox_pix, uint32_t *it_bits, double *it_x, double *it_y,
+    double *it_z, uint32_t *status, void *stream);
+int dfu3d_bp_clear_chain(int32_t *blk_cnt, int32_t V, int32_t H, int32_t W, int64_t table_entries, void *a, size_t bytes_a,
+                         void *b, size_t bytes_b, void *c, size_t bytes_c, void *stream);
+int dfu3d_bp_tables_forget(int32_t *blk_cnt, int32_t V, int32_t H, int32_t W, int32_t cap_vox, int32_t max_points,
+                           int64_t table_entries, void *stream);
diff --git a/dfu3d_amd/csrc/dbg.hpp b/dfu3d_amd/csrc/dbg.hpp
--- a/dfu3d_amd/csrc/dbg.hpp
+++ b/dfu3d_amd/csrc/dbg.hpp
@@ -38,3 +38,9 @@
 #define DBG_T_MAX(k, v) do {} while (0)
 #define DBG_T_READER(name)
 #endif
+
+#ifdef DFU3D_DBG_COUNT_LAUNCHES
+extern long long g_dbg_launches;
+#undef hipLaunchKernelGGL
+#define hipLaunchKernelGGL(kernelName, ...) do { ++g_dbg_launches; hipLaunchKernelGGLInternal((kernelName), __VA_ARGS__); } while (0)
+#endif
diff --git a/dfu3d_amd/csrc/fit_stage.hip b/dfu3d_amd/csrc/fit_stage.hip
--- a/dfu3d_amd/csrc/fit_stage.hip
+++ b/dfu3d_amd/csrc/fit_stage.hip
@@ -679,30 +679,7 @@
   }
 }
 
-__global__ __launch_bounds__(CT) void k_range_cluster_small(
-    const double *__restrict__ px, const double *__restrict__ py,
-    const long long *__restrict__ seg_base, const int *__restrict__ seg_cnt, double R0,
-    double Rd, int *__restrict__ label, double *__restrict__ sx, double *__restrict__ sy,
-    int *__restrict__ si, long long pool_cap) {
-  __shared__ __attribute__((aligned(16))) int s_parent[SMALL_N];
-  __shared__ int s_summ[SMALL_N / GRP];
-  __shared__ float4 s_box[SMALL_N / GRP];
-  __shared__ int s_summ2[SMALL_N / GRP / BLK];
-  __shared__ float4 s_box2[SMALL_N / GRP / BLK];
-  __shared__ double s_red[4 * (CT / 64)];
-  __shared__ int s_w[CT / 64];
-  const int s = blockIdx.x;
-  const int n = seg_cnt[s];
-  if (n == 0 || n > SMALL_N) return;
-  const long long base = seg_base[s];
-  if (si[2 * pool_cap + base]) return;
-  cell_sort<SMALL_N>(px + base, py + base, n, s_parent, s_red, s_w, sx + base, sy + base, si + base);
-  ParI par{s_parent, false};
-  cluster_body<ParI, SMALL_N / GRP>(par, s_summ, s_box, s_summ2, s_box2, s_red, sx + base, sy + base,
-                                    n, R0, Rd, si + base, si + pool_cap + base, label + base);
-}
-
-__global__ __launch_bounds__(CT) void k_range_cluster_large(
+__global__ __launch_bounds__(CT) void k_range_cluster_fallback(
     const double *__restrict__ px, const double *__restrict__ py,
     const long long *__restrict__ seg_base, const int *__restrict__ seg_cnt, double R0,
     double Rd, int *__restrict__ label, double *__restrict__ sx, double *__restrict__ sy,
@@ -714,11 +691,19 @@
   __shared__ float4 s_box2[LARGE_GRP / BLK];
   __shared__ double s_red[4 * (CT / 64)];
   __shared__ int s_w[CT / 64];
+  static_assert(sizeof(int) * SMALL_N <= sizeof(unsigned short) * LARGE_N && SMALL_N / GRP <= LARGE_GRP, "the small form fits");
   const int s = blockIdx.x;
   const int n = seg_cnt[s];
-  if (n <= SMALL_N) return;
+  if (n == 0) return;
   const long long base = seg_base[s];
   if (si[2 * pool_cap + base]) return;
+  if (n <= SMALL_N) {
+    cell_sort<SMALL_N>(px + base, py + base, n, (int *)s_parent, s_red, s_w, sx + base, sy + base, si + base);
+    ParI par{(int *)s_parent, false};
+    cluster_body<ParI, SMALL_N / GRP>(par, s_summ, s_box, s_summ2, s_box2, s_red, sx + base, sy + base,
+                                      n, R0, Rd, si + base, si + pool_cap + base, label + base);
+    return;
+  }
   cell_sort<LARGE_N / 2>(px + base, py + base, n, (int *)s_parent, s_red, s_w, sx + base, sy + base,
                          si + base);
   if (n <= LARGE_N) {
@@ -1521,11 +1506,7 @@
                      (hipStream_t)stream, px, py, (const long long *)seg_base, seg_cnt, R0, Rd,
                      label, sx, sy, si, (long long)pool_cap, 0, 0x7FFFFFFF);
   DFU3D_LAUNCH_CHECK();
-  hipLaunchKernelGGL(k_range_cluster_small, dim3(S), dim3(CT), 0, (hipStream_t)stream, px, py,
-                     (const long long *)seg_base, seg_cnt, R0, Rd, label, sx, sy, si,
-                     (long long)pool_cap);
-  DFU3D_LAUNCH_CHECK();
-  hipLaunchKernelGGL(k_range_cluster_large, dim3(S), dim3(CT), 0, (hipStream_t)stream, px, py,
+  hipLaunchKernelGGL(k_range_cluster_fallback, dim3(S), dim3(CT), 0, (hipStream_t)stream, px, py,
                      (const long long *)seg_base, seg_cnt, R0, Rd, label, sx, sy, si,
                      (long long)pool_cap);
   DFU3D_LAUNCH_CHECK();
diff --git a/dfu3d_amd/csrc/pixel_stage.hip b/dfu3d_amd/csrc/pixel_stage.hip
--- a/dfu3d_amd/csrc/pixel_stage.hip
+++ b/dfu3d_amd/csrc/pixel_stage.hip
@@ -189,10 +189,8 @@
 inline int tables_threads(const FastGeom &fg, const dfu3d_bin_geom &g) {
   return fg.tJ + fg.pJ + 4 + (fg.mid_ok ? g.t_n + g.p_n + 2 : 0);
 }
-__global__ void k_bp_tables(dfu3d_bin_geom g, FastGeom fg, float2 *__restrict__ tab, BinCold *__restrict__ cold) {
-  const int i = blockIdx.x * blockDim.x + threadIdx.x;
+__device__ __forceinline__ void tables_entry(int i, const dfu3d_bin_geom &g, const FastGeom &fg, float2 *__restrict__ tab) {
   const double pi = 3.14159265358979323846;
-  if (i == 0 && cold) { cold->g = g; cold->fg = fg; }
   if (i >= fg.tJ + fg.pJ + 4) {
     const int e = i - (fg.tJ + fg.pJ + 4);
     if (!fg.mid_ok || e >= g.t_n + g.p_n + 2) return;
@@ -231,6 +229,11 @@
   const bool ok = (edge(kn) <= c) && (c < edge(kn + 1)) && others >= (0.5 + TAB_SLOP_W) * w + 1.001 * (double)TAB_DMAX;
   tab[i] = ok ? make_float2((float)edge(k1), __int_as_float((int)k1)) : make_float2(__int_as_float(0x7FC00000), __int_as_float(0));
 }
+__global__ void k_bp_tables(dfu3d_bin_geom g, FastGeom fg, float2 *__restrict__ tab, BinCold *__restrict__ cold) {
+  const int i = blockIdx.x * blockDim.x + threadIdx.x;
+  if (i == 0 && cold) { cold->g = g; cold->fg = fg; }
+  tables_entry(i, g, fg, tab);
+}
 
 __device__ __forceinline__ bool tab_bin(const float2 *__restrict__ tab, float inv_w, float c1, int J, float q,
                                         float delta, uint32_t &k) {
@@ -253,8 +256,7 @@
   return r;
 }
 
-__global__ void k_bp_prep(const ViewCalib *__restrict__ calib, int V, int H, int W, FastCal *__restrict__ out) {
-  const int v = blockIdx.x * blockDim.x + threadIdx.x;
+__device__ __forceinline__ void prep_view(int v, const ViewCalib *__restrict__ calib, int V, int H, int W, FastCal *__restrict__ out) {
   if (v >= V) return;
   const ViewCalib c = calib[v];
   FastCal f;
@@ -274,6 +276,53 @@
   const Recip r = make_recip(c);
   f.rfu = r.rfu; f.rfv = r.rfv;
   out[v] = f;
+}
+__global__ void k_bp_prep(const ViewCalib *__restrict__ calib, int V, int H, int W, FastCal *__restrict__ out) {
+  prep_view(blockIdx.x * blockDim.x + threadIdx.x, calib, V, H, W, out);
+}
+
+constexpr int PTB = 256;
+__global__ __launch_bounds__(PTB) void k_bp_prep_tables(const ViewCalib *__restrict__ calib, int V, int H, int W,
+                                                        FastCal *__restrict__ out, int prep_blocks, int tab_blocks,
+                                                        BinCold want, float2 *__restrict__ tab, BinCold *cold, int *tab_done) {
+  if ((int)blockIdx.x < prep_blocks) {
+    prep_view(blockIdx.x * PTB + threadIdx.x, calib, V, H, W, out);
+    return;
+  }
+  static_assert(sizeof(BinCold) % 4 == 0, "BinCold: compared as words");
+  const uint32_t *have = (const uint32_t *)cold, *w = (const uint32_t *)&want;
+  bool same = true;
+  for (int k = 0; k < (int)(sizeof(BinCold) / 4); k++) same = same && (have[k] == w[k]);
+  if (same) return;
+  tables_entry((blockIdx.x - prep_blocks) * PTB + threadIdx.x, want.g, want.fg, tab);
+  __syncthreads();
+  if (threadIdx.x == 0) {
+    __threadfence();
+    if (atomicAdd(tab_done, 1) == tab_blocks - 1) {
+      *cold = want;
+      *tab_done = 0;
+    }
+  }
+}
+__global__ __launch_bounds__(256) void k_fill_words_and_small(uint32_t *__restrict__ p, size_t n, uint32_t *a, int na,
+                                                              uint32_t *b, int nb, uint32_t *c, int nc) {
+  const size_t head = ((16u - (unsigned)((uintptr_t)p & 15u)) & 15u) / 4u < n ? ((16u - (unsigned)((uintptr_t)p & 15u)) & 15u) / 4u : n;
+  uint4 *q = (uint4 *)(p + head);
+  const size_t nq = (n - head) / 4;
+  const size_t tid = (size_t)blockIdx.x * 256 + threadIdx.x, nth = (size_t)gridDim.x * 256;
+  for (size_t i = tid; i < nq; i += nth) q[i] = make_uint4(0u, 0u, 0u, 0u);
+  const size_t done = head + nq * 4;
+  if (tid < head) p[tid] = 0u;
+  if (tid < n - done) p[done + tid] = 0u;
+  if (blockIdx.x == 0) {
+    for (int i = threadIdx.x; i < na; i += 256) a[i] = 0u;
+    for (int i = threadIdx.x; i < nb; i += 256) b[i] = 0u;
+    for (int i = threadIdx.x; i < nc; i += 256) c[i] = 0u;
+  }
+}
+__global__ void k_bp_tables_forget(BinCold *cold, int *tab_done) {
+  if (threadIdx.x < sizeof(BinCold) / 4) ((uint32_t *)cold)[threadIdx.x] = 0xFFFFFFFFu;
+  if (threadIdx.x == 0) *tab_done = 0;
 }
 
 __device__ __forceinline__ void backproject_f32(const FastCal &fc, int col, int row, float d, float &xf, float &yf,
@@ -686,12 +735,14 @@
 
 __device__ __forceinline__ void emit_voxel(const VoxOut &o, size_t at, const ViewCalib &c, const Recip &rc,
                                            const float *depth_v, int W, uint32_t pix, const void *masks,
-                                           int mask_format, int m, int max_inst, int HW, int v) {
+                                           int mask_format, int m, int max_inst, int HW, int v, bool lean) {
   const int row = (int)pix / W, col = (int)pix - row * W;
   double x, y, z;
   pixel_to_lidar(c, rc, col, row, depth_v[pix], x, y, z);
+  const uint32_t bits = masks ? mask_bits_at(masks, mask_format, v, max_inst, m, HW, (int)pix) : 0u;
+  o.it_bits[at] = bits;
+  if (lean && bits == 0u) return;
   o.vox_pix[at] = pix;
-  o.it_bits[at] = masks ? mask_bits_at(masks, mask_format, v, max_inst, m, HW, (int)pix) : 0u;
   o.it_x[at] = x;
   o.it_y[at] = y;
   o.it_z[at] = z;
@@ -704,6 +755,7 @@
   const uint32_t *bitmap, *wpre;
   int NSEG, BW, NJ, tiles_x;
 };
+template <bool LEAN>
 __global__ __launch_bounds__(VXB) void k_bp_vox(
     const float *__restrict__ depth, const ViewCalib *__restrict__ calib, const void *__restrict__ masks, int mask_format,
     const int *__restrict__ n_inst, int max_inst, int W, int HW, int64_t E_view, void *table, int64_t E_total, int cap_vox,
@@ -760,11 +812,13 @@
         keep = true;
       } else if (k < max_voxels) {
         const size_t at = (size_t)v * cap_vox + k;
-        out.vox_pix[at] = pix;
         out.it_bits[at] = m_bits;
-        out.it_x[at] = x;
-        out.it_y[at] = yy;
-        out.it_z[at] = z;
+        if (!LEAN || m_bits != 0u) {
+          out.vox_pix[at] = pix;
+          out.it_x[at] = x;
+          out.it_y[at] = yy;
+          out.it_z[at] = z;
+        }
       }
     }
     if (!keep) {
@@ -776,29 +830,32 @@
   }
 }
 
-__global__ __launch_bounds__(PB) void k_bp_rebin(
-    const float *__restrict__ depth, const ViewCalib *__restrict__ calib, dfu3d_bin_geom g, int W, int HW,
+__device__ __forceinline__ void ph_rebin(int v, int bx, int gx,
+    const float *__restrict__ depth, const ViewCalib *__restrict__ calib, const dfu3d_bin_geom &g, int W, int HW,
     int key_axis, const int *__restrict__ n_q, uint32_t *__restrict__ pix_bin) {
-  const int v = blockIdx.y;
   if (n_q[v] == 0) return;
   const ViewCalib c = calib[v];
   const Recip rc = make_recip(c);
   bool rerr = false;
-  for (int pix = blockIdx.x * PB + threadIdx.x; pix < HW; pix += gridDim.x * PB) {
+  for (int pix = bx * PB + threadIdx.x; pix < HW; pix += gx * PB) {
     double key;
     pix_bin[(size_t)v * HW + pix] = pixel_bin(c, rc, g, W, pix, depth[(size_t)v * HW + pix], key_axis, key, rerr);
   }
 }
-
-__global__ void k_ovf_alloc(void *table, int64_t E_total, int64_t E_view, int cap_q,
+__global__ __launch_bounds__(PB) void k_bp_rebin(
+    const float *__restrict__ depth, const ViewCalib *__restrict__ calib, dfu3d_bin_geom g, int W, int HW,
+    int key_axis, const int *__restrict__ n_q, uint32_t *__restrict__ pix_bin) {
+  ph_rebin(blockIdx.y, blockIdx.x, gridDim.x, depth, calib, g, W, HW, key_axis, n_q, pix_bin);
+}
+
+__device__ __forceinline__ void ph_ovf_alloc(int v, int bx, int gx, void *table, int64_t E_total, int64_t E_view, int cap_q,
                             const uint32_t *__restrict__ q_bins,
                             const int *__restrict__ n_q, int *__restrict__ q_cnt,
                             int *__restrict__ q_cursor, int HW,
                             uint32_t *__restrict__ status) {
-  const int v = blockIdx.y;
   const int no = min(n_q[v], cap_q);
   const Table T = table_view(table, E_total);
-  for (int s = blockIdx.x * blockDim.x + threadIdx.x; s < no; s += gridDim.x * blockDim.x) {
+  for (int s = bx * blockDim.x + threadIdx.x; s < no; s += gx * blockDim.x) {
     const int64_t e = (int64_t)v * E_view + q_bins[(size_t)v * cap_q + s];
     const int c = (int)T.cnt[e];
     const int off = atomicAdd(&q_cursor[v], c);
@@ -808,14 +865,18 @@
     T.cnt[e] = OVF_FLAG;
   }
 }
-
-__global__ __launch_bounds__(PB) void k_ovf_gather(
+__global__ void k_ovf_alloc(void *table, int64_t E_total, int64_t E_view, int cap_q, const uint32_t *__restrict__ q_bins,
+                            const int *__restrict__ n_q, int *__restrict__ q_cnt, int *__restrict__ q_cursor, int HW,
+                            uint32_t *__restrict__ status) {
+  ph_ovf_alloc(blockIdx.y, blockIdx.x, gridDim.x, table, E_total, E_view, cap_q, q_bins, n_q, q_cnt, q_cursor, HW, status);
+}
+
+__device__ __forceinline__ void ph_ovf_gather(int v, int bx, int gx,
     const uint32_t *__restrict__ pix_bin, void *table, int64_t E_total, int64_t E_view,
     int HW, const int *__restrict__ n_q, uint32_t *__restrict__ q_list) {
-  const int v = blockIdx.y;
   if (n_q[v] == 0) return;
   const Table T = table_view(table, E_total);
-  for (int base = blockIdx.x * PBLK + threadIdx.x * PPT; base < HW; base += gridDim.x * PBLK) {
+  for (int base = bx * PBLK + threadIdx.x * PPT; base < HW; base += gx * PBLK) {
     for (int k = 0; k < PPT; k++) {
       const int pix = base + k;
       if (pix >= HW) break;
@@ -829,8 +890,13 @@
     }
   }
 }
-
-__global__ __launch_bounds__(256) void k_ovf_select(
+__global__ __launch_bounds__(PB) void k_ovf_gather(
+    const uint32_t *__restrict__ pix_bin, void *table, int64_t E_total, int64_t E_view,
+    int HW, const int *__restrict__ n_q, uint32_t *__restrict__ q_list) {
+  ph_ovf_gather(blockIdx.y, blockIdx.x, gridDim.x, pix_bin, table, E_total, E_view, HW, n_q, q_list);
+}
+
+__device__ __forceinline__ void ph_ovf_select(int v, int bx, int gx,
     const float *__restrict__ depth, const ViewCalib *__restrict__ calib, int W, int HW,
     int key_axis, int max_points, void *table, int64_t E_total, int64_t E_view,
     int cap_ovf, const uint32_t *__restrict__ ovf_bins, const int *__restrict__ n_ovf,
@@ -838,12 +904,11 @@
   __shared__ int hist[256];
   __shared__ uint32_t s_sel[2];
   __shared__ unsigned long long s_min[4];
-  const int v = blockIdx.y;
   const int no = min(n_ovf[v], cap_ovf);
   const Table T = table_view(table, E_total);
   const ViewCalib c = calib[v];
   const Recip rc = make_recip(c);
-  for (int s = blockIdx.x; s < no; s += gridDim.x) {
+  for (int s = bx; s < no; s += gx) {
   const int64_t e = (int64_t)v * E_view + ovf_bins[(size_t)v * cap_ovf + s];
   const int n = ovf_cnt[(size_t)v * cap_ovf + s];
   const uint32_t *lst = ovf_list + (size_t)v * HW + T.rep[e];
@@ -915,37 +980,84 @@
   }
   }
 }
-
+__global__ __launch_bounds__(256) void k_ovf_select(
+    const float *__restrict__ depth, const ViewCalib *__restrict__ calib, int W, int HW,
+    int key_axis, int max_points, void *table, int64_t E_total, int64_t E_view,
+    int cap_ovf, const uint32_t *__restrict__ ovf_bins, const int *__restrict__ n_ovf,
+    const int *__restrict__ ovf_cnt, const uint32_t *__restrict__ ovf_list) {
+  ph_ovf_select(blockIdx.y, blockIdx.x, gridDim.x, depth, calib, W, HW, key_axis, max_points, table, E_total, E_view,
+                cap_ovf, ovf_bins, n_ovf, ovf_cnt, ovf_list);
+}
+
+__device__ __forceinline__ void ph_fix(int v, int bx, int gx, bool lean,
+    const float *__restrict__ depth, const ViewCalib *__restrict__ calib,
+    const void *__restrict__ masks, int mask_format, const int *__restrict__ n_inst, int max_inst, int W,
+    int HW, int max_voxels, int64_t E_view, void *table, int64_t E_total, int cap_vox, const VoxOut &out, int cap_q,
+    const uint32_t *__restrict__ q_bins, const int *__restrict__ q_rank, const int *__restrict__ n_q) {
+  const int no = min(n_q[v], cap_q);
+  if (bx * 256 >= no) return;
+  const Table T = table_view(table, E_total);
+  const ViewCalib c = calib[v];
+  const Recip rc = make_recip(c);
+  const int m = masks ? min(max(n_inst[v], 0), max_inst) : 0;
+  for (int s = bx * 256 + threadIdx.x; s < no; s += gx * 256) {
+    const int64_t e = (int64_t)v * E_view + q_bins[(size_t)v * cap_q + s];
+    const int k = q_rank[(size_t)v * cap_q + s];
+    if (k < max_voxels)
+      emit_voxel(out, (size_t)v * cap_vox + k, c, rc, depth + (size_t)v * HW, W, T.rep[e], masks, mask_format, m,
+                 max_inst, HW, v, lean);
+    T.kmin[e] = ~0ull;
+    T.combo[e] = ~0ull;
+    T.cnt[e] = 0u;
+    T.first[e] = NOBIN;
+    T.rep[e] = NOBIN;
+  }
+}
 __global__ __launch_bounds__(256) void k_bp_fix(
     const float *__restrict__ depth, const ViewCalib *__restrict__ calib,
     const void *__restrict__ masks, int mask_format, const int *__restrict__ n_inst, int max_inst, int W,
     int HW, int max_voxels, int64_t E_view, void *table, int64_t E_total, int cap_vox, VoxOut out, int cap_q,
     const uint32_t *__restrict__ q_bins, const int *__restrict__ q_rank, const int *__restrict__ n_q) {
-  const int v = blockIdx.y;
-  const int no = min(n_q[v], cap_q);
-  if (blockIdx.x * 256 >= no) return;
-  const Table T = table_view(table, E_total);
-  const ViewCalib c = calib[v];
-  const Recip rc = make_recip(c);
-  const int m = masks ? min(max(n_inst[v], 0), max_inst) : 0;
-  for (int s = blockIdx.x * 256 + threadIdx.x; s < no; s += gridDim.x * 256) {
-    const int64_t e = (int64_t)v * E_view + q_bins[(size_t)v * cap_q + s];
-    const int k = q_rank[(size_t)v * cap_q + s];
-    if (k < max_voxels)
-      emit_voxel(out, (size_t)v * cap_vox + k, c, rc, depth + (size_t)v * HW, W, T.rep[e], masks, mask_format, m,
-                 max_inst, HW, v);
-    T.kmin[e] = ~0ull;
-    T.combo[e] = ~0ull;
-    T.cnt[e] = 0u;
-    T.first[e] = NOBIN;
-    T.rep[e] = NOBIN;
-  }
+  ph_fix(blockIdx.y, blockIdx.x, gridDim.x, false, depth, calib, masks, mask_format, n_inst, max_inst, W, HW, max_voxels,
+         E_view, table, E_total, cap_vox, out, cap_q, q_bins, q_rank, n_q);
 }
 
 __global__ void k_bp_finalize(int V, int max_voxels, int cap_vox, int *__restrict__ n_vox) {
   const int v = blockIdx.x * blockDim.x + threadIdx.x;
   if (v >= V) return;
   n_vox[v] = min(min(n_vox[v], cap_vox), max_voxels);
+}
+
+struct RepairArgs {
+  const float *depth;
+  const ViewCalib *calib;
+  const void *masks;
+  const int *n_inst;
+  void *table;
+  uint32_t *pix_bin, *q_list, *q_bins, *status;
+  int *q_cnt, *q_cursor, *q_rank, *n_q, *n_vox;
+  int64_t E_view, E_total;
+  int mask_format, max_inst, W, HW, key_axis, max_points, max_voxels, cap_vox, cap_q, lean;
+  VoxOut out;
+};
+static_assert(PB == 256, "k_bp_repair: every phase with 256 threads");
+__global__ __launch_bounds__(256) void k_bp_repair(dfu3d_bin_geom g, RepairArgs a) {
+  const int v = blockIdx.x;
+  if (threadIdx.x == 0) a.n_vox[v] = min(min(a.n_vox[v], a.cap_vox), a.max_voxels);
+  if (a.n_q[v] == 0) return;
+  ph_rebin(v, 0, 1, a.depth, a.calib, g, a.W, a.HW, a.key_axis, a.n_q, a.pix_bin);
+  ph_ovf_alloc(v, 0, 1, a.table, a.E_total, a.E_view, a.cap_q, a.q_bins, a.n_q, a.q_cnt, a.q_cursor, a.HW, a.status);
+  __threadfence();
+  __syncthreads();
+  ph_ovf_gather(v, 0, 1, a.pix_bin, a.table, a.E_total, a.E_view, a.HW, a.n_q, a.q_list);
+  __threadfence();
+  __syncthreads();
+  ph_ovf_select(v, 0, 1, a.depth, a.calib, a.W, a.HW, a.key_axis, a.max_points, a.table, a.E_total, a.E_view, a.cap_q,
+                a.q_bins, a.n_q, a.q_cnt, a.q_list);
+  __threadfence();
+  __syncthreads();
+  ph_fix(v, 0, 1, a.lean != 0, a.depth, a.calib, a.masks, a.mask_format, a.n_inst, a.max_inst, a.W, a.HW, a.max_voxels,
+         a.E_view, a.table, a.E_total, a.cap_vox, a.out, a.cap_q, a.q_bins, a.q_rank, a.n_q);
 }
 
 __global__ void k_selftest_classify(const ViewCalib *__restrict__ calib, const FastCal *__restrict__ fastcal,
@@ -1110,17 +1222,16 @@
   if (pix_words) *pix_words = 2 * V * HW;
   const int64_t NSEG = table_segments(table_entries), OW = (NSEG + 3) / 4;
   if (blk_words) *blk_words = 4 * (int64_t)V + V * BW + V * OW + V * NJ + V * NSEG + 3 * V * cap_q + 20 * (int64_t)V + (int64_t)(sizeof(BinCold) / 4) + 16 +
-                              4 * (int64_t)(TAB_T_MAX + TAB_P_MAX) + 16;
+                              4 * (int64_t)(TAB_T_MAX + TAB_P_MAX) + 16 + 4;
   return 0;
 }
 
-extern "C" int dfu3d_backproject_bin(
+static int backproject_bin_impl(
     const float *depth, const float *calib, const void *masks, int32_t mask_format, const int32_t *n_inst,
     int32_t V, int32_t max_inst, int32_t H, int32_t W, const dfu3d_bin_geom *geom,
     int32_t key_axis, void *table, uint32_t *pix_bin, int32_t *blk_cnt, int32_t cap_vox,
     int32_t *n_vox, uint32_t *vox_pix, uint32_t *it_bits, double *it_x, double *it_y,
-    double *it_z, uint32_t *status, int32_t phases, void *stream) {
-  DFU3D_CLEAR_STALE_ERROR();
+    double *it_z, uint32_t *status, int32_t phases, void *stream, int chain) {
   if (!depth || !calib || !geom || !table || !pix_bin || !blk_cnt || !n_vox || !vox_pix ||
       !it_bits || !it_x || !it_y || !it_z || !status)
     return DFU3D_EINVAL;
@@ -1157,6 +1268,7 @@
   FastCal *fastcal = (FastCal *)(((uintptr_t)(q_rank + (size_t)V * cap_q) + 15) & ~(uintptr_t)15);
   BinCold *cold = (BinCold *)(fastcal + V);
   const float2 *tab = (const float2 *)(cold + 1);
+  int *tab_done = (int *)(tab + 2 * (size_t)(TAB_T_MAX + TAB_P_MAX));
   const FastGeom fg = make_fast_geom(*geom);
   int pix_bits = 1;
   while ((1ll << pix_bits) < HW64) pix_bits++;
@@ -1166,11 +1278,24 @@
   const VoxWalk Wk = {seg_list, n_occ, bitmap, wpre, NSEG, BW, NJ, tiles_x};
 
   if (phases & DFU3D_BP_BIN) {
-    if (dfu3d_fill_async(blk_cnt, 0, sizeof(int) * (4 * (size_t)V + (size_t)V * BW + (size_t)V * OW), st) != hipSuccess) return DFU3D_ELAUNCH;
-    hipLaunchKernelGGL(k_bp_prep, dim3((V + 63) / 64), dim3(64), 0, st, cal, V, H, W, fastcal);
-    DFU3D_LAUNCH_CHECK();
-    hipLaunchKernelGGL(k_bp_tables, dim3((tables_threads(fg, *geom) + 255) / 256), dim3(256), 0, st, *geom, fg, (float2 *)tab, cold);
-    DFU3D_LAUNCH_CHECK();
+    if (!chain && dfu3d_fill_async(blk_cnt, 0, sizeof(int) * (4 * (size_t)V + (size_t)V * BW + (size_t)V * OW), st) != hipSuccess) return DFU3D_ELAUNCH;
+    if (chain) {
+      BinCold want;
+      memset(&want, 0, sizeof(want));
+      memcpy(&want.g, geom, sizeof(dfu3d_bin_geom));
+      const size_t pad0 = offsetof(dfu3d_bin_geom, max_voxels) + sizeof(int32_t), pad1 = offsetof(dfu3d_bin_geom, theta_min);
+      memset((char *)&want.g + pad0, 0, pad1 - pad0);
+      want.fg = fg;
+      const int prep_blocks = (V + PTB - 1) / PTB, tab_blocks = (tables_threads(fg, *geom) + PTB - 1) / PTB;
+      hipLaunchKernelGGL(k_bp_prep_tables, dim3(prep_blocks + tab_blocks), dim3(PTB), 0, st, cal, V, H, W, fastcal, prep_blocks,
+                         tab_blocks, want, (float2 *)tab, cold, tab_done);
+      DFU3D_LAUNCH_CHECK();
+    } else {
+      hipLaunchKernelGGL(k_bp_prep, dim3((V + 63) / 64), dim3(64), 0, st, cal, V, H, W, fastcal);
+      DFU3D_LAUNCH_CHECK();
+      hipLaunchKernelGGL(k_bp_tables, dim3((tables_threads(fg, *geom) + 255) / 256), dim3(256), 0, st, *geom, fg, (float2 *)tab, cold);
+      DFU3D_LAUNCH_CHECK();
+    }
     hipLaunchKernelGGL(k_bp_bin, dim3(tiles_x * ((tiles_y + RPT - 1) / RPT), V), dim3(PB), 0, st, depth, cal, fastcal, tab,
                        make_hot_geom(*geom, fg), W, H, tiles_x, tiles_y, key_axis, E_view, table, E_total, n_amb, q_list, pix_bits,
                        bitmap, BW, (uint8_t *)occ, OW);
@@ -1188,12 +1313,28 @@
   }
   if (phases & DFU3D_BP_VOX) {
     const int gx = std::min((NSEG + (VXB / 64) - 1) / (VXB / 64), VOX_GX);
-    hipLaunchKernelGGL(k_bp_vox, dim3(gx, (V + 7) / 8 * 8), dim3(VXB), 0, st, depth, cal, masks, mask_format, n_inst, max_inst, W, HW, E_view,
-                       table, E_total, cap_vox, Wk, out, key_axis, pix_bits, geom->max_points_per_voxel, geom->max_voxels,
-                       cap_q, q_bins, q_rank, n_q, status, V);
+    if (chain)
+      hipLaunchKernelGGL(k_bp_vox<true>, dim3(gx, (V + 7) / 8 * 8), dim3(VXB), 0, st, depth, cal, masks, mask_format, n_inst, max_inst, W, HW, E_view,
+                         table, E_total, cap_vox, Wk, out, key_axis, pix_bits, geom->max_points_per_voxel, geom->max_voxels,
+                         cap_q, q_bins, q_rank, n_q, status, V);
+    else
+      hipLaunchKernelGGL(k_bp_vox<false>, dim3(gx, (V + 7) / 8 * 8), dim3(VXB), 0, st, depth, cal, masks, mask_format, n_inst, max_inst, W, HW, E_view,
+                         table, E_total, cap_vox, Wk, out, key_axis, pix_bits, geom->max_points_per_voxel, geom->max_voxels,
+                         cap_q, q_bins, q_rank, n_q, status, V);
     DFU3D_LAUNCH_CHECK();
   }
-  if (phases & DFU3D_BP_REPAIR) {
+  if ((phases & DFU3D_BP_REPAIR) && chain) {
+    RepairArgs a;
+    a.depth = depth; a.calib = cal; a.masks = masks; a.n_inst = n_inst; a.table = table;
+    a.pix_bin = pix_bin; a.q_list = q_list; a.q_bins = q_bins; a.status = status;
+    a.q_cnt = q_cnt; a.q_cursor = q_cursor; a.q_rank = q_rank; a.n_q = n_q; a.n_vox = n_vox;
+    a.E_view = E_view; a.E_total = E_total;
+    a.mask_format = mask_format; a.max_inst = max_inst; a.W = W; a.HW = HW; a.key_axis = key_axis;
+    a.max_points = geom->max_points_per_voxel; a.max_voxels = geom->max_voxels; a.cap_vox = cap_vox; a.cap_q = cap_q; a.lean = 1;
+    a.out = out;
+    hipLaunchKernelGGL(k_bp_repair, dim3(V), dim3(256), 0, st, *geom, a);
+    DFU3D_LAUNCH_CHECK();
+  } else if (phases & DFU3D_BP_REPAIR) {
     const int nblk = (HW + PB - 1) / PB;
     hipLaunchKernelGGL(k_bp_rebin, dim3(nblk < 16 ? nblk : 16, V), dim3(PB), 0, st, depth, cal, *geom, W, HW,
                        key_axis, n_q, pix_bin);
@@ -1219,3 +1360,55 @@
   }
   return DFU3D_OK;
 }
+
+extern "C" int dfu3d_backproject_bin(
+    const float *depth, const float *calib, const void *masks, int32_t mask_format, const int32_t *n_inst,
+    int32_t V, int32_t max_inst, int32_t H, int32_t W, const dfu3d_bin_geom *geom,
+    int32_t key_axis, void *table, uint32_t *pix_bin, int32_t *blk_cnt, int32_t cap_vox,
+    int32_t *n_vox, uint32_t *vox_pix, uint32_t *it_bits, double *it_x, double *it_y,
+    double *it_z, uint32_t *status, int32_t phases, void *stream) {
+  DFU3D_CLEAR_STALE_ERROR();
+  return backproject_bin_impl(depth, calib, masks, mask_format, n_inst, V, max_inst, H, W, geom, key_axis, table, pix_bin,
+                              blk_cnt, cap_vox, n_vox, vox_pix, it_bits, it_x, it_y, it_z, status, phases, stream, 0);
+}
+
+int dfu3d_backproject_bin_chain(
+    const float *depth, const float *calib, const void *masks, int32_t mask_format, const int32_t *n_inst,
+    int32_t V, int32_t max_inst, int32_t H, int32_t W, const dfu3d_bin_geom *geom,
+    int32_t key_axis, void *table, uint32_t *pix_bin, int32_t *blk_cnt, int32_t cap_vox,
+    int32_t *n_vox, uint32_t *vox_pix, uint32_t *it_bits, double *it_x, double *it_y,
+    double *it_z, uint32_t *status, void *stream) {
+  return backproject_bin_impl(depth, calib, masks, mask_format, n_inst, V, max_inst, H, W, geom, key_axis, table, pix_bin,
+                              blk_cnt, cap_vox, n_vox, vox_pix, it_bits, it_x, it_y, it_z, status, DFU3D_BP_ALL, stream, 1);
+}
+
+int dfu3d_bp_clear_chain(int32_t *blk_cnt, int32_t V, int32_t H, int32_t W, int64_t table_entries, void *a, size_t bytes_a,
+                         void *b, size_t bytes_b, void *c, size_t bytes_c, void *stream) {
+  if (!blk_cnt || V <= 0 || H <= 0 || W <= 0 || table_entries <= 0 || (((uintptr_t)blk_cnt) & 3u)) return DFU3D_EINVAL;
+  const int64_t tiles_x = (W + TILE_W - 1) / TILE_W, tiles_y = (H + TILE_H - 1) / TILE_H;
+  const int64_t BW = tiles_x * tiles_y * 32;
+  const int64_t NSEG = table_segments(table_entries), OW = (NSEG + 3) / 4;
+  const size_t n = 4 * (size_t)V + (size_t)V * BW + (size_t)V * OW, quads = (n + 3) / 4;
+  const unsigned grid = (unsigned)((quads + 255) / 256 < 8192 ? (quads + 255) / 256 : 8192);
+  hipLaunchKernelGGL(k_fill_words_and_small, dim3(grid ? grid : 1), dim3(256), 0, (hipStream_t)stream, (uint32_t *)blk_cnt, n,
+                     (uint32_t *)a, (int)(bytes_a / 4), (uint32_t *)b, (int)(bytes_b / 4), (uint32_t *)c, (int)(bytes_c / 4));
+  DFU3D_LAUNCH_CHECK();
+  return DFU3D_OK;
+}
+
+int dfu3d_bp_tables_forget(int32_t *blk_cnt, int32_t V, int32_t H, int32_t W, int32_t cap_vox, int32_t max_points,
+                           int64_t table_entries, void *stream) {
+  if (!blk_cnt || V <= 0 || H <= 0 || W <= 0 || cap_vox <= 0 || max_points < 1 || table_entries <= 0) return DFU3D_EINVAL;
+  const int64_t HW = (int64_t)H * W;
+  const int64_t tiles_x = (W + TILE_W - 1) / TILE_W, tiles_y = (H + TILE_H - 1) / TILE_H;
+  const int64_t BW = tiles_x * tiles_y * 32, NJ = (int64_t)H * tiles_x;
+  const int64_t cap_q = queue_cap(HW, max_points, cap_vox);
+  const int64_t NSEG = table_segments(table_entries), OW = (NSEG + 3) / 4;
+  int32_t *q_end = blk_cnt + 4 * (int64_t)V + V * BW + V * OW + V * NJ + V * NSEG + 3 * V * cap_q;
+  FastCal *fastcal = (FastCal *)(((uintptr_t)q_end + 15) & ~(uintptr_t)15);
+  BinCold *cold = (BinCold *)(fastcal + V);
+  float2 *tab = (float2 *)(cold + 1);
+  hipLaunchKernelGGL(k_bp_tables_forget, dim3(1), dim3(64), 0, (hipStream_t)stream, cold, (int *)(tab + 2 * (size_t)(TAB_T_MAX + TAB_P_MAX)));
+  DFU3D_LAUNCH_CHECK();
+  return DFU3D_OK;
+}
```

New measurement: 10540 frames/s (median of 6 runs). 3.3% higher.
